# ZJU-FAST-Lab/uneven_planner

Hardware: AMD Instinct MI355X
Metric: MINCO traj-opts/sec (batch) (higher is better)
Workload: dtype f64

## Files before the change

### include/uneven_hip.h

```cpp
#ifndef UNEVEN_HIP_H
#define UNEVEN_HIP_H

#include <stdint.h>

#ifdef __cplusplus
extern "C" {
#endif

typedef struct uph_map uph_map;
typedef struct uph_ctx uph_ctx;
typedef struct uph_kino uph_kino;

#define UPH_OK 0
#define UPH_ERR_INVALID (-1)
#define UPH_ERR_HIP (-2)
#define UPH_ERR_NO_DEVICE (-3)
#define UPH_ERR_LIMIT (-4)
#define UPH_ERR_NO_CACHE (-5)

#define UPH_RET_STOPPED 3
#define UPH_RET_UNSUPPORTED 4

#define UPH_RET_LEFT_TILE 5
#define UPH_TILE_MARGIN 2.0
// ... 114 lines not shown
int uph_map_create(const uph_map_params* mp, int device, uph_map** out);
int uph_map_create_f32(const uph_map_params* mp, int device, uph_map** out);
int uph_map_storage_bytes(const uph_map* m);
int uph_map_create_tile(const uph_map_params* mp, int device, int32_t x0, int32_t x1, int32_t f32, uph_map** out);
int uph_map_tile(const uph_map* m, int32_t* x0, int32_t* x1);
int uph_map_fill_fbm(uph_map* m, const uph_fbm_params* fp, int32_t x0, int32_t x1);
int uph_fbm_table(const uph_fbm_params* fp, double* table);
int uph_map_get_window(uph_map* m, int32_t x0, int32_t x1, int32_t y0, int32_t y1, double* rxs2);
void uph_map_destroy(uph_map* m);
int uph_map_dims(const uph_map* m, int32_t dims3[3]);
int uph_map_set_cells(uph_map* m, const double* rxs2);
int uph_map_get_cells(uph_map* m, double* rxs2, double* c, char* occ, char* occ_r2);
int uph_map_save_csv(const char* path, const double* rxs2, const int32_t dims3[3]);
int uph_map_load_csv(const char* path, const int32_t dims3[3], double* rxs2, double* c, int64_t* n_lines);
int uph_map_save_bin(const char* path, const double* rxs2, const int32_t dims3[3]);
int uph_map_load_bin(const char* path, const int32_t dims3[3], double* rxs2);
int uph_map_save_cache(uph_map* m, const char* csv_path, const char* bin_path);
int uph_map_load_cache(uph_map* m, const char* csv_path, const char* bin_path, int32_t* source);
int uph_map_build(uph_map* m, const float* xyz, int64_t n, int32_t x0, int32_t x1);
int uph_map_build_filtered(uph_map* m, const float* xyz, int64_t n, int32_t x0, int32_t x1);
typedef struct uph_map_update_info {
    int32_t dirty[4];
    int32_t changed[4];
    int32_t n_refit;
    int32_t n_far;
    int32_t n_changed;
    int32_t full_refit;
    int64_t n_removed, n_added, n_cloud;
} uph_map_update_info;
int uph_map_update(uph_map* m, const float box[4], const float* xyz, int64_t n, uph_map_update_info* info);
int uph_map_update_rect(const uph_map_params* mp, const float box[4], int32_t rect[4]);
int uph_map_update_stages(uph_map* m, double* out6);
int uph_map_build_multi(uph_map* const* maps, int32_t n_gpus, const float* xyz, int64_t n);
int uph_multi_slab_plan(int32_t nx, int32_t n_gpus, int32_t* x0, int32_t* x1, int32_t* per, int32_t* in_place);
int uph_map_fill_fbm_multi(uph_map* const* maps, int32_t n_gpus, const uph_fbm_params* fp);
int uph_map_multi_stats(uph_map* lead, double* fit_ms, double* exchange_ms, double* commit_ms, double* exchange_device_ms, int32_t* via_rccl);
int uph_rccl_selftest(int32_t n_devices, char* info, int32_t info_cap);
void uph_multi_shutdown(void);

int uph_map_cells_device(uph_map* m, void** dptr, int64_t* nbytes);
int uph_map_commit(uph_map* m);
int uph_map_export_slab_dev(uph_map* m, int32_t x0, int32_t x1, void* dst_dev);
int uph_map_import_cells_dev(uph_map* m, const void* src_dev);
int uph_terrain_query(uph_map* m, const double* pos, int32_t n, double* values7, double* grads21);
int uph_frontend_query(uph_map* m, const double* pos, int32_t n, double* sigma, int32_t* occ, int32_t* occ_xy);
int uph_terrain_pose_query(uph_map* m, const double* pos, int32_t n, double* pose12);
int uph_frontend_query_ms(uph_map* m, double* kernel_ms);
int64_t uph_map_filter_cloud(const float* xyz, int64_t n, float* out_xyz, int64_t cap);
int uph_map_build_stats(uph_map* m, double* kernel_ms, int64_t* cell_iters, int64_t* cloud_points);
int uph_map_build_stages(uph_map* m, double* out6);
int64_t uph_map_built_cloud(uph_map* m, float* out_xyz, int64_t cap);

int uph_kino_create(uph_map* m, const uph_kino_params* kp, int32_t slots, uph_kino** out);
void uph_kino_destroy(uph_kino* k);
int uph_kino_slots(const uph_kino* k);
int uph_kino_set_wps(uph_kino* k, int32_t wps);
int uph_kino_set_flags(uph_kino* k, int32_t flags);
int uph_kino_primitives(const uph_kino* k);
int uph_kino_plan_batch(uph_kino* k, int32_t B, const double* starts, const double* goals, int32_t path_cap, double* paths, int32_t* n_path, int32_t* status,
                        int32_t* iter_num, int32_t* use_node_num, int32_t max_expand, int32_t exp_cap, int32_t* expanded);
int uph_kino_stats(uph_kino* k, double* kernel_ms);

#define UPH_PLAN_PATH_CAP 1024
int uph_plan_upload(uph_kino* k, uph_ctx* c, const uph_manager_params* mp, int32_t B, const double* starts, const double* goals, int32_t path_cap,
                    int32_t* status, int32_t* traj_of, int32_t* n_inner_xy, int32_t* n_inner_yaw);
int uph_replan_upload(uph_kino* k, uph_ctx* src, uph_ctx* dst, const uph_manager_params* mp, int32_t B, const int32_t* src_traj, const double* t_switch,
                      const double* goals, int32_t path_cap, double* switch_states, int32_t* status, int32_t* traj_of, int32_t* n_inner_xy, int32_t* n_inner_yaw);
int uph_traj_states(uph_ctx* c, int32_t n, const int32_t* traj, const double* t, double* out10);
#define UPH_REFINE_AT_END 7
int uph_refine_upload(uph_ctx* src, uph_ctx* dst, int32_t B, const int32_t* src_traj, const double* t_switch, double* switch_states ,
                      int32_t* status, int32_t* traj_of, int32_t* n_inner_xy, int32_t* n_inner_yaw);
int uph_plan_staged(uph_ctx* c, int32_t cap_xy, int32_t cap_yaw, double* init_xy, double* end_xy, double* init_yaw, double* end_yaw, double* inner_xy,
                    double* inner_yaw, int32_t* n_inner_xy, int32_t* n_inner_yaw, double* total_time);

int uph_ctx_create(uph_map* m, const uph_opt_params* p, uph_ctx** out);
void uph_ctx_destroy(uph_ctx* c);
int uph_ctx_set_lanes(uph_ctx* c, int32_t lanes);
int uph_ctx_set_xcd_locality(uph_ctx* c, int32_t group);
int uph_ctx_set_wps(uph_ctx* c, int32_t wps);
int uph_ctx_set_sample_precision(uph_ctx* c, int32_t bits);
int uph_ctx_set_rho(uph_ctx* c, double rho);
int uph_ctx_get_rho(uph_ctx* c, double* rho);
int uph_ctx_set_trial_abandon(uph_ctx* c, int32_t on);

int uph_ctx_set_trace(uph_ctx* c, int32_t cap);
int uph_ctx_get_trace(uph_ctx* c, double* out);

int uph_optimize_batch(uph_ctx* c, int32_t B, const uph_problem* probs, uph_result* results);
int uph_optimize_batch_multi(uph_ctx* const* ctxs, int32_t n_gpus, int32_t B, const uph_problem* probs, uph_result* results);
int uph_multi_batch_plan(int32_t n_gpus, int32_t B, const uph_problem* probs, int32_t* share_of, double* predicted_cost);
int uph_batch_count(const uph_ctx* c);
int uph_batch_origin(const uph_ctx* c, int32_t* idx);
int uph_batch_upload(uph_ctx* c, int32_t B, const uph_problem* probs);
int uph_batch_solve(uph_ctx* c);
int uph_batch_solve_async(uph_ctx* c);
int uph_batch_wait(uph_ctx* c);
int uph_batch_download(uph_ctx* c, uph_result* results);
int uph_batch_stats(uph_ctx* c, double* kernel_ms, int64_t* evals, int64_t* sample_evals, int64_t* lbfgs_iters, int64_t* hist_bytes);
int uph_batch_abandon_stats(uph_ctx* c, int64_t* out5);

int uph_batch_prepare_ms(uph_ctx* c, double* ms);

int uph_batch_cycles(uph_ctx* c, long long* out);

int uph_eval_batch(uph_ctx* c, const double* x_packed, double* f, double* grad_packed, int32_t repeat);
int uph_penalty_batch(uph_ctx* c, int32_t repeat, int32_t store_residuals, double* cost, double* gdcxy_packed, double* gdcyaw_packed, double* gdT2);
int uph_init_scaling_batch(uph_ctx* c);
int uph_microbench_batch(uph_ctx* c, int32_t reps);
int uph_batch_set_state(uph_ctx* c, const double* lambda, const double* mu, const double* scale_cx, const double* scale_fx, const double* rho);
int uph_batch_set_x(uph_ctx* c, const double* x_packed);
int uph_batch_alm_passes(uph_ctx* c, int32_t max_passes);
int uph_batch_set_lbfgs_state(uph_ctx* c, const double* g, const double* d, const double* pf, const double* lm_s, const double* lm_y, const double* lm_ys, const double* scal5);
int uph_batch_lbfgs_resume(uph_ctx* c, int32_t budget, int32_t finish_pass);
int uph_batch_get_lbfgs_state(uph_ctx* c, double* g, double* d, double* pf, double* lm_s, double* lm_y, double* lm_ys, double* scal8);
int uph_report_batch(uph_ctx* c, double* out7);

#define UPH_ROLLOUT_STATE 1
#define UPH_ROLLOUT_TERRAIN 2
#define UPH_ROLLOUT_POSE 4
#define UPH_ROLLOUT_ALL 7
#define UPH_ROLLOUT_MAX_SAMPLES 262144
int uph_rollout_sizes(int32_t B, const int32_t* n_xy, const double* T_xy, const int32_t* n_yaw, const double* T_yaw, double dt, int32_t with_end,
                      int64_t* offsets);
int uph_rollout_plan(uph_ctx* c, double dt, int32_t with_end, int64_t* offsets);
int uph_rollout_batch(uph_ctx* c, double dt, int32_t with_end, int32_t channels, int32_t b0, int32_t b1, double* out);
int uph_rollout_batch_dev(uph_ctx* c, double dt, int32_t with_end, int32_t channels, int32_t b0, int32_t b1, void* out_dev);

#define UPH_CHECK_OCC_BIT 7
int uph_check_limits(const uph_ctx* c, double* lim7);
int uph_check_window(double dt, int32_t with_end, double total, double t_from, double t_to, int32_t* q_lo, int32_t* q_hi, int32_t* end_row);
int uph_check_batch(uph_ctx* c, int32_t n, const int32_t* traj, const double* t_from, const double* t_to , double dt, int32_t with_end,
                    const double* lim7 , double* first_t , int32_t* first_mask ,
                    int32_t* counts , double* worst , double* worst_t );
int uph_check_kernel_ms(const uph_ctx* c, double* kernel_ms);

int uph_locate_batch(uph_ctx* c, int32_t n, const int32_t* traj, const double* poses , const double* t_from, const double* t_to ,
                     double dt, int32_t with_end, double* near_t , double* near_d2 , int32_t* count , double* t ,
                     int32_t* refined , double* state , double* d2 , double* err );
int uph_within_batch(uph_ctx* c, int32_t n, const int32_t* traj, const double* rects , const double* t_from, const double* t_to ,
                     double dt, int32_t with_end, double* enter_t , double* leave_t , int32_t* counts );
int uph_locate_kernel_ms(const uph_ctx* c, double* kernel_ms);

int uph_separation_times(double t_from, double t_to, double dt, int64_t* K);
int uph_extent_batch(uph_ctx* c, int32_t n, const int32_t* traj, const double* t0, const double* t_from, const double* t_to, double dt,
                     double* box , int32_t* counts );
int uph_separation_batch(uph_ctx* ca, uph_ctx* cb , int32_t n, const int32_t* traj_a, const int32_t* traj_b, const double* t0_a, const double* t0_b,
                         const double* t_from, const double* t_to, double dt, const double* radius, double* min_d2 , double* min_t ,
                         double* first_t , double* last_t , int32_t* counts );
int uph_conflict_candidates(int32_t n, const double* box , const double* radius , int64_t cap, int32_t* pairs , int64_t* n_pairs);
int uph_conflicts_batch(uph_ctx* c, int32_t n, const int32_t* traj, const double* t0, const double* radius , double t_from, double t_to, double dt,
                        int64_t cap, int32_t* pairs , double* rows , int32_t* below ,
                        int64_t* n_conflicts, int64_t* n_candidates);
int uph_separation_kernel_ms(const uph_ctx* c, double* kernel_ms);

int uph_footprint_radii(int32_t n, const double* shape , const double* margin , double* r );
int uph_footprint_separation_batch(uph_ctx* ca, uph_ctx* cb , int32_t n, const int32_t* traj_a, const int32_t* traj_b, const double* t0_a,
                                   const double* t0_b, const double* t_from, const double* t_to, double dt, const double* shape_a ,
                                   const double* shape_b , const double* margin , double* min_c2 , double* min_t ,
                                   double* first_t , double* last_t , int32_t* counts );
int uph_footprint_conflicts_batch(uph_ctx* c, int32_t n, const int32_t* traj, const double* t0, const double* shape ,
                                  const double* margin , double t_from, double t_to, double dt, int64_t cap, int32_t* pairs ,
                                  double* rows , int32_t* below , int64_t* n_conflicts,
                                  int64_t* n_candidates);
int uph_footprint_kernel_ms(const uph_ctx* c, double* kernel_ms);

#define UPH_DELAY_TILE 128
// ... 28 lines not shown
```

### uneven_planner_amd/_lib.py

```python
import ctypes as C
import os

_HERE = os.path.dirname(os.path.abspath(__file__))
LIB_PATH = os.environ.get("UNEVENHIP_LIB") or os.path.join(_HERE, "libunevenhip.so")


class MapParams(C.Structure):
    _fields_ = [("iter_num", C.c_int32), ("map_size_x", C.c_double), ("map_size_y", C.c_double),
                ("ellipsoid_x", C.c_double), ("ellipsoid_y", C.c_double), ("ellipsoid_z", C.c_double),
                ("xy_resolution", C.c_double), ("yaw_resolution", C.c_double), ("min_cnormal", C.c_double),
                ("max_rho", C.c_double), ("gravity", C.c_double)]


class OptParams(C.Structure):
    _fields_ = [("rho_T", C.c_double), ("rho_ter", C.c_double), ("max_vel", C.c_double), ("max_acc_lon", C.c_double),
                ("max_acc_lat", C.c_double), ("max_kap", C.c_double), ("min_cxi", C.c_double), ("max_sig", C.c_double),
                ("use_scaling", C.c_int32), ("rho", C.c_double), ("beta", C.c_double), ("gamma", C.c_double),
                ("epsilon_con", C.c_double), ("max_iter", C.c_double), ("g_epsilon", C.c_double),
                ("min_step", C.c_double), ("inner_max_iter", C.c_double), ("delta", C.c_double),
                ("mem_size", C.c_int32), ("past", C.c_int32), ("int_K", C.c_int32)]


class ManagerParams(C.Structure):
    _fields_ = [("piece_len", C.c_double), ("mean_vel", C.c_double), ("init_time_times", C.c_double), ("yaw_piece_times", C.c_double),
# ... 18 lines not shown
                ("full_refit", C.c_int32), ("n_removed", C.c_int64), ("n_added", C.c_int64), ("n_cloud", C.c_int64)]


FBM_MAX_WAVES = 48
FBM_TABLE_DOUBLES = 4 * FBM_MAX_WAVES + 12 + 9
DP = C.POINTER(C.c_double)


class Problem(C.Structure):
    _fields_ = [("n_inner_xy", C.c_int32), ("n_inner_yaw", C.c_int32), ("init_xy", C.c_double * 6),
                ("end_xy", C.c_double * 6), ("init_yaw", C.c_double * 3), ("end_yaw", C.c_double * 3),
                ("inner_xy", DP), ("inner_yaw", DP), ("total_time", C.c_double)]


class Result(C.Structure):
    _fields_ = [("ret_code", C.c_int32), ("alm_iters", C.c_int32), ("lbfgs_iters", C.c_int32), ("evals", C.c_int32),
                ("last_lbfgs_ret", C.c_int32), ("cost", C.c_double), ("jerk_cost", C.c_double),
                ("piece_T_xy", C.c_double), ("piece_T_yaw", C.c_double), ("rho_final", C.c_double),
                ("scale_fx", C.c_double), ("x_final", DP), ("c_xy", DP), ("c_yaw", DP), ("hx", DP), ("gx", DP),
                ("lambda_", DP), ("mu", DP), ("scale_cx", DP)]


_VP = C.c_void_p
_I32, _I64 = C.c_int32, C.c_int64
SYMBOLS = {
    "uph_last_error": (C.c_char_p, []),
    "uph_device_count": (C.c_int, []),
    "uph_version": (C.c_char_p, []),
    "uph_resample_batch": (C.c_int, [C.POINTER(ManagerParams), _I32, DP, C.POINTER(_I64), _I32, _I32, DP, DP, DP, DP, DP, DP, C.POINTER(_I32), C.POINTER(_I32), DP, DP]),
    "uph_map_create": (C.c_int, [C.POINTER(MapParams), C.c_int, C.POINTER(_VP)]),
    "uph_map_create_f32": (C.c_int, [C.POINTER(MapParams), C.c_int, C.POINTER(_VP)]),
    "uph_map_storage_bytes": (C.c_int, [_VP]),
    "uph_map_create_tile": (C.c_int, [C.POINTER(MapParams), C.c_int, _I32, _I32, _I32, C.POINTER(_VP)]),
    "uph_map_tile": (C.c_int, [_VP, C.POINTER(_I32), C.POINTER(_I32)]),
    "uph_map_fill_fbm": (C.c_int, [_VP, C.POINTER(FbmParams), _I32, _I32]),
    "uph_fbm_table": (C.c_int, [C.POINTER(FbmParams), DP]),
    "uph_map_get_window": (C.c_int, [_VP, _I32, _I32, _I32, _I32, DP]),
    "uph_map_save_csv": (C.c_int, [C.c_char_p, DP, C.POINTER(_I32)]),
    "uph_map_load_csv": (C.c_int, [C.c_char_p, C.POINTER(_I32), DP, DP, C.POINTER(_I64)]),
    "uph_map_save_bin": (C.c_int, [C.c_char_p, DP, C.POINTER(_I32)]),
    "uph_map_load_bin": (C.c_int, [C.c_char_p, C.POINTER(_I32), DP]),
    "uph_map_save_cache": (C.c_int, [_VP, C.c_char_p, C.c_char_p]),
    "uph_map_load_cache": (C.c_int, [_VP, C.c_char_p, C.c_char_p, C.POINTER(_I32)]),
    "uph_map_destroy": (None, [_VP]),
    "uph_map_dims": (C.c_int, [_VP, C.POINTER(_I32)]),
    "uph_map_set_cells": (C.c_int, [_VP, DP]),
    "uph_map_get_cells": (C.c_int, [_VP, DP, DP, C.c_char_p, C.c_char_p]),
    "uph_map_build": (C.c_int, [_VP, C.POINTER(C.c_float), _I64, _I32, _I32]),
    "uph_map_build_filtered": (C.c_int, [_VP, C.POINTER(C.c_float), _I64, _I32, _I32]),
    "uph_map_update": (C.c_int, [_VP, C.POINTER(C.c_float), C.POINTER(C.c_float), _I64, C.POINTER(MapUpdateInfo)]),
    "uph_map_update_rect": (C.c_int, [C.POINTER(MapParams), C.POINTER(C.c_float), C.POINTER(_I32)]),
    "uph_map_update_stages": (C.c_int, [_VP, DP]),
    "uph_map_build_multi": (C.c_int, [C.POINTER(_VP), _I32, C.POINTER(C.c_float), _I64]),
    "uph_map_fill_fbm_multi": (C.c_int, [C.POINTER(_VP), _I32, C.POINTER(FbmParams)]),
    "uph_multi_slab_plan": (C.c_int, [_I32, _I32, C.POINTER(_I32), C.POINTER(_I32), C.POINTER(_I32), C.POINTER(_I32)]),
    "uph_multi_batch_plan": (C.c_int, [_I32, _I32, C.POINTER(Problem), C.POINTER(_I32), DP]),
    "uph_map_multi_stats": (C.c_int, [_VP, DP, DP, DP, DP, C.POINTER(_I32)]),
    "uph_multi_shutdown": (None, []),
    "uph_rccl_selftest": (C.c_int, [_I32, C.c_char_p, _I32]),
    "uph_optimize_batch_multi": (C.c_int, [C.POINTER(_VP), _I32, _I32, C.POINTER(Problem), C.POINTER(Result)]),
    "uph_batch_count": (C.c_int, [_VP]),
    "uph_batch_origin": (C.c_int, [_VP, C.POINTER(_I32)]),
    "uph_map_cells_device": (C.c_int, [_VP, C.POINTER(_VP), C.POINTER(_I64)]),
    "uph_map_commit": (C.c_int, [_VP]),
    "uph_map_export_slab_dev": (C.c_int, [_VP, _I32, _I32, _VP]),
    "uph_map_import_cells_dev": (C.c_int, [_VP, _VP]),
    "uph_terrain_query": (C.c_int, [_VP, DP, _I32, DP, DP]),
    "uph_frontend_query": (C.c_int, [_VP, DP, _I32, DP, C.POINTER(C.c_int32), C.POINTER(C.c_int32)]),
    "uph_terrain_pose_query": (C.c_int, [_VP, DP, _I32, DP]),
    "uph_frontend_query_ms": (C.c_int, [_VP, DP]),
    "uph_map_filter_cloud": (_I64, [C.POINTER(C.c_float), _I64, C.POINTER(C.c_float), _I64]),
    "uph_map_build_stats": (C.c_int, [_VP, DP, C.POINTER(_I64), C.POINTER(_I64)]),
    "uph_map_build_stages": (C.c_int, [_VP, DP]),
    "uph_map_built_cloud": (_I64, [_VP, C.POINTER(C.c_float), _I64]),
    "uph_ctx_create": (C.c_int, [_VP, C.POINTER(OptParams), C.POINTER(_VP)]),
    "uph_ctx_destroy": (None, [_VP]),
    "uph_ctx_set_lanes": (C.c_int, [_VP, _I32]),
    "uph_ctx_set_wps": (C.c_int, [_VP, _I32]),
    "uph_ctx_set_xcd_locality": (C.c_int, [_VP, _I32]),
    "uph_ctx_set_sample_precision": (C.c_int, [_VP, _I32]),
    "uph_ctx_set_rho": (C.c_int, [_VP, C.c_double]),
    "uph_ctx_get_rho": (C.c_int, [_VP, DP]),
    "uph_ctx_set_trial_abandon": (C.c_int, [_VP, _I32]),
    "uph_ctx_set_trace": (C.c_int, [_VP, _I32]),
    "uph_ctx_get_trace": (C.c_int, [_VP, DP]),
    "uph_optimize_batch": (C.c_int, [_VP, _I32, C.POINTER(Problem), C.POINTER(Result)]),
    "uph_batch_upload": (C.c_int, [_VP, _I32, C.POINTER(Problem)]),
    "uph_batch_solve": (C.c_int, [_VP]),
    "uph_batch_solve_async": (C.c_int, [_VP]),
    "uph_batch_wait": (C.c_int, [_VP]),
    "uph_batch_download": (C.c_int, [_VP, C.POINTER(Result)]),
    "uph_batch_stats": (C.c_int, [_VP, DP, C.POINTER(_I64), C.POINTER(_I64), C.POINTER(_I64), C.POINTER(_I64)]),
    "uph_batch_prepare_ms": (C.c_int, [_VP, DP]),
    "uph_batch_abandon_stats": (C.c_int, [_VP, C.POINTER(_I64)]),
    "uph_batch_cycles": (C.c_int, [_VP, C.POINTER(C.c_longlong)]),
    "uph_build_id": (C.c_char_p, []),
    "uph_eval_batch": (C.c_int, [_VP, DP, DP, DP, _I32]),
    "uph_penalty_batch": (C.c_int, [_VP, _I32, _I32, DP, DP, DP, DP]),
    "uph_init_scaling_batch": (C.c_int, [_VP]),
    "uph_microbench_batch": (C.c_int, [_VP, _I32]),
    "uph_batch_set_state": (C.c_int, [_VP, DP, DP, DP, DP, DP]),
    "uph_report_batch": (C.c_int, [_VP, DP]),
    "uph_rollout_sizes": (C.c_int, [_I32, C.POINTER(_I32), DP, C.POINTER(_I32), DP, C.c_double, _I32, C.POINTER(_I64)]),
    "uph_rollout_plan": (C.c_int, [_VP, C.c_double, _I32, C.POINTER(_I64)]),
    "uph_rollout_batch": (C.c_int, [_VP, C.c_double, _I32, _I32, _I32, _I32, DP]),
    "uph_rollout_batch_dev": (C.c_int, [_VP, C.c_double, _I32, _I32, _I32, _I32, _VP]),
    "uph_batch_set_x": (C.c_int, [_VP, DP]),
    "uph_batch_alm_passes": (C.c_int, [_VP, _I32]),
    "uph_batch_set_lbfgs_state": (C.c_int, [_VP, DP, DP, DP, DP, DP, DP, DP]),
    "uph_batch_lbfgs_resume": (C.c_int, [_VP, _I32, _I32]),
    "uph_batch_get_lbfgs_state": (C.c_int, [_VP, DP, DP, DP, DP, DP, DP, DP]),
    "uph_kino_create": (C.c_int, [_VP, C.POINTER(KinoParams), _I32, C.POINTER(_VP)]),
    "uph_kino_destroy": (None, [_VP]),
    "uph_kino_slots": (C.c_int, [_VP]),
    "uph_kino_set_wps": (C.c_int, [_VP, _I32]),
    "uph_kino_set_flags": (C.c_int, [_VP, _I32]),
    "uph_kino_primitives": (C.c_int, [_VP]),
    "uph_kino_plan_batch": (C.c_int, [_VP, _I32, DP, DP, _I32, DP, C.POINTER(_I32), C.POINTER(_I32), C.POINTER(_I32), C.POINTER(_I32), _I32, _I32, C.POINTER(_I32)]),
    "uph_kino_stats": (C.c_int, [_VP, DP]),
    "uph_plan_upload": (C.c_int, [_VP, _VP, C.POINTER(ManagerParams), _I32, DP, DP, _I32, C.POINTER(_I32), C.POINTER(_I32), C.POINTER(_I32), C.POINTER(_I32)]),
    "uph_plan_staged": (C.c_int, [_VP, _I32, _I32, DP, DP, DP, DP, DP, DP, C.POINTER(_I32), C.POINTER(_I32), DP]),
    "uph_replan_upload": (C.c_int, [_VP, _VP, _VP, C.POINTER(ManagerParams), _I32, C.POINTER(_I32), DP, DP, _I32, DP, C.POINTER(_I32), C.POINTER(_I32),
                                    C.POINTER(_I32), C.POINTER(_I32)]),
    "uph_traj_states": (C.c_int, [_VP, _I32, C.POINTER(_I32), DP, DP]),
    "uph_refine_upload": (C.c_int, [_VP, _VP, _I32, C.POINTER(_I32), DP, DP, C.POINTER(_I32), C.POINTER(_I32), C.POINTER(_I32), C.POINTER(_I32)]),
    "uph_check_limits": (C.c_int, [_VP, DP]),
    "uph_check_window": (C.c_int, [C.c_double, _I32, C.c_double, C.c_double, C.c_double, C.POINTER(_I32), C.POINTER(_I32), C.POINTER(_I32)]),
    "uph_check_batch": (C.c_int, [_VP, _I32, C.POINTER(_I32), DP, DP, C.c_double, _I32, DP, DP, C.POINTER(_I32), C.POINTER(_I32), DP, DP]),
    "uph_check_kernel_ms": (C.c_int, [_VP, DP]),
    "uph_locate_batch": (C.c_int, [_VP, _I32, C.POINTER(_I32), DP, DP, DP, C.c_double, _I32, DP, DP, C.POINTER(_I32), DP, C.POINTER(_I32), DP, DP, DP]),
    "uph_within_batch": (C.c_int, [_VP, _I32, C.POINTER(_I32), DP, DP, DP, C.c_double, _I32, DP, DP, C.POINTER(_I32)]),
    "uph_locate_kernel_ms": (C.c_int, [_VP, DP]),
    "uph_separation_times": (C.c_int, [C.c_double, C.c_double, C.c_double, C.POINTER(_I64)]),
    "uph_extent_batch": (C.c_int, [_VP, _I32, C.POINTER(_I32), DP, DP, DP, C.c_double, DP, C.POINTER(_I32)]),
    "uph_separation_batch": (C.c_int, [_VP, _VP, _I32, C.POINTER(_I32), C.POINTER(_I32), DP, DP, DP, DP, C.c_double, DP, DP, DP, DP, DP, C.POINTER(_I32)]),
    "uph_conflict_candidates": (C.c_int, [_I32, DP, DP, _I64, C.POINTER(_I32), C.POINTER(_I64)]),
    "uph_conflicts_batch": (C.c_int, [_VP, _I32, C.POINTER(_I32), DP, DP, C.c_double, C.c_double, C.c_double, _I64, C.POINTER(_I32), DP, C.POINTER(_I32),
                                      C.POINTER(_I64), C.POINTER(_I64)]),
    "uph_separation_kernel_ms": (C.c_int, [_VP, DP]),
    "uph_footprint_radii": (C.c_int, [_I32, DP, DP, DP]),
    "uph_footprint_separation_batch": (C.c_int, [_VP, _VP, _I32, C.POINTER(_I32), C.POINTER(_I32), DP, DP, DP, DP, C.c_double, DP, DP, DP, DP, DP, DP, DP,
                                                 C.POINTER(_I32)]),
    "uph_footprint_conflicts_batch": (C.c_int, [_VP, _I32, C.POINTER(_I32), DP, DP, DP, C.c_double, C.c_double, C.c_double, _I64, C.POINTER(_I32), DP,
                                                C.POINTER(_I32), C.POINTER(_I64), C.POINTER(_I64)]),
    "uph_footprint_kernel_ms": (C.c_int, [_VP, DP]),
    "uph_delay_times": (C.c_int, [C.c_double, C.c_double, _I32, DP]),
    "uph_delay_levels": (C.c_int, [_I32, _I64, C.POINTER(_I32), C.POINTER(_I32)]),
    "uph_delay_sweep_batch": (C.c_int, [_VP, _VP, _I32, C.POINTER(_I32), C.POINTER(_I32), DP, DP, DP, DP, C.c_double, DP, C.c_double, C.c_double, _I32, DP, DP,
                                        C.POINTER(_I32), C.POINTER(_I32), C.POINTER(_I32)]),
    "uph_delay_extent_batch": (C.c_int, [_VP, _I32, C.POINTER(_I32), DP, DP, DP, C.c_double, C.c_double, C.c_double, _I32, DP, C.POINTER(_I32)]),
    "uph_delays_batch": (C.c_int, [_VP, _I32, C.POINTER(_I32), DP, DP, C.POINTER(_I32), C.c_double, C.c_double, C.c_double, C.c_double, C.c_double, _I32,
                                   C.POINTER(_I32), DP, C.POINTER(_I32), C.POINTER(_I64), C.POINTER(_I32), C.POINTER(_I32)]),
    "uph_footprint_delay_sweep_batch": (C.c_int, [_VP, _VP, _I32, C.POINTER(_I32), C.POINTER(_I32), DP, DP, DP, DP, C.c_double, DP, DP, DP, C.c_double, C.c_double,
                                                  _I32, DP, DP, C.POINTER(_I32), C.POINTER(_I32), C.POINTER(_I32), C.POINTER(_I32)]),
    "uph_footprint_delays_batch": (C.c_int, [_VP, _I32, C.POINTER(_I32), DP, DP, DP, C.POINTER(_I32), C.c_double, C.c_double, C.c_double, C.c_double, C.c_double,
                                             _I32, C.POINTER(_I32), DP, C.POINTER(_I32), C.POINTER(_I64), C.POINTER(_I32), C.POINTER(_I32)]),
    "uph_delay_kernel_ms": (C.c_int, [_VP, DP]),
}

_LIB = None


UPH_ERR_NO_CACHE = -5
UPH_PLAN_PATH_CAP = 1024
UPH_MAX_PIECE_XY = 128
UPH_MAX_PIECE_YAW = 256
# ... 70 lines not shown
```

### uneven_planner_amd/alm_traj_opt.py

```python
import ctypes as C

import numpy as np

from . import _lib

HILL_OPT_PARAMS = dict(rho_T=100000.0, rho_ter=10.0, max_vel=0.5, max_acc_lon=5.0, max_acc_lat=10.0, max_kap=2.1,
                       min_cxi=0.8, max_sig=0.05, use_scaling=True, rho=1.0, beta=1000.0, gamma=1.0,
                       epsilon_con=0.001, max_iter=10.0, g_epsilon=1.0e-3, min_step=1.0e-32, inner_max_iter=10000.0,
                       delta=1.0e-4, mem_size=256, past=3, int_K=16)
_INT_FIELDS = ("use_scaling", "mem_size", "past", "int_K")


def pack_problems(probs, int_K=16, with_sizes=False):
    arr = (_lib.Problem * len(probs))()
    keep, sizes = [], []
    for i, pr in enumerate(probs):
        ixy = np.ascontiguousarray(np.asarray(pr["inner_xy"], dtype=np.float64).T)
        iyw = np.ascontiguousarray(pr["inner_yaw"], dtype=np.float64)
        keep += [ixy, iyw]
        a = arr[i]
        a.n_inner_xy, a.n_inner_yaw = ixy.shape[0], iyw.shape[0]
        a.init_xy[:] = np.asarray(pr["init_xy"], dtype=np.float64).T.ravel().tolist()
        a.end_xy[:] = np.asarray(pr["end_xy"], dtype=np.float64).T.ravel().tolist()
        a.init_yaw[:] = np.asarray(pr["init_yaw"], dtype=np.float64).ravel().tolist()
# ... 417 lines not shown
        raise _lib.UnevenHipError("delay_levels: a pair does not have 0 <= i < j < n")
    level = np.zeros(n, dtype=np.int32)
    for j, i in sorted(map(tuple, pairs[:, ::-1].tolist())):
        level[j] = max(level[j], level[i] + 1)
    return level


def delay_schedule(sweep, pairs, n, n_delays=None, order=None):
    pairs = np.asarray(pairs, dtype=np.int64).reshape(-1, 2)
    ahead = [[] for _ in range(n)]
    for h, i in sorted(map(tuple, pairs.tolist())):
        ahead[i].append(h)
    choice, blocker = np.zeros(n, dtype=np.int32), np.full(n, -1, dtype=np.int32)
    placed = np.zeros(n, dtype=bool)
    for i in (range(n) if order is None else order):
        assert all(placed[h] for h in ahead[i]), "delay_schedule: a vehicle ahead of %d is not placed yet" % i
        placed[i] = True
        if not ahead[i]:
            continue
        below = np.stack([np.asarray(sweep(h, max(int(choice[h]), 0), i)) for h in ahead[i]])
        nd = below.shape[1] if n_delays is None else int(n_delays[i])
        clear = np.nonzero((below[:, :nd] == 0).all(axis=0))[0]
        if clear.size:
            choice[i] = clear[0]
        else:
            choice[i] = -1
            blocker[i] = ahead[i][int(np.nonzero(below[:, 0] > 0)[0][0])]
    return dict(choice=choice, blocker=blocker)


class ALMTrajOpt:
    def __init__(self, uneven_map=None, params=None):
        self.L = _lib.load()
        q = dict(HILL_OPT_PARAMS)
        if params:
            q.update(params)
        for k, v in q.items():
            setattr(self, k, v)
        self._pnames = list(q.keys())
        self.h = None
        self.uneven_map = None
        self.in_opt = False
        self._B = 0
        self._sizes = []
        self._last = []
        if uneven_map is not None:
            self.setEnvironment(uneven_map)

    def __del__(self):
        try:
            if self.h:
                self.L.uph_ctx_destroy(self.h)
                self.h = None
        except Exception:
            pass

    def setEnvironment(self, env):
        self.uneven_map = env
        if self.h:
            self.L.uph_ctx_destroy(self.h)
            self.h = None
        p = _lib.OptParams(**{k: (int(getattr(self, k)) if k in _INT_FIELDS else float(getattr(self, k))) for k in self._pnames})
        h = C.c_void_p()
        _lib.check(self.L.uph_ctx_create(env.h, C.byref(p), C.byref(h)), "uph_ctx_create")
        self.h = h

    def set_lanes(self, lanes):
        _lib.check(self.L.uph_ctx_set_lanes(self.h, int(lanes)), "uph_ctx_set_lanes")

    def set_xcd_locality(self, group):
        _lib.check(self.L.uph_ctx_set_xcd_locality(self.h, int(group)), "uph_ctx_set_xcd_locality")

    def set_wps(self, wps):
        _lib.check(self.L.uph_ctx_set_wps(self.h, int(wps)), "uph_ctx_set_wps")

    def set_sample_precision(self, bits):
        _lib.check(self.L.uph_ctx_set_sample_precision(self.h, int(bits)), "uph_ctx_set_sample_precision")

    def set_rho(self, rho):
        _lib.check(self.L.uph_ctx_set_rho(self.h, float(rho)), "uph_ctx_set_rho")

    def set_trial_abandon(self, on):
        _lib.check(self.L.uph_ctx_set_trial_abandon(self.h, 1 if on else 0), "uph_ctx_set_trial_abandon")

    def get_rho(self):
        r = C.c_double(0)
        _lib.check(self.L.uph_ctx_get_rho(self.h, C.byref(r)), "uph_ctx_get_rho")
        return r.value

    def _make_problems(self, probs):
        arr, keep, self._sizes = pack_problems(probs, int(self.int_K), with_sizes=True)
        return arr, keep

    def upload(self, probs):
        arr, keep = self._make_problems(probs)
        self._B = 0
        _lib.check(self.L.uph_batch_upload(self.h, len(probs), arr), "uph_batch_upload")
        self._B = len(probs)
        self._trace_cap_up = getattr(self, "_trace_cap", 0)

    def solve(self):
        _lib.check(self.L.uph_batch_solve(self.h), "uph_batch_solve")

    def solve_async(self):
        _lib.check(self.L.uph_batch_solve_async(self.h), "uph_batch_solve_async")

    def wait(self):
        _lib.check(self.L.uph_batch_wait(self.h), "uph_batch_wait")

    def stats(self):
        ms = C.c_double(0)
        v = [C.c_int64(0) for _ in range(4)]
        _lib.check(self.L.uph_batch_stats(self.h, C.byref(ms), *[C.byref(x) for x in v]), "uph_batch_stats")
        pm = C.c_double(0)
        _lib.check(self.L.uph_batch_prepare_ms(self.h, C.byref(pm)), "uph_batch_prepare_ms")
        ab = (C.c_int64 * 5)()
        _lib.check(self.L.uph_batch_abandon_stats(self.h, ab), "uph_batch_abandon_stats")
        return dict(kernel_ms=ms.value, prepare_ms=pm.value, evals=v[0].value, sample_evals=v[1].value, lbfgs_iters=v[2].value, hist_bytes=v[3].value,
                    ls_rejected=ab[0], ls_guarded=ab[1], ls_abandoned=ab[2], chunks_skipped=ab[3], adjoints_skipped=ab[4])

    def cycles(self):
        out = np.zeros((max(0, self.L.uph_batch_count(self.h)), 16), dtype=np.int64)
        _lib.check(self.L.uph_batch_cycles(self.h, out.ctypes.data_as(C.POINTER(C.c_longlong))), "uph_batch_cycles")
        return out

    def origin(self):
        idx = np.zeros(max(0, self.L.uph_batch_count(self.h)), dtype=np.int32)
        _lib.check(self.L.uph_batch_origin(self.h, _ip(idx)), "uph_batch_origin")
        return idx

    def download(self, full=True):
        res, bufs = self._result_array(self._sizes, full)
        _lib.check(self.L.uph_batch_download(self.h, res), "uph_batch_download")
        self._last = self._collect(res, bufs)
        return self._last

    def optimize_batch(self, probs):
        self.upload(probs)
        self.solve()
        return self.download()

    def _result_array(self, sizes, full):
        res = (_lib.Result * len(sizes))()
        bufs = []
        for i, sz in enumerate(sizes):
            b = dict(x=np.zeros(sz["n"]), c_xy=np.zeros((6 * sz["Nxy"], 2)), c_yaw=np.zeros(6 * sz["Nyaw"]))
            r = res[i]
            r.x_final, r.c_xy, r.c_yaw = _dp(b["x"]), _dp(b["c_xy"]), _dp(b["c_yaw"])
            if full:
                b.update(hx=np.zeros(sz["S"]), gx=np.zeros(6 * sz["S"]), lam=np.zeros(sz["S"]), mu=np.zeros(6 * sz["S"]), scale_cx=np.zeros(7 * sz["S"]))
                r.hx, r.gx, r.lambda_, r.mu, r.scale_cx = _dp(b["hx"]), _dp(b["gx"]), _dp(b["lam"]), _dp(b["mu"]), _dp(b["scale_cx"])
            bufs.append(b)
        return res, bufs

    @staticmethod
    def _collect(res, bufs):
        out = []
        for i, b in enumerate(bufs):
            r = res[i]
            b.update(ret=r.ret_code, alm_iters=r.alm_iters, lbfgs_iters=r.lbfgs_iters, evals=r.evals, last_lbfgs_ret=r.last_lbfgs_ret,
                     cost=r.cost, jerk_cost=r.jerk_cost, T_xy=r.piece_T_xy, T_yaw=r.piece_T_yaw, rho_final=r.rho_final, scale_fx=r.scale_fx)
            out.append(b)
        return out

    def prepare_boundary(self, probs, full=False):
        arr, keep = self._make_problems(probs)
# ... 518 lines not shown
```

### uneven_planner_amd/csrc/solver_program.hpp

```cpp
#pragma once
#include "terrain_dev.hpp"
#include "trajectory_dev.hpp"
#include "uph_common.hpp"

namespace uph {

#ifndef UPH_GRID_FROM_MEM
#define UPH_GRID_FROM_MEM 1
#endif
#ifndef UPH_PHASE_MASK
#define UPH_PHASE_MASK 15
#endif
#ifndef UPH_STATE_PROBE
#define UPH_STATE_PROBE(st) do { } while (0)
#endif
#ifndef UPH_SCALING_WB
#define UPH_SCALING_WB 8
#endif
#ifndef UPH_SC_XB
#define UPH_SC_XB 9
#endif
#ifndef UPH_SC_YB
#define UPH_SC_YB 14
#endif
#ifndef UPH_SC_WLO
#define UPH_SC_WLO 2
#endif
#ifndef UPH_SC_WHI
#define UPH_SC_WHI 3
#endif

#ifndef UPH_ASIDE_PREP
#define UPH_ASIDE_PREP 1
#endif
template <class WG, class F>
UPH_HD void asideKnotSolve(WG& wg, int lenW, int lenX, int n, F f) {
    (void)lenW; (void)lenX;
    wg.pfor(n, f);
}

template <class WG, class SR = double>
struct Solver {
    WG& wg;
    const GridDev& grid;
    const OptParams& P;
    const BatchDev& bd;
    const TrajDesc& td;
    int Nxy, Nyaw, n, S, K, mem, CH, CHP, recd;
    int CHS;
    int* rtag;
    double *x, *xp, *g, *gp, *d, *cxy, *cyaw, *Gxy, *Gyaw, *gamxy, *gamyaw, *bt, *rec, *wtab, *ttab, *pf, *hd;
    double* ab;
    int* abn;
    static constexpr int AB_DOUBLES = 4;
    double* up;
    static constexpr int UP_DOUBLES = 6;
    UPH_HD void tally(int k, bool yes) {
#if defined(__HIP_DEVICE_COMPILE__)
        if (yes && wg.wave == 0) abn[k] = abn[k] + 1;
#else
        if (yes) abn[k]++;
#endif
    }
    double *dual, *res, *scl, *hist;
    int hrow, hnp;
    const double *Wr_xy, *Wr_yaw;
    double rho, scale_fx, Txy, Tyaw, last_jerk, last_gd;
    long long hist_reads;
    long long cyc[16];
    long long t_last_eval_end;
    long long* sub_t = nullptr;
    int evals, bidx, trace_n;
    float inv_k1;
    double ec_irho, ec_step, ec_invK, ec_iTyaw, ec_omega, ec_omega_h;

    static constexpr int REC_FIELDS = 12;
    static UPH_HD size_t ldsDoubles(int Nxy, int Nyaw, int n, int CH, int mem, int K) {
        size_t recd = (size_t)REC_FIELDS * (CH + 1) + (CH + 1) / 2;
        const size_t nvec = 2 * (Nxy + 5) + (Nyaw + 5);
        const size_t knd = (size_t)knotBufDoubles(Nxy + 1, 4) + knotBufDoubles(Nyaw + 1, 2), adj = (size_t)knotBufDoubles(Nxy, 4) + knotBufDoubles(Nyaw, 2) + nvec;
        recd = recd < knd ? knd : recd;
        recd = recd < adj ? adj : recd;
        recd = recd < (size_t)mem ? (size_t)mem : recd;
        const size_t td_ = (size_t)Nxy + K + 2;
        return (size_t)5 * n + (nvec < td_ ? td_ : nvec) + 2 * (12 * Nxy + 6 * Nyaw) + recd + (size_t)6 * (K + 1) + THOMAS_DOUBLES + MAX_PAST + 8 + 18 + AB_DOUBLES + UP_DOUBLES;
    }

    UPH_HD Solver(WG& w, const GridDev& gr, const OptParams& p, const BatchDev& b, int bi, double* lds)
        : wg(w), grid(gr), P(p), bd(b), td(b.desc[bi]) {
        bidx = bi;
        Nxy = td.Nxy; Nyaw = td.Nyaw; n = td.n; S = td.S; K = P.int_K; mem = P.mem_size;
        inv_k1 = 1.0f / (float)(K + 1);
        CH = wg.size(); CHP = CH + 1; recd = REC_FIELDS * CHP + (CH + 1) / 2;
        CHS = CH;
#if !defined(UPH_ALIGNED_CHUNKS) || UPH_ALIGNED_CHUNKS
        {
            const int ppc = CH / (K + 1);
            if (ppc >= 1 && (Nxy + ppc - 1) / ppc == (S + CH - 1) / CH) CHS = ppc * (K + 1);
        }
#endif
        double* q = lds;
        x = q; q += n; g = q; q += n; d = q; q += n;
        xp = q; q += n; gp = q; q += n;
        const int nvec = 2 * (Nxy + 5) + (Nyaw + 5);
        bt = q;
        gamxy = q; gamyaw = q + 2 * (Nxy + 5);
        q += nvec < Nxy + K + 2 ? Nxy + K + 2 : nvec;
        cxy = q; q += 12 * Nxy; cyaw = q; q += 6 * Nyaw;
        Gxy = q; q += 12 * Nxy; Gyaw = q; q += 6 * Nyaw;
        wtab = q; q += 6 * (K + 1);
        rec = q;
        {
            size_t rd = (size_t)recd;
            const size_t knd = (size_t)knotBufDoubles(Nxy + 1, 4) + knotBufDoubles(Nyaw + 1, 2), adj = (size_t)knotBufDoubles(Nxy, 4) + knotBufDoubles(Nyaw, 2) + nvec;
            rd = rd < knd ? knd : rd; rd = rd < adj ? adj : rd; rd = rd < (size_t)mem ? (size_t)mem : rd;
            q += rd;
        }
        rtag = (int*)(rec + (size_t)REC_FIELDS * CHP);
        ttab = q; q += THOMAS_DOUBLES;
        pf = q; q += MAX_PAST + 8;
        hd = q; q += 18;
        ab = q; q += AB_DOUBLES;
        abn = (int*)(ab + 1);
        up = q; q += UP_DOUBLES;
        dual = bd.dual + 7 * td.off_s; res = bd.res + 7 * td.off_s; scl = bd.scl + 7 * td.off_s;
        hist = bd.hist + td.off_hist; hrow = histRowDoubles(n); hnp = 64 * histNQ(n);
        Wr_xy = bd.ops[td.op_xy].Wr; Wr_yaw = bd.ops[td.op_yaw].Wr;
        rho = 0; scale_fx = 1.0; Txy = Tyaw = 0; last_jerk = 0; hist_reads = 0; evals = 0; trace_n = 0;
        for (int q = 0; q < 16; q++) cyc[q] = 0;
        t_last_eval_end = 0;
        wg.pfor(18 + THOMAS_DOUBLES, [&](int t) {
            if (t == 0) { ab[0] = 0.0; abn[0] = abn[1] = abn[2] = abn[3] = 0; }
            if (t < 18) hd[t] = t < 6 ? td.init_xy[t] : (t < 12 ? td.end_xy[t - 6] : (t < 15 ? td.init_yaw[t - 12] : td.end_yaw[t - 15]));
            else ttab[t - 18] = bd.thomas[t - 18];
        });
    }

    UPH_HD void tracePush(double v) {
        if (bd.trace != nullptr && trace_n < bd.trace_cap) {
            const int at = trace_n;
            wg.one([&]() { bd.trace[(size_t)bidx * bd.trace_cap + at] = v; });
        }
        trace_n++;
    }

    static UPH_HD int divSmall(int a, int b, float inv) {
        int q = (int)((float)a * inv);
        const int r = a - q * b;
        if (r < 0) q--;
        else if (r >= b) q++;
        return q;
    }
    static UPH_HD int knotCol(int j, int N) { return j == 0 ? 0 : (j == N ? N + 2 : j + 2); }
    UPH_HD double knotPos(const double* xin, int j, int dd) const {
        if (dd < 2) return j == 0 ? hd[dd] : (j == Nxy ? hd[6 + dd] : xin[1 + 2 * (j - 1) + dd]);
        return j == 0 ? hd[12] : (j == Nyaw ? hd[15] : xin[1 + 2 * (Nxy - 1) + (j - 1)]);
    }

    UPH_HD double dot(const double* a, const double* b, int m) {
        double r[1];
        wg.template sum<1>(m, r, [&](int i, double* acc) { acc[0] += a[i] * b[i]; });
        return r[0];
    }
    UPH_HD double absmax(const double* a, int m) {
        return wg.maxv(m, [&](int i) { return fabs(a[i]); });
    }

    template <bool STEP>
    UPH_HD void generate(double* xin, double st) {
        UPH_MARK("generate");
        const long long tsub_start = wg.clock();
        const double tau_ = STEP ? fma(st, d[0], xp[0]) : xin[0];
        const double Ttot = expC2(tau_);
        Txy = wg.bcast(Ttot / (double)Nxy);
        Tyaw = wg.bcast(Ttot / (double)Nyaw);
#if !(UPH_ASIDE_PREP)
        ec_iTyaw = wg.bcast(1.0 / Tyaw);
#endif
        const double Tx = Txy, Ty = Tyaw;
        double* zxy = rec;
        double* zyaw = rec + knotBufDoubles(Nxy + 1, 4);
        wg.pfor(2 * (Nxy + 1) + (Nyaw + 1), [&](int t) {
            const bool isxy = t < 2 * (Nxy + 1);
            const int j = isxy ? (t >> 1) : t - 2 * (Nxy + 1), dd = isxy ? (t & 1) : 2, N = isxy ? Nxy : Nyaw, os = isxy ? 2 : 1;
            const double T1 = isxy ? Tx : Ty;
            const double* h0 = isxy ? hd + (dd & 1) : hd + 12;
            const double* h1 = isxy ? hd + 6 + (dd & 1) : hd + 15;
            double* z = isxy ? zxy + knotOffJ(j, 4) + (dd & 1) : zyaw + knotOffJ(j, 2);
            if (STEP && t == 0) xin[0] = tau_;
            if (j == 0) { z[0] = T1 * h0[os]; z[os] = T1 * T1 * h0[2 * os]; }
            else if (j == N) { z[0] = T1 * h1[os]; z[os] = T1 * T1 * h1[2 * os]; }
            else {
                double pm, p0, pp;
                if (STEP) {
                    const int ix = isxy ? 1 + 2 * (j - 1) + dd : 1 + 2 * (Nxy - 1) + (j - 1), ws = isxy ? 2 : 1;
                    p0 = fma(st, d[ix], xp[ix]);
                    pm = j == 1 ? h0[0] : fma(st, d[ix - ws], xp[ix - ws]);
                    pp = j == N - 1 ? h1[0] : fma(st, d[ix + ws], xp[ix + ws]);
                    xin[ix] = p0;
                } else { pm = knotPos(xin, j - 1, dd); p0 = knotPos(xin, j, dd); pp = knotPos(xin, j + 1, dd); }
                const double dp = pp - p0, dm = p0 - pm;
                double r0 = 20.0 * (dp - dm), r1 = -15.0 * (dp + dm);
                if (j == 1) { const double v0 = T1 * h0[os], a0 = T1 * T1 * h0[2 * os]; r0 += 8.0 * v0 + a0; r1 += 7.0 * v0 + a0; }
                if (j == N - 1) { const double vN = T1 * h1[os], aN = T1 * T1 * h1[2 * os]; r0 += -8.0 * vN + aN; r1 += 7.0 * vN - aN; }
                z[0] = r0; z[os] = r1;
            }
        });
// ... 575 lines not shown
    template <bool STEP>
    UPH_HD double eval(double* xin, double* gout, double st = 0.0, double thr = __builtin_huge_val()) {
        evals++;
        long long t0 = wg.clock();
        if (t_last_eval_end) cyc[5] += t0 - t_last_eval_end;
        if (UPH_PHASE_MASK & 1) generate<STEP>(xin, st);
        const double tau = wg.bcast(xin[0]);
        const double jw = wg.bcast(P.use_scaling ? scale_trick_jerk * scale_fx : scale_fx);
        double js[3] = {0.0, 0.0, 0.0};
        if (UPH_PHASE_MASK & 1) expand(xin, jw, js);
        long long t1 = wg.clock(); cyc[0] += t1 - t0;
        last_jerk = js[0];
        const double jerk_cost = wg.bcast(P.use_scaling ? js[0] * scale_fx * scale_trick_jerk : js[0] * scale_fx);
        evalConsts(evalStep());
        if (STEP && thr < __builtin_huge_val()) {
#if UPH_ASIDE_PREP
            double eq = wg.bcast(up[3]);
            pinv(eq);
            const double tau_lb = P.rho_T * eq * scale_fx;
#else
            double tq = tau;
            pinv(tq);
            const double tau_lb = P.rho_T * expC2(tq) * scale_fx;
#endif
            const double lbd = wg.bcast(ab[0]);
            const double L0 = wg.bcast(jerk_cost + tau_lb - lbd);
            const double mag = wg.bcast(fabs(jerk_cost) + fabs(tau_lb) + lbd);
            if (L0 > thr + ABANDON_REL * mag && L0 < __builtin_huge_val() && ec_omega >= 0.0) {
                tally(2, true);
                t_last_eval_end = wg.clock();
                return L0;
            }
        }
        double sm[3] = {0.0, 0.0, 0.0};
        wg.template accBegin<3>();
        for (int s0 = 0; s0 < S; s0 += CHS) {
            const int cnt = S - s0 < CHS ? S - s0 : CHS;
            t0 = wg.clock();
            if (UPH_PHASE_MASK & 2) wg.template accChunk<3>(cnt, [&](int t, double* acc) { sampleEval<false, SR>(s0 + t, t, acc); });
            t1 = wg.clock(); cyc[1] += t1 - t0;
            if (UPH_PHASE_MASK & 4) scatterChunk(s0, cnt);
            cyc[2] += wg.clock() - t1;
        }
        wg.template accEnd<3>(sm);
        t1 = wg.clock();
        if (STEP && thr < __builtin_huge_val()) {
#if UPH_ASIDE_PREP
            double eq = wg.bcast(up[3]);
            pinv(eq);
            const double tau_q = P.rho_T * eq * scale_fx;
#else
            double tq = tau;
            pinv(tq);
            const double tau_q = P.rho_T * expC2(tq) * scale_fx;
#endif
            const double fq = wg.bcast(jerk_cost + sm[0] + tau_q);
            const double mag = wg.bcast(fabs(jerk_cost) + fabs(sm[0]) + fabs(tau_q));
            if (fq > thr + ABANDON_REL_F * mag && fq < __builtin_huge_val()) {
                tally(3, true);
                t_last_eval_end = wg.clock();
                return fq;
            }
        }
        double chx = 0.0, chy = 0.0, gdw = 0.0;
        if (UPH_PHASE_MASK & 8) adjoint(chx, chy, gout, &gdw);
        t0 = wg.clock(); cyc[3] += t0 - t1;
        const double gTx = js[1] * jw + sm[1] + chx;
        const double gTy = js[2] * jw + sm[2] + chy;
        const double grad_Tsum = P.rho_T * scale_fx + gTx / Nxy + gTy / Nyaw;
#if UPH_ASIDE_PREP
        const double g0 = wg.bcast(grad_Tsum * wg.bcast(up[4]));
        const double etau = wg.bcast(up[3]);
#else
        const double g0 = wg.bcast(grad_Tsum * getTtoTauGrad(tau));
        const double etau = expC2(tau);
#endif
        wg.pfor(1, [&](int) { gout[0] = g0; });
        last_gd = wg.bcast(gdw + g0 * d[0]);
        const double tau_cost = P.rho_T * etau * scale_fx;
        t_last_eval_end = wg.clock();
        return wg.bcast(jerk_cost + sm[0] + tau_cost);
    }

    UPH_HD void initScaling(double* x0) {
        generate<false>(x0, 0.0);
        const double tau = x0[0];
        const double dTau = getTtoTauGrad(tau);
        double js[3];
        expand(x0, 1.0, js);
        double sm[3] = {0.0, 0.0, 0.0};
        for (int s0 = 0; s0 < S; s0 += CHS) {
            const int cnt = S - s0 < CHS ? S - s0 : CHS;
            double part[3];
            wg.template sum<3>(cnt, part, [&](int t, double* acc) { sampleObjective(s0 + t, t, acc); });
            sm[0] += part[0]; sm[1] += part[1]; sm[2] += part[2];
            scatterChunk(s0, cnt);
        }
        double chx, chy;
        adjoint(chx, chy);
        const double gTau_fx = (P.rho_T + (js[1] + sm[1] + chx) / Nxy + (js[2] + sm[2] + chy) / Nyaw) * dTau;
        const double mq = wg.maxv((Nxy - 1) * 2 + (Nyaw - 1), [&](int t) {
            return t < (Nxy - 1) * 2 ? fabs(gamxy[3 * 2 + t]) : fabs(gamyaw[3 + (t - (Nxy - 1) * 2)]);
        });
        scale_fx = wg.bcast(1.0 / dmax(1.0, dmax(mq, fabs(gTau_fx))));
        wg.pfor(2, [&](int u) { fillTimes(u); });
        wg.pfor(S, [&](int s) { scalingSample(s, dTau); });
    }

    UPH_HD void scalingSample(int s, double dTau) {
        const int i = divSmall(s, K + 1, inv_k1), j = s - i * (K + 1);
        Kin k;
        kin(i, j, k);
#if !defined(UPH_SCALING_GROUPS) || UPH_SCALING_GROUPS == 2
        scalingGroup<0, 4>(s, i, j, k, dTau);
        scalingGroup<4, 3>(s, i, j, k, dTau);
#elif UPH_SCALING_GROUPS == 3
        scalingGroup<0, 3>(s, i, j, k, dTau);
        scalingGroup<3, 2>(s, i, j, k, dTau);
        scalingGroup<5, 2>(s, i, j, k, dTau);
#else
        scalingGroup<0, 7>(s, i, j, k, dTau);
#endif
    }
    template <int Q0, int NQS>
    UPH_HD void scalingGroup(int s, int i, int j, const Kin& k, double dTau) {
        const int nbx = Nxy + 5, nby = Nyaw + 5;
        const double Tx = Txy, Ty = Tyaw, itx = 1.0 / Txy, ity = 1.0 / Tyaw;
        const double gravity = grid.gravity;
        const double alpha = 1.0 / K * j;
        const double icvx = k.tv[0], icvy = k.tv[2], icxi = k.tv[5];
        const int m = k.yaw_idx;
        double dpL[NQS][2], dvL[NQS][2], daL[NQS][2], dpR[NQS][2], dvR[NQS][2], daR[NQS][2];
        double ypL[NQS], yvL[NQS], yaL[NQS], ypR[NQS], yvR[NQS], yaR[NQS];
        double sumx[NQS], sumy[NQS], mx[NQS];
#pragma unroll
        for (int qi = 0; qi < NQS; qi++) {
            const int q = Q0 + qi;
            double gp_[2] = {0, 0}, gv_[2] = {0, 0}, ga_[2] = {0, 0}, gyaw = 0.0, gdyaw = 0.0, gse2[3];
            if (q == 0) {
                gv_[0] = k.syaw; gv_[1] = -k.cyaw;
                gyaw = k.vel[0] * k.cyaw + k.vel[1] * k.syaw;
            } else if (q == 1) {
                for (int t = 0; t < 2; t++) gv_[t] = 1.0 * icvx * icvx * 2.0 * k.vel[t];
                for (int t = 0; t < 3; t++) gse2[t] = 1.0 * k.v_norm * k.v_norm * 2.0 * icvx * k.tg[0][t];
                gp_[0] = gse2[0]; gp_[1] = gse2[1]; gyaw = gse2[2];
            } else if (q == 2) {
                const double gax = 2.0 * k.ax;
                ga_[0] = gax * icvx * k.cyaw; ga_[1] = gax * icvx * k.syaw;
                gyaw = gax * icvx * k.lat_acc;
                for (int t = 0; t < 3; t++) gse2[t] = gax * (gravity * k.tg[1][t] + k.tg[0][t] * k.lon_acc);
                gp_[0] = gse2[0]; gp_[1] = gse2[1]; gyaw += gse2[2];
            } else if (q == 3) {
                const double gay = 2.0 * k.ay;
                ga_[0] = gay * icvy * (-k.syaw); ga_[1] = gay * icvy * k.cyaw;
                gyaw = -gay * icvy * k.lon_acc;
                for (int t = 0; t < 3; t++) gse2[t] = gay * (gravity * k.tg[3][t] + k.tg[2][t] * k.lat_acc);
                gp_[0] = gse2[0]; gp_[1] = gse2[1]; gyaw += gse2[2];
            } else if (q == 4) {
                const double den = 1.0 / (k.vx * k.vx + delta_sigl);
                const double gwz = den * 2.0 * k.wz;
                const double gvx2 = -k.curv_snorm * den;
                gdyaw = gwz * icxi;
                for (int t = 0; t < 3; t++) gse2[t] = gwz * k.dyaw * k.tg[5][t];
                for (int t = 0; t < 2; t++) gv_[t] = gvx2 * icvx * icvx * 2.0 * k.vel[t];
                for (int t = 0; t < 3; t++) gse2[t] += gvx2 * k.v_norm * k.v_norm * 2.0 * icvx * k.tg[0][t];
                gp_[0] = gse2[0]; gp_[1] = gse2[1]; gyaw = gse2[2];
            } else if (q == 5) {
                gp_[0] = -k.tg[4][0]; gp_[1] = -k.tg[4][1]; gyaw = -k.tg[4][2];
            } else {
                gp_[0] = k.tg[6][0]; gp_[1] = k.tg[6][1]; gyaw = k.tg[6][2];
            }
            double gx_[6][2], gy_[6];
            double chain_x = 0.0, chain_y = 0.0, sx = 1.0, sy = 1.0;
            for (int kk = 0; kk < 6; kk++) {
                for (int t = 0; t < 2; t++) {
                    const double v = k.b0[kk] * gp_[t] + k.b1[kk] * gv_[t] + k.b2[kk] * ga_[t];
                    chain_x += -(double)kk * cxy[12 * i + kk * 2 + t] * itx * v;
                    gx_[kk][t] = v * sx;
                }
                const double vy = k.y0[kk] * gyaw + k.y1[kk] * gdyaw;
                chain_y += -(double)kk * cyaw[6 * m + kk] * ity * vy;
                gy_[kk] = vy * sy;
                sx *= itx; sy *= ity;
            }
            double tx = ((gp_[0] * k.vel[0] + gp_[1] * k.vel[1]) + (gv_[0] * k.acc[0] + gv_[1] * k.acc[1]) + (ga_[0] * k.jer[0] + ga_[1] * k.jer[1])) * alpha;
            const double yawdot = gyaw * k.dyaw + gdyaw * k.d2yaw;
            tx += yawdot * (alpha + i);
            const double ty = -yawdot * m;
            sumx[qi] = tx + chain_x;
            sumy[qi] = ty + chain_y;
            mx[qi] = 0.0;
            for (int t = 0; t < 2; t++) {
                const double g0 = gx_[0][t], g1 = gx_[1][t], g2 = gx_[2][t], g3 = gx_[3][t], g4 = gx_[4][t], g5 = gx_[5][t];
                dpL[qi][t] = g0 - 10.0 * g3 + 15.0 * g4 - 6.0 * g5; dvL[qi][t] = g1 - 6.0 * g3 + 8.0 * g4 - 3.0 * g5; daL[qi][t] = 0.5 * g2 - 1.5 * g3 + 1.5 * g4 - 0.5 * g5;
                dpR[qi][t] = 10.0 * g3 - 15.0 * g4 + 6.0 * g5; dvR[qi][t] = -4.0 * g3 + 7.0 * g4 - 3.0 * g5; daR[qi][t] = 0.5 * g3 - g4 + 0.5 * g5;
            }
            {
                const double g0 = gy_[0], g1 = gy_[1], g2 = gy_[2], g3 = gy_[3], g4 = gy_[4], g5 = gy_[5];
                ypL[qi] = g0 - 10.0 * g3 + 15.0 * g4 - 6.0 * g5; yvL[qi] = g1 - 6.0 * g3 + 8.0 * g4 - 3.0 * g5; yaL[qi] = 0.5 * g2 - 1.5 * g3 + 1.5 * g4 - 0.5 * g5;
                ypR[qi] = 10.0 * g3 - 15.0 * g4 + 6.0 * g5; yvR[qi] = -4.0 * g3 + 7.0 * g4 - 3.0 * g5; yaR[qi] = 0.5 * g3 - g4 + 0.5 * g5;
            }
        }
        const bool inL = i >= 1, inR = i + 1 <= Nxy - 1;
        const auto WL = UPH_AS_GLOBAL(Wr_xy + (size_t)(inL ? 2 * (i - 1) : 0) * nbx);
        const auto WR = UPH_AS_GLOBAL(Wr_xy + (size_t)(inR ? 2 * i : 0) * nbx);
        const int pcL = knotCol(i, Nxy), pcR = knotCol(i + 1, Nxy);
        for (int c0 = 3; c0 < Nxy + 2; c0 += UPH_SCALING_WB) {
            double w[4][UPH_SCALING_WB];
#pragma unroll
            for (int u = 0; u < UPH_SCALING_WB; u++) {
                const int cc = c0 + u < Nxy + 2 ? c0 + u : Nxy + 1;
                w[0][u] = WL[cc]; w[1][u] = WL[nbx + cc]; w[2][u] = WR[cc]; w[3][u] = WR[nbx + cc];
            }
#pragma unroll
            for (int q = 0; q < NQS; q++) {
                const double c00 = inL ? dvL[q][0] : 0.0, c01 = inL ? dvL[q][1] : 0.0, c10 = inL ? daL[q][0] : 0.0, c11 = inL ? daL[q][1] : 0.0;
                const double c20 = inR ? dvR[q][0] : 0.0, c21 = inR ? dvR[q][1] : 0.0, c30 = inR ? daR[q][0] : 0.0, c31 = inR ? daR[q][1] : 0.0;
                double mq = mx[q];
#pragma unroll
                for (int u = 0; u < UPH_SCALING_WB; u++) {
                    const int col = c0 + u;
                    double a0 = (w[0][u] * c00 + w[1][u] * c10) + (w[2][u] * c20 + w[3][u] * c30);
                    double a1 = (w[0][u] * c01 + w[1][u] * c11) + (w[2][u] * c21 + w[3][u] * c31);
                    if (col == pcL) { a0 += dpL[q][0]; a1 += dpL[q][1]; }
                    if (col == pcR) { a0 += dpR[q][0]; a1 += dpR[q][1]; }
                    if (col < Nxy + 2) mq = dmax(mq, dmax(fabs(a0), fabs(a1)));
                }
                mx[q] = mq;
            }
        }
        double htx[NQS], hty[NQS];
        {
            const int sc[4] = {1, 2, Nxy + 3, Nxy + 4};
            double w[4][4];
#pragma unroll
            for (int u = 0; u < 4; u++) { w[0][u] = WL[sc[u]]; w[1][u] = WL[nbx + sc[u]]; w[2][u] = WR[sc[u]]; w[3][u] = WR[nbx + sc[u]]; }
#pragma unroll
            for (int q = 0; q < NQS; q++) {
                const double c00 = inL ? dvL[q][0] : 0.0, c01 = inL ? dvL[q][1] : 0.0, c10 = inL ? daL[q][0] : 0.0, c11 = inL ? daL[q][1] : 0.0;
                const double c20 = inR ? dvR[q][0] : 0.0, c21 = inR ? dvR[q][1] : 0.0, c30 = inR ? daR[q][0] : 0.0, c31 = inR ? daR[q][1] : 0.0;
                double a0[4], a1[4];
#pragma unroll
                for (int u = 0; u < 4; u++) {
                    a0[u] = (w[0][u] * c00 + w[1][u] * c10) + (w[2][u] * c20 + w[3][u] * c30);
                    a1[u] = (w[0][u] * c01 + w[1][u] * c11) + (w[2][u] * c21 + w[3][u] * c31);
                }
                if (!inL) { a0[0] += dvL[q][0]; a1[0] += dvL[q][1]; a0[1] += daL[q][0]; a1[1] += daL[q][1]; }
                if (!inR) { a0[2] += dvR[q][0]; a1[2] += dvR[q][1]; a0[3] += daR[q][0]; a1[3] += daR[q][1]; }
                double headtail_x = 0.0;
                headtail_x += a0[0] * hd[2] + a1[0] * hd[3];
                headtail_x += 2.0 * Tx * (a0[1] * hd[4] + a1[1] * hd[5]);
                headtail_x += a0[2] * hd[8] + a1[2] * hd[9];
                headtail_x += 2.0 * Tx * (a0[3] * hd[10] + a1[3] * hd[11]);
                htx[q] = headtail_x;
            }
        }
        const bool yL = m >= 1, yR = m + 1 <= Nyaw - 1;
        const auto VL = UPH_AS_GLOBAL(Wr_yaw + (size_t)(yL ? 2 * (m - 1) : 0) * nby);
        const auto VR = UPH_AS_GLOBAL(Wr_yaw + (size_t)(yR ? 2 * m : 0) * nby);
        const int qL = knotCol(m, Nyaw), qR = knotCol(m + 1, Nyaw);
        for (int c0 = 3; c0 < Nyaw + 2; c0 += UPH_SCALING_WB) {
            double w[4][UPH_SCALING_WB];
#pragma unroll
            for (int u = 0; u < UPH_SCALING_WB; u++) {
                const int cc = c0 + u < Nyaw + 2 ? c0 + u : Nyaw + 1;
                w[0][u] = VL[cc]; w[1][u] = VL[nby + cc]; w[2][u] = VR[cc]; w[3][u] = VR[nby + cc];
            }
#pragma unroll
            for (int q = 0; q < NQS; q++) {
                const double y0_ = yL ? yvL[q] : 0.0, y1_ = yL ? yaL[q] : 0.0, y2_ = yR ? yvR[q] : 0.0, y3_ = yR ? yaR[q] : 0.0;
                double mq = mx[q];
#pragma unroll
                for (int u = 0; u < UPH_SCALING_WB; u++) {
                    const int col = c0 + u;
                    double a0 = (w[0][u] * y0_ + w[1][u] * y1_) + (w[2][u] * y2_ + w[3][u] * y3_);
                    if (col == qL) a0 += ypL[q];
                    if (col == qR) a0 += ypR[q];
                    if (col < Nyaw + 2) mq = dmax(mq, fabs(a0));
                }
                mx[q] = mq;
            }
        }
        {
            const int sc[4] = {1, 2, Nyaw + 3, Nyaw + 4};
            double w[4][4];
#pragma unroll
            for (int u = 0; u < 4; u++) { w[0][u] = VL[sc[u]]; w[1][u] = VL[nby + sc[u]]; w[2][u] = VR[sc[u]]; w[3][u] = VR[nby + sc[u]]; }
#pragma unroll
            for (int q = 0; q < NQS; q++) {
                const double y0_ = yL ? yvL[q] : 0.0, y1_ = yL ? yaL[q] : 0.0, y2_ = yR ? yvR[q] : 0.0, y3_ = yR ? yaR[q] : 0.0;
                double a0[4];
#pragma unroll
                for (int u = 0; u < 4; u++) a0[u] = (w[0][u] * y0_ + w[1][u] * y1_) + (w[2][u] * y2_ + w[3][u] * y3_);
                if (!yL) { a0[0] += yvL[q]; a0[1] += yaL[q]; }
                if (!yR) { a0[2] += yvR[q]; a0[3] += yaR[q]; }
                double headtail_y = 0.0;
                headtail_y += a0[0] * hd[13];
                headtail_y += 2.0 * Ty * a0[1] * hd[14];
                headtail_y += a0[2] * hd[16];
                headtail_y += 2.0 * Ty * a0[3] * hd[17];
                hty[q] = headtail_y;
            }
        }
#pragma unroll
        for (int q = 0; q < NQS; q++) {
            const double gTau = ((sumx[q] + htx[q]) / Nxy + (sumy[q] + hty[q]) / Nyaw) * dTau;
            scl[(Q0 + q) * S + s] = 1.0 / dmax(1.0, dmax(mx[q], fabs(gTau)));
        }
    }

    UPH_HD bool abandonAllowed() const {
        if (sizeof(SR) != sizeof(double)) return false;
#if defined(__HIP_DEVICE_COMPILE__) && UPH_GRID_FROM_MEM
        typedef const __attribute__((address_space(4))) int* pi_t;
        pi_t pt = (pi_t)(const void*)&bd.params_mem->no_trial_abandon;
        asm volatile("" : "+s"(pt));
        return *pt == 0;
#else
        return P.no_trial_abandon == 0;
#endif
    }
    static UPH_HD bool noExitAfterRejection(int count, double stp, double mu, double stpmin, double stpmax, int max_linesearch, double machine_prec) {
        return count + 1 < max_linesearch && (stp - mu) >= machine_prec * stp && 0.5 * (mu + stp) >= stpmin && stp <= stpmax;
    }
    UPH_HD int lineSearch(double& f, double& stp, double stpmin, double stpmax, double dginit) {
        int count = 0;
        bool brackt = false, touched = false;
        double mu = 0.0, nu = stpmax;
        if (!(stp > 0.0)) return LBFGSERR_INVALIDPARAMETERS;
        if (0.0 < dginit) return LBFGSERR_INCREASEGRADIENT;
        const double finit = wg.bcast(f);
        const double dgtest = wg.bcast(P.f_dec_coeff * dginit);
        const double dstest = wg.bcast(P.s_curv_coeff * dginit);
        const bool on = abandonAllowed();
        const double pst = wg.bcast(P.past > 0 ? P.delta / P.past * (fabs(finit) + 1.0) : 0.0);
        while (true) {
            const double arm = stp * dgtest;
            const bool may = on && noExitAfterRejection(count, stp, mu, stpmin, stpmax, P.max_linesearch, P.machine_prec);
            const double thr = wg.bcast(may ? dmax(finit + arm, finit + pst) + ABANDON_REL * (fabs(finit) + fabs(arm) + pst) : __builtin_huge_val());
            f = eval<true>(x, g, stp, thr);
            ++count;
            if (isinf(f) || isnan(f)) return LBFGSERR_INVALID_FUNCVAL;
            if (P.past > 0 && fabs(finit - f) / (fabs(finit) + 1.0) < P.delta / P.past) return count;
            if (f > finit + stp * dgtest) {
                tally(0, on); tally(1, on && !may);
                nu = stp;
                brackt = true;
            } else {
                if (last_gd < dstest) mu = stp;
                else return count;
            }
            if (P.max_linesearch <= count) return LBFGSERR_MAXIMUMLINESEARCH;
            if (brackt && (nu - mu) < P.machine_prec * nu) return LBFGSERR_WIDTHTOOSMALL;
            if (brackt) stp = wg.bcast(0.5 * (mu + nu));
            else stp = wg.bcast(stp * 2.0);
            if (stp < stpmin) return LBFGSERR_MINIMUMSTEP;
            if (stp > stpmax) {
                if (touched) return LBFGSERR_MAXIMUMSTEP;
                touched = true;
                stp = stpmax;
            }
        }
    }

    struct ResumeIO { double step, fx; int k, end, bound, budget; };
    static constexpr int LBFGS_RUNNING_HOOK = 999;
    template <bool RESUME>
    UPH_HD int lbfgs(double& f_out, int& k_out, ResumeIO* io = nullptr) {
        int ret = 0, k = 0, ls, end = 0, bound = 0, budget = 0;
        double step = 0.0, fx = 0.0, ys, yy, dginit = 0.0;
        const int m = mem;
        bool run = true;
        if constexpr (RESUME) {
            step = io->step; fx = io->fx; k = io->k; end = io->end; bound = io->bound; budget = io->budget;
            wg.pfor(n, [&](int i) { xp[i] = x[i]; gp[i] = g[i]; });
            dginit = dot(g, d, n);
        } else {
            fx = eval<false>(x, g);
            wg.pfor(n + 1, [&](int i) { if (i < n) { d[i] = -g[i]; xp[i] = x[i]; gp[i] = g[i]; } else pf[0] = fx; });
            const double gnorm0 = absmax(g, n), xnorm0 = absmax(x, n);
            if (gnorm0 / dmax(1.0, xnorm0) < P.g_epsilon) {
                ret = LBFGS_CONVERGENCE;
                run = false;
            } else {
                const double dd0 = dot(d, d, n);
                step = 1.0 / sqrt(dd0);
                dginit = -dd0;
                k = 1; end = 0; bound = 0;
            }
        }
// ... 47 lines not shown
                        double* h0 = hist + (size_t)e0 * hrow;
                        h0[0] = ysv; h0[1] = 1.0 / ysv;
                    });
                }
                ++k;
                dginit = -r5[4];
                if (ys > cau) {
                    ++bound;
                    bound = m < bound ? m : bound;
                    end = (end + 1) % m;
                    const long long tq = wg.clock();
                    cyc[7] += tq - t_last_eval_end;
                    UPH_MARK("twoLoop");
                    wg.twoLoop(d, g, n, hist, pf + MAX_PAST, rec, m, end, bound, ys / yy);
                    dginit = wg.bcast(pf[MAX_PAST]);
                    t_last_eval_end = wg.clock();
                    cyc[4] += t_last_eval_end - tq;
                    hist_reads += (long long)4 * bound * n;
                }
                step = 1.0;
            }
        }
        if constexpr (RESUME) { io->step = step; io->fx = fx; io->k = k; io->end = end; io->bound = bound; }
        f_out = fx;
        k_out = k;
        return ret;
    }

    UPH_HD void setDualBound(double sq) {
        const double v = rho > 0.0 ? sq * (0.5 / rho) : __builtin_huge_val();
        wg.one([&]() { ab[0] = v; });
    }
    UPH_HD void formDualBound() {
        double sq[1];
        wg.template sum<1>(S, sq, [&](int s, double* acc) {
            double a = 0.0;
            for (int q = 0; q < 7; q++) { const double v = dual[q * S + s]; a += v * v; }
            acc[0] += a;
        });
        setDualBound(sq[0]);
    }
    UPH_HD void updateDualVars() {
        UPH_MARK("updateDualVars");
        const double r = rho;
        double sq[1];
        wg.template sum<1>(S, sq, [&](int s, double* acc) {
            dual[s] += r * res[s];
            for (int q = 1; q < 7; q++) dual[q * S + s] = dmax(dual[q * S + s] + r * res[q * S + s], 0.0);
            double a = 0.0;
            for (int q = 0; q < 7; q++) { const double v = dual[q * S + s]; a += v * v; }
            acc[0] += a;
        });
        rho = wg.bcast(dmin((1 + P.gamma) * rho, P.beta));
        setDualBound(sq[0]);
    }
    UPH_HD bool judgeConvergence() {
        const double r = rho;
        const double rh = wg.maxv(S, [&](int s) { return fabs(res[s]); });
        const double rg = wg.maxv(6 * S, [&](int t) { return fabs(dmax(res[S + t], -dual[S + t] / r)); });
        return dmax(rh, rg) < P.epsilon_con;
    }

    UPH_HD void storeTrajectory(TrajState& st) {
        double* oc = bd.cxy + td.off_cxy;
        double* oy = bd.cyaw + td.off_cyaw;
        wg.pfor(12 * Nxy + 6 * Nyaw, [&](int t) { if (t < 12 * Nxy) oc[t] = cxy[t]; else oy[t - 12 * Nxy] = cyaw[t - 12 * Nxy]; });
        wg.pfor(1, [&](int) {
            st.T_xy = Txy; st.T_yaw = Tyaw; st.jerk_cost = last_jerk; st.scale_fx = scale_fx; st.rho = rho;
            st.evals = evals; st.hist_reads = hist_reads;
            st.ls_rejected = abn[0]; st.ls_guarded = abn[1]; st.ls_abandoned = abn[2]; st.adjoints_skipped = abn[3] + abn[2];
            st.chunks_skipped = abn[2] * ((S + CHS - 1) / CHS);
#ifdef UPH_TL_PROF
            for (int q = 0; q < 6; q++) cyc[8 + q] = wg.tl[q];
#endif
            for (int q = 0; q < 16; q++) st.cyc[q] = cyc[q];
        });
        UPH_STATE_PROBE(st);
#ifdef UPH_BAR_PROF
        wg.sync();
        wg.dumpBar(&st.cyc[8]);
#endif
    }

    UPH_HD void prepare(TrajState& st) {
        const double* gx0 = bd.x0 + td.off_x;
        double* gx = bd.x + td.off_x;
        rho = wg.bcast(st.rho);
        scale_fx = 1.0;
        wg.pfor(S > n ? S : n, [&](int t) {
            if (t < n) { x[t] = gx0[t]; gx[t] = gx0[t]; }
            if (t < S) for (int q = 0; q < 7; q++) { dual[q * S + t] = 0.0; res[q * S + t] = 0.0; scl[q * S + t] = 1.0; }
        });
        const long long tstart = wg.clock();
        if (P.use_scaling) initScaling(x);
        cyc[5] += wg.clock() - tstart;
        wg.pfor(1, [&](int) { st.scale_fx = scale_fx; st.cyc[5] = cyc[5]; });
    }

    UPH_HD void optimize(TrajState& st, int cap = 0) {
        double* gx0 = bd.x + td.off_x;
        rho = wg.bcast(st.rho);
        scale_fx = wg.bcast(st.scale_fx);
        wg.pfor(n, [&](int t) { x[t] = gx0[t]; });
        formDualBound();
        const long long tstart = wg.clock();
        cyc[14] = wg.realtime();
        int ret_code = 0, iter = 0, total_k = 0, last_ret = 0;
        double inner_cost = 0.0;
        while (true) {
            int kk = 0;
            tracePush(-1.0);
            const int result = lbfgs<false>(inner_cost, kk);
            refreshResiduals();
            total_k += kk;
            last_ret = result;
            if (result == LBFGS_CONVERGENCE || result == LBFGS_CANCELED || result == LBFGS_STOP || result == LBFGSERR_MAXIMUMITERATION) {
            } else if (result == LBFGSERR_MAXIMUMLINESEARCH) {
            } else { ret_code = 1; break; }
            updateDualVars();
            if (judgeConvergence()) break;
            if (++iter > P.max_iter) { ret_code = 2; break; }
            if (cap > 0 && iter >= cap) { ret_code = 3; break; }
        }
        wg.pfor(n, [&](int t) { gx0[t] = x[t]; bd.gout[td.off_x + t] = g[t]; });
        cyc[6] = wg.clock() - tstart;
        cyc[15] = wg.realtime();
        storeTrajectory(st);
        wg.pfor(1, [&](int) {
            st.ret_code = ret_code; st.alm_iters = iter; st.lbfgs_iters = total_k; st.last_lbfgs_ret = last_ret; st.f = inner_cost;
        });
    }

    UPH_HD void resumeHook(TrajState& st, int budget, int finish) {
        double* gx = bd.x + td.off_x;
        double* gg = bd.gout + td.off_x;
        double* gd = bd.rs_d + td.off_x;
        double* rs = bd.rs + (size_t)bidx * 24;
        rho = wg.bcast(st.rho); scale_fx = wg.bcast(st.scale_fx);
        formDualBound();
        wg.pfor(n + MAX_PAST, [&](int t) { if (t < n) { x[t] = gx[t]; g[t] = gg[t]; d[t] = gd[t]; } else pf[t - n] = rs[8 + t - n]; });
        ResumeIO io;
        io.step = wg.bcast(rs[0]); io.fx = wg.bcast(rs[1]);
        io.k = (int)wg.bcast(rs[2]); io.end = (int)wg.bcast(rs[3]); io.bound = (int)wg.bcast(rs[4]); io.budget = budget;
        double f = 0.0;
        int kk = 0;
        const int ret = lbfgs<true>(f, kk, &io);
        int accepted = 0, conv = 0;
        if (evals > 0) refreshResiduals();
        if (finish && ret != LBFGS_RUNNING_HOOK) {
            accepted = (ret == LBFGS_CONVERGENCE || ret == LBFGS_CANCELED || ret == LBFGS_STOP || ret == LBFGSERR_MAXIMUMITERATION || ret == LBFGSERR_MAXIMUMLINESEARCH) ? 1 : 0;
            if (accepted) { updateDualVars(); conv = judgeConvergence() ? 1 : 0; }
        }
        wg.pfor(n + MAX_PAST, [&](int t) { if (t < n) { gx[t] = x[t]; gg[t] = g[t]; gd[t] = d[t]; } else rs[8 + t - n] = pf[t - n]; });
        wg.pfor(1, [&](int) {
            rs[0] = io.step; rs[1] = io.fx; rs[2] = io.k; rs[3] = io.end; rs[4] = io.bound; rs[5] = ret; rs[6] = accepted; rs[7] = conv;
            st.f = io.fx; st.last_lbfgs_ret = ret; st.lbfgs_iters = io.k;
        });
        storeTrajectory(st);
    }

    UPH_HD void microbench(TrajState& st, int reps) {
        const double* gx0 = bd.x + td.off_x;
        rho = wg.bcast(st.rho); scale_fx = wg.bcast(st.scale_fx);
        wg.pfor(n, [&](int t) { x[t] = gx0[t]; d[t] = 0.5; xp[t] = gx0[t]; gp[t] = 0.25; });
        long long a[9];
        long long sub[8] = {0, 0, 0, 0, 0, 0, 0, 0};
        sub_t = sub;
        double acc = 0.0, js[3], part[3], c1, c2;
        const int cnt = S < CH ? S : CH;
        a[0] = wg.clock();
        for (int r = 0; r < reps; r++) generate<false>(x, 0.0);
        a[1] = wg.clock();
        for (int r = 0; r < reps; r++) { expand(x, 1.0, js); acc += js[0]; }
        a[2] = wg.clock();
        for (int r = 0; r < reps; r++) evalConsts(evalStep());
        a[3] = wg.clock();
        for (int r = 0; r < reps; r++) { wg.template sum<3>(cnt, part, [&](int t, double* ac) { sampleEval<false>(t, t, ac); }); acc += part[0]; }
        a[4] = wg.clock();
        for (int r = 0; r < reps; r++) scatterChunk(0, cnt);
        a[5] = wg.clock();
        for (int r = 0; r < reps; r++) { adjoint(c1, c2); acc += c1 + c2; }
        a[6] = wg.clock();
        const int m = mem;
        for (int r = 0; r < reps; r++) {
            const int end = (r * 7) % m, bound = m;
            acc += absmax(g, n) + absmax(x, n);
            wg.sync();
            wg.pfor(1, [&](int) { pf[r % 3] = acc; });
            double* sc = hist + (size_t)end * hrow + 2;
            double* yc = sc + hnp;
            double r6[6] = {0, 0, 0, 0, 0, 0};
            wg.template sum<3>(n, r6, [&](int i, double* ac) {
                const double sv = x[i] - xp[i], yv = g[i] - gp[i];
                sc[i] = sv; yc[i] = yv;
                ac[0] += yv * sv; ac[1] += yv * yv; ac[2] += sv * sv;
                d[i] = -g[i];
            });
            acc += r6[0] + r6[3] + sqrt(dot(gp, gp, n));
            wg.sync();
            wg.pfor(1, [&](int) { hist[(size_t)end * hrow] = acc; });
            (void)bound;
        }
        a[7] = wg.clock();
        wg.pfor(1, [&](int) {
            for (int q = 0; q < 7; q++) st.cyc[q] = (a[q + 1] - a[q]) / reps;
            st.cyc[7] = a[7] - a[0];
            for (int q = 0; q < 8; q++) st.cyc[8 + q] = sub[q] / reps;
            st.f = acc;
        });
        sub_t = nullptr;
    }

    UPH_HD void evalOnly(TrajState& st, int repeat) {
        const double* gx0 = bd.x + td.off_x;
        rho = wg.bcast(st.rho); scale_fx = wg.bcast(st.scale_fx);
        wg.pfor(n, [&](int t) { x[t] = gx0[t]; });
        double f = 0.0;
        for (int r = 0; r < repeat; r++) f = eval<false>(x, g);
        refreshResiduals();
        wg.pfor(n, [&](int t) { bd.gout[td.off_x + t] = g[t]; });
        storeTrajectory(st);
        wg.pfor(1, [&](int) { st.f = f; });
    }
    template <bool STORE_RES>
    UPH_HD void penaltyOnly(TrajState& st, int repeat) {
        rho = wg.bcast(st.rho); scale_fx = wg.bcast(st.scale_fx);
        Txy = wg.bcast(st.T_xy); Tyaw = wg.bcast(st.T_yaw);
        ec_iTyaw = wg.bcast(1.0 / Tyaw);
        const double* oc = bd.cxy + td.off_cxy;
        const double* oy = bd.cyaw + td.off_cyaw;
        const int nc = 12 * Nxy + 6 * Nyaw;
        wg.pfor(nc, [&](int t) { if (t < 12 * Nxy) cxy[t] = oc[t]; else cyaw[t - 12 * Nxy] = oy[t - 12 * Nxy]; });
        double sm[3] = {0.0, 0.0, 0.0};
        for (int r = 0; r < repeat; r++) {
            wg.pfor(nc + 2, [&](int t) { if (t < 12 * Nxy) Gxy[t] = 0.0; else if (t < nc) Gyaw[t - 12 * Nxy] = 0.0; else fillTimes(t - nc); });
            evalConsts(Txy / K);
            wg.template accBegin<3>();
            for (int s0 = 0; s0 < S; s0 += CHS) {
                const int cnt = S - s0 < CHS ? S - s0 : CHS;
                wg.template accChunk<3>(cnt, [&](int t, double* acc) { sampleEval<STORE_RES ? 2 : 0, SR>(s0 + t, t, acc); });
                scatterChunk(s0, cnt);
            }
            wg.template accEnd<3>(sm);
        }
        double* ogx = bd.pen_gxy + td.off_cxy;
        double* ogy = bd.pen_gyaw + td.off_cyaw;
        wg.pfor(nc + 1, [&](int t) {
            if (t < 12 * Nxy) ogx[t] = Gxy[t];
            else if (t < nc) ogy[t - 12 * Nxy] = Gyaw[t - 12 * Nxy];
            else { double* o = bd.pen_out + (size_t)bidx * 3; o[0] = sm[0]; o[1] = sm[1]; o[2] = sm[2]; }
        });
    }
    UPH_HD void scalingOnly(TrajState& st) {
        const double* gx0 = bd.x + td.off_x;
        rho = wg.bcast(st.rho); scale_fx = 1.0;
        wg.pfor(n, [&](int t) { x[t] = gx0[t]; });
        initScaling(x);
        storeTrajectory(st);
    }

    UPH_HD void report(const TrajState& st) {
        const double* oc = bd.cxy + td.off_cxy;
        const double* oy = bd.cyaw + td.off_cyaw;
        wg.pfor(12 * Nxy + 6 * Nyaw, [&](int t) { if (t < 12 * Nxy) cxy[t] = oc[t]; else cyaw[t - 12 * Nxy] = oy[t - 12 * Nxy]; });
        const double Tx = st.T_xy, Ty = st.T_yaw;
        double durx = 0.0, dury = 0.0;
        for (int i = 0; i < Nxy; i++) durx += Tx;
        for (int i = 0; i < Nyaw; i++) dury += Ty;
        const double total = dmin(durx, dury);
        int cnt = 0;
        {
            double cnt_d[1];
            wg.template sum<1>(1, cnt_d, [&](int, double* acc) { double t = 0.0; int q = 0; for (; q < 200000 && t < total; q++) t += 0.01; acc[0] += (double)q; });
            cnt = (int)cnt_d[0];
        }
        const double gravity = grid.gravity;
        const GridDev fgrid = framedGrid();
        double tcur = 0.0;
        int qcur = 0;
        auto sampleAt = [&](int q, double out[7]) {
            if (q < qcur) { tcur = 0.0; qcur = 0; }
            for (; qcur < q; qcur++) tcur += 0.01;
            TrajSample smp;
            trajectorySample<true>(cxy, cyaw, Nxy, Nyaw, Tx, Ty, tcur, fgrid, gravity, smp, out);
        };
        double o[7], e1[1], ma[7], mb[3], dum[1];
        wg.template sumMax<1, 7>(cnt, e1, ma, [&](int q, double* acc, double* mx) {
            double r[7];
            sampleAt(q, r);
            acc[0] += r[6];
            mx[0] = dmax(mx[0], r[0]); mx[1] = dmax(mx[1], -r[0]); mx[2] = dmax(mx[2], r[1]); mx[3] = dmax(mx[3], -r[1]);
            mx[4] = dmax(mx[4], r[2]); mx[5] = dmax(mx[5], -r[2]); mx[6] = dmax(mx[6], r[3]);
        });
        wg.template sumMax<1, 3>(cnt, dum, mb, [&](int q, double* acc, double* mx) {
            double r[7];
            sampleAt(q, r);
            acc[0] += 0.0;
            mx[0] = dmax(mx[0], -r[3]); mx[1] = dmax(mx[1], r[4] + 1.0); mx[2] = dmax(mx[2], r[5]);
        });
        o[0] = ma[0] >= ma[1] ? ma[0] : -ma[1];
        o[1] = ma[2] >= ma[3] ? ma[2] : -ma[3];
        o[2] = ma[4] >= ma[5] ? ma[4] : -ma[5];
        o[3] = ma[6] >= mb[0] ? ma[6] : -mb[0];
        o[4] = mb[1] - 1.0;
        o[5] = mb[2];
        o[6] = e1[0];
        wg.pfor(7, [&](int t) { bd.report[(size_t)bidx * 7 + t] = o[t]; });
    }
};

}
```

### uneven_planner_amd/csrc/unevenhip.hip

```cpp
#include <hip/hip_runtime.h>

#include <type_traits>

#include <algorithm>
#include <cmath>
#include <cstdio>
#include <cstdlib>
#include <cstring>
#include <map>
#include <numeric>
#include <string>
#include <thread>
#include <vector>

#include "../../include/uneven_hip.h"
#include "minco_op_host.hpp"
#include "resample_walk.hpp"
#include "solver_program.hpp"
#include "uph_ctx.hpp"
#include "wave_dev.hpp"

using namespace uph;

#ifndef UPH_THOMAS_KPL
// ... 5 lines not shown
#ifndef UPH_TWOLOOP_PF
#define UPH_TWOLOOP_PF 5
#endif

template <int NT>
struct DevWG {
    static constexpr int NW = NT / 64;
    static constexpr int MAXM = 8;
    static constexpr int SCRATCH = 2 * NW * MAXM;
    double* red;
    int tid, lane, wave, par;
#ifdef UPH_TL_PROF
    long long tl[6] = {0, 0, 0, 0, 0, 0};
#endif
#ifdef UPH_BAR_PROF
    long long barw[4] = {0, 0, 0, 0};
    __device__ __forceinline__ void bar(int cls) {
        const long long t0 = __builtin_readcyclecounter();
        __syncthreads();
        barw[cls] += __builtin_readcyclecounter() - t0;
    }
    __device__ __forceinline__ void dumpBar(long long* dst) {
        if (lane == 0 && wave == 0) for (int q = 0; q < 4; q++) dst[q] = barw[q];
        if (lane == 0 && wave == 1) { dst[4] = barw[0] + barw[3]; dst[5] = barw[1] + barw[2]; }
    }
#else
    __device__ __forceinline__ void bar(int) { __syncthreads(); }
#endif
    __device__ DevWG(double* scratch) : red(scratch), tid(threadIdx.x), lane(threadIdx.x & 63), wave(uni((int)(threadIdx.x >> 6))), par(0) {}
    __device__ __forceinline__ int ftid() const { int v = tid; asm volatile("" : "+v"(v)); return v; }
    __device__ __forceinline__ int flane() const { int v = lane; asm volatile("" : "+v"(v)); return v; }

    template <class F>
    __device__ __forceinline__ void pfor(int n, F f) {
        for (int i = ftid(); i < n; i += NT) f(i);
        bar(0);
    }
    template <class F>
    __device__ __forceinline__ void pforRev(int n, F f) {
        for (int i = (NW - 1 - wave) * 64 + flane(); i < n; i += NT) f(i);
        bar(3);
    }
#ifndef UPH_MFMA_SCATTER
#define UPH_MFMA_SCATTER 1
#endif
    static constexpr bool MFMA_SCATTER = UPH_MFMA_SCATTER != 0;
    __device__ __forceinline__ void scatterXY17(const double* rec, const double* wtab, double* Gxy, int i0_, int P_, int s0_, int cnt_) {
        typedef double d4_t __attribute__((ext_vector_type(4)));
        constexpr int K1 = 17, NQ = 3 * K1, CHP = NT + 1;
        const int P = uni(P_), s0 = uni(s0_), cnt = uni(cnt_), i0 = uni(i0_);
        const int ntile = (2 * P + 15) >> 4;
        const int ln = flane();
        const int c = ln & 15, kk = (ln >> 4) & 3;
        const double c1 = (double)c, c2 = (double)(c * (c - 1));
        for (int t = wave; t < ntile; t += NW) {
            const int col = 16 * t + c, pi = col >> 1, dd = col & 1;
            const int pbase = (i0 + pi) * K1 - s0;
            const int jlo = pbase < 0 ? -pbase : 0;
            int jhi = cnt - pbase < K1 ? cnt - pbase : K1;
            if (pi >= P) jhi = 0;
            const double* rb = rec + dd * CHP + pbase;
            d4_t acc0 = {0.0, 0.0, 0.0, 0.0}, acc1 = {0.0, 0.0, 0.0, 0.0};
#pragma unroll
            for (int st = 0; st < (NQ + 3) / 4; st++) {
                const int q = 4 * st + kk;
                const int f = (q >= K1 ? 1 : 0) + (q >= 2 * K1 ? 1 : 0) + (q >= 3 * K1 ? 1 : 0);
                const int j = q - K1 * f;
                const double wv = wtab[6 * j + c - f];
                const double rv = rb[2 * f * CHP + j];
                const double cf = f == 0 ? 1.0 : (f == 1 ? c1 : c2);
                const double a = (c < 6 && c >= f && q < NQ) ? cf * wv : 0.0;
                const double b = (j >= jlo && j < jhi && q < NQ) ? rv : 0.0;
                if (st & 1) acc1 = __builtin_amdgcn_mfma_f64_16x16x4f64(a, b, acc1, 0, 0, 0);
                else acc0 = __builtin_amdgcn_mfma_f64_16x16x4f64(a, b, acc0, 0, 0, 0);
            }
            if (pi < P) {
                double* gp = Gxy + 12 * (i0 + pi) + dd;
                gp[2 * kk] += acc0[0] + acc1[0];
                if (kk < 2) gp[2 * (4 + kk)] += acc0[1] + acc1[1];
            }
        }
    }
    __device__ __forceinline__ void sync() { bar(0); }
    __device__ __forceinline__ int size() const { return NT; }
#ifndef UPH_CYC
#define UPH_CYC 0
#endif
#if UPH_CYC
    __device__ __forceinline__ long long clock() { return (long long)__builtin_readcyclecounter(); }
    __device__ __forceinline__ long long realtime() { return (long long)__builtin_amdgcn_s_memrealtime(); }
#else
    __device__ __forceinline__ long long clock() { return 0; }
    __device__ __forceinline__ long long realtime() { return 0; }
#endif
    template <class F>
    __device__ __forceinline__ void one(F f) { if (tid == 0) f(); }

    template <int M, class F>
    __device__ __forceinline__ void sum(int n, double* out, F f) {
        double acc[M];
#pragma unroll
        for (int m = 0; m < M; m++) acc[m] = 0.0;
        for (int i = ftid(); i < n; i += NT) f(i, acc);
#pragma unroll
        for (int m = 0; m < M; m++) acc[m] = waveSum(acc[m]);
        double* r = red + par * (NW * MAXM);
        par ^= 1;
        if (lane == 0) {
#pragma unroll
            for (int m = 0; m < M; m++) r[wave * MAXM + m] = acc[m];
        }
        bar(0);
#pragma unroll
        for (int m = 0; m < M; m++) {
            double t = r[m];
#pragma unroll
            for (int w = 1; w < NW; w++) t += r[w * MAXM + m];
            out[m] = uni(t);
        }
    }
    double pacc[MAXM];
    template <int M>
    __device__ __forceinline__ void accBegin() {
#pragma unroll
        for (int m = 0; m < M; m++) pacc[m] = 0.0;
    }
    template <int M, class F>
    __device__ __forceinline__ void accChunk(int n, F f) {
        for (int i = ftid(); i < n; i += NT) f(i, pacc);
        bar(0);
    }
    template <int M>
    __device__ __forceinline__ void accEnd(double* out) {
        double acc[M];
#pragma unroll
        for (int m = 0; m < M; m++) acc[m] = waveSum(pacc[m]);
        double* r = red + par * (NW * MAXM);
        par ^= 1;
        if (lane == 0) {
#pragma unroll
            for (int m = 0; m < M; m++) r[wave * MAXM + m] = acc[m];
        }
        bar(0);
#pragma unroll
        for (int m = 0; m < M; m++) {
            double t = r[m];
#pragma unroll
            for (int w = 1; w < NW; w++) t += r[w * MAXM + m];
            out[m] = uni(t);
        }
    }
    template <int MS, int MM, class F>
    __device__ __forceinline__ void sumMax(int n, double* outS, double* outM, F f) {
        static_assert(MS + MM <= MAXM, "reduction scratch too small");
        double acc[MS], mx[MM];
#pragma unroll
        for (int m = 0; m < MS; m++) acc[m] = 0.0;
#pragma unroll
        for (int m = 0; m < MM; m++) mx[m] = 0.0;
        for (int i = ftid(); i < n; i += NT) f(i, acc, mx);
#pragma unroll
        for (int m = 0; m < MS; m++) acc[m] = waveSum(acc[m]);
#pragma unroll
        for (int m = 0; m < MM; m++) mx[m] = waveMax(mx[m]);
        double* r = red + par * (NW * MAXM);
        par ^= 1;
// ... 222 lines not shown
        }
        double z0 = 0.0, z1 = 0.0;
        for (int s = 0; s < steps; s++) {
            const double p0 = shl1(z0), p1 = shl1(z1);
            z0 = fma(F[0][1], p1, fma(F[0][0], p0, c[0][0]));
            z1 = fma(F[0][3], p1, fma(F[0][2], p0, c[0][1]));
        }
        {
            const double p0 = shl1(z0), p1 = shl1(z1);
#pragma unroll
            for (int k = 0; k < KPL; k++) {
                if (j0 + k <= len) {
                    pk[k * ks] = fma(F[k][1], p1, fma(F[k][0], p0, c[k][0]));
                    pk[k * ks + cs] = fma(F[k][3], p1, fma(F[k][2], p0, c[k][1]));
                }
            }
        }
    }
    template <bool ADJ>
    __device__ __forceinline__ void thomasT(const double* tab, double* bw, int lenW, double* bx, int lenX) {
        UPH_MARK("thomas");
        __builtin_amdgcn_s_setprio(3);
        const bool packed = uni(lenW) <= 32 * UPH_THOMAS_KPL - 1 && uni(lenX) <= 16 * UPH_THOMAS_KPL - 1;
        if (packed) {
            if (wave == 0) thomasWave<2, ADJ, UPH_THOMAS_KPL>(tab, bw, lenW, bx, lenX);
        } else if (NW >= 2) {
            if (wave == 0) thomasWave<0, ADJ, UPH_THOMAS_KPL>(tab, bw, lenW, bx, lenX);
            else if (wave == 1) thomasWave<1, ADJ, UPH_THOMAS_KPL>(tab, bw, lenW, bx, lenX);
        } else {
            thomasWave<0, ADJ, UPH_THOMAS_KPL>(tab, bw, lenW, bx, lenX);
            thomasWave<1, ADJ, UPH_THOMAS_KPL>(tab, bw, lenW, bx, lenX);
        }
        __builtin_amdgcn_s_setprio(0);
        bar(2);
    }
    template <class F>
    __device__ __forceinline__ void aside(int lenW, int lenX, int n, F f) {
        const bool packed = uni(lenW) <= 32 * UPH_THOMAS_KPL - 1 && uni(lenX) <= 16 * UPH_THOMAS_KPL - 1;
        const int aw = NW >= 2 && packed ? 1 : (NW >= 3 ? 2 : 0);
        if (wave == aw) {
            const int l = flane();
            if (l < n) f(l);
        }
    }
    __device__ __forceinline__ void thomas(const double* tab, bool adj, double* bw, int lenW, double* bx, int lenX) {
        if (adj) thomasT<true>(tab, bw, lenW, bx, lenX);
        else thomasT<false>(tab, bw, lenW, bx, lenX);
    }
    __device__ __forceinline__ void twoLoop(double* d, const double* g, int n, const double* __restrict__ hist, double* dg_out, double* al_lds, int m, int end, int bound, double scale) {
        if (wave == 0) {
            __builtin_amdgcn_s_setprio(3);
            constexpr int PF = UPH_TWOLOOP_PF;
            const int nq = uni((n + 63) >> 6);
            if (nq == 1) twoLoopT<1, PF>(d, g, dg_out, al_lds, n, hist, m, end, bound, scale);
            else if (nq == 2) twoLoopT<2, PF>(d, g, dg_out, al_lds, n, hist, m, end, bound, scale);
            else if (nq == 3) twoLoopT<3, PF>(d, g, dg_out, al_lds, n, hist, m, end, bound, scale);
            else if (nq == 4) twoLoopT<4, PF>(d, g, dg_out, al_lds, n, hist, m, end, bound, scale);
            else if (nq == 5) twoLoopT<5, 2>(d, g, dg_out, al_lds, n, hist, m, end, bound, scale);
            else if (nq == 6) twoLoopT<6, 2>(d, g, dg_out, al_lds, n, hist, m, end, bound, scale);
            else if (nq == 7) twoLoopT<7, 2>(d, g, dg_out, al_lds, n, hist, m, end, bound, scale);
            else twoLoopT<8, 2>(d, g, dg_out, al_lds, n, hist, m, end, bound, scale);
            __builtin_amdgcn_s_setprio(0);
        }
        bar(1);
    }
    template <class F>
    __device__ __forceinline__ double maxv(int n, F f) {
        double a = 0.0;
        for (int i = ftid(); i < n; i += NT) { const double v = f(i); a = v > a ? v : a; }
        a = waveMax(a);
        double* r = red + par * (NW * MAXM);
        par ^= 1;
        if (lane == 0) r[wave * MAXM] = a;
        bar(0);
        double t = r[0];
#pragma unroll
        for (int w = 1; w < NW; w++) t = r[w * MAXM] > t ? r[w * MAXM] : t;
        return uni(t);
    }
};

template <int NT, class F>
__device__ __forceinline__ void asideKnotSolve(DevWG<NT>& wg, int lenW, int lenX, int n, F f) { wg.aside(lenW, lenX, n, f); }

template <int NT, int WPS, int MODE, bool F32S = false>
__global__ __launch_bounds__(NT, WPS) void uph_solver_kernel(GridDev grid, OptParams P, BatchDev bd, int repeat) {
    extern __shared__ double lds[];
    const int w = blockIdx.x;
    if (w >= bd.B) return;
    const int b = bd.order ? bd.order[w] : w;
    DevWG<NT> wg(lds);
    typedef typename std::conditional<F32S, f32r, double>::type SR;
    Solver<DevWG<NT>, SR> sol(wg, grid, P, bd, b, lds + DevWG<NT>::SCRATCH);
    TrajState& st = bd.state[b];
    if (MODE == 0) sol.evalOnly(st, repeat);
    else if (MODE == 1) sol.prepare(st);
    else if (MODE == 2) sol.optimize(st, repeat);
    else if (MODE == 7) sol.resumeHook(st, repeat >> 1, repeat & 1);
    else if (MODE == 8) { if (repeat & 1) sol.template penaltyOnly<true>(st, repeat >> 1); else sol.template penaltyOnly<false>(st, repeat >> 1); }
    else if (MODE == 3) sol.report(st);
    else if (MODE == 5) sol.microbench(st, repeat);
    else sol.scalingOnly(st);
}

__global__ void uph_fill_kernel(double* __restrict__ p, size_t n, double v) {
    for (size_t i = (size_t)blockIdx.x * blockDim.x + threadIdx.x; i < n; i += (size_t)gridDim.x * blockDim.x) p[i] = v;
}

__global__ void uph_terrain_kernel(GridDev grid, const double* __restrict__ pos, int n, double* __restrict__ values, double* __restrict__ grads) {
    const int i = blockIdx.x * blockDim.x + threadIdx.x;
    if (i >= n) return;
    const double yaw = pos[3 * i + 2];
    double v[7], g[7][3];
    terrainAllWithGrad(grid, pos[3 * i], pos[3 * i + 1], yaw, cos(yaw), sin(yaw), v, g);
    for (int k = 0; k < 7; k++) {
        values[7 * i + k] = v[k];
        for (int q = 0; q < 3; q++) grads[21 * i + 3 * k + q] = g[k][q];
    }
}

constexpr int PLAN_SX = UPH_MAX_PIECE_XY - 1, PLAN_SY = UPH_MAX_PIECE_YAW - 1;
struct PlanHead {
    int32_t n_inner_xy, n_inner_yaw;
    int32_t short_path, pad;
    double p_init[2], p_end[2];
    double yaw_init, yaw_end;
    double total_time;
    double lo[2], hi[2];
    double turn, kink;
};
struct PlanPath {
    const double* p;
    __host__ __device__ double operator()(int64_t k, int j) const { return p[3 * k + j]; }
};
struct PlanSink {
    double *oxy, *oyw;
    int nxy, nyw;
    double nlo[2], nhi[2], prev, turn, kink;
    __device__ void xy(double x, double y) {
        if (nxy < PLAN_SX) { oxy[2 * nxy] = x; oxy[2 * nxy + 1] = y; }
        nxy++;
        nlo[0] = x < nlo[0] ? x : nlo[0]; nlo[1] = y < nlo[1] ? y : nlo[1];
        nhi[0] = nhi[0] < x ? x : nhi[0]; nhi[1] = nhi[1] < y ? y : nhi[1];
    }
    __device__ void yaw(double v) {
        if (nyw < PLAN_SY) oyw[nyw] = v;
        nyw++;
        const double d = fabs(v - prev);
        turn += d; kink = kink < d ? d : kink; prev = v;
    }
    __device__ void unwrapped(int64_t, double) {}
};
__global__ __launch_bounds__(64) void uph_plan_resample_kernel(uph_manager_params mp, const double* __restrict__ paths, int path_cap, const int* __restrict__ n_path,
                                                               const int* __restrict__ status, int nq, const int* __restrict__ goal_of, double* __restrict__ st_xy,
                                                               double* __restrict__ st_yaw, PlanHead* __restrict__ heads) {
#pragma clang fp contract(off)
    const int q = blockIdx.x * blockDim.x + threadIdx.x;
    if (q >= nq) return;
    const int m = n_path[q];
    if (status[q] != UPH_KINO_OK || m > path_cap) return;
    const int g = goal_of ? goal_of[q] : q;
    PlanHead h = PlanHead{};
    if (m < 2) { h.short_path = 1; heads[g] = h; return; }
    const double* p = paths + (size_t)q * path_cap * 3;
    const WalkSetup ws = walkSetup(mp);
    PlanSink s;
    s.oxy = st_xy + (size_t)g * PLAN_SX * 2; s.oyw = st_yaw + (size_t)g * PLAN_SY;
    s.nxy = s.nyw = 0;
    s.nlo[0] = s.nlo[1] = __builtin_huge_val(); s.nhi[0] = s.nhi[1] = -__builtin_huge_val();
    s.prev = p[2]; s.turn = 0.0; s.kink = 0.0;
    const WalkEnd e = resampleWalk(ws, PlanPath{p}, (int64_t)m, s);
    h.n_inner_xy = s.nxy; h.n_inner_yaw = s.nyw;
    h.p_init[0] = p[0]; h.p_init[1] = p[1]; h.p_end[0] = p[3 * (m - 1)]; h.p_end[1] = p[3 * (m - 1) + 1];
    h.yaw_init = e.yaw_first; h.yaw_end = e.yaw_last;
    h.total_time = walkTotalTime(ws, mp, e.len);
    for (int d = 0; d < 2; d++) {
        const double a = h.p_init[d] < h.p_end[d] ? h.p_init[d] : h.p_end[d], b = h.p_init[d] < h.p_end[d] ? h.p_end[d] : h.p_init[d];
        h.lo[d] = s.nlo[d] < a ? s.nlo[d] : a;
        h.hi[d] = b < s.nhi[d] ? s.nhi[d] : b;
    }
    const double d = fabs(e.yaw_last - s.prev);
    h.turn = s.turn + d; h.kink = s.kink < d ? d : s.kink;
    heads[g] = h;
}
struct PlanScatter {
// ... 14 lines not shown
            v = (r.src >= 0 ? st_xy[(size_t)r.src * PLAN_SX * 2 + j] : (j == 0 ? 0.3 : 0.0)) - r.shift[j & 1];
        } else {
            const int j = i - 1 - 2 * r.nxy;
            v = r.src >= 0 ? st_yaw[(size_t)r.src * PLAN_SY + j] : 0.0;
        }
        x[r.off_x + i] = v;
        x0[r.off_x + i] = v;
    }
}

struct RefineStage {
    int32_t q, nxy, nyw, pad;
    int64_t row_xy, row_yaw;
    double p_end[2], yaw_end;
    double total_time;
};
__global__ __launch_bounds__(64) void uph_refine_stage_kernel(const RefineStage* __restrict__ rec, int n, const double* __restrict__ states,
                                                              double* __restrict__ st_xy, double* __restrict__ st_yaw, PlanHead* __restrict__ heads) {
    const int j = blockIdx.x * blockDim.x + threadIdx.x;
    if (j >= n) return;
    const RefineStage r = rec[j];
    const double* z = states + (size_t)r.q * TRAJ_STATE_COLS;
    PlanHead h = PlanHead{};
    h.n_inner_xy = r.nxy; h.n_inner_yaw = r.nyw;
    h.p_init[0] = z[0]; h.p_init[1] = z[1]; h.p_end[0] = r.p_end[0]; h.p_end[1] = r.p_end[1];
    h.yaw_init = z[9]; h.yaw_end = r.yaw_end;
    h.total_time = r.total_time;
    for (int d = 0; d < 2; d++) {
        h.lo[d] = h.p_end[d] < h.p_init[d] ? h.p_end[d] : h.p_init[d];
        h.hi[d] = h.p_init[d] < h.p_end[d] ? h.p_end[d] : h.p_init[d];
    }
    double* oxy = st_xy + (size_t)r.q * PLAN_SX * 2;
    for (int k = 0; k < r.nxy; k++) {
        const double* w = states + (size_t)(r.row_xy + k) * TRAJ_STATE_COLS;
        for (int d = 0; d < 2; d++) {
            oxy[2 * k + d] = w[d];
            h.lo[d] = w[d] < h.lo[d] ? w[d] : h.lo[d];
            h.hi[d] = h.hi[d] < w[d] ? w[d] : h.hi[d];
        }
    }
    double* oyw = st_yaw + (size_t)r.q * PLAN_SY;
    double prev = h.yaw_init;
    for (int k = 0; k <= r.nyw; k++) {
        const double cur = k < r.nyw ? states[(size_t)(r.row_yaw + k) * TRAJ_STATE_COLS + 9] : h.yaw_end;
        if (k < r.nyw) oyw[k] = cur;
        const double dy = fabs(cur - prev);
        h.turn += dy; h.kink = h.kink < dy ? dy : h.kink; prev = cur;
    }
    heads[r.q] = h;
}

#ifdef UPH_ONE_KERNEL
#ifndef UPH_OK_F32
#define UPH_OK_F32 false
#endif
template __global__ void uph_solver_kernel<UPH_OK_NT, UPH_OK_WPS, UPH_OK_MODE, UPH_OK_F32>(GridDev, OptParams, BatchDev, int);
#else
namespace uph {
thread_local std::string g_last_error;
void setError(const std::string& s) { g_last_error = s; }
}

static BatchDev makeBatchDev(uph_ctx* c) {
    BatchDev bd;
    std::memset(&bd, 0, sizeof(bd));
    bd.B = c->B;
    bd.desc = c->d_desc.as<TrajDesc>();
    bd.state = c->d_state.as<TrajState>();
    bd.ops = c->d_ops.as<MincoOp>();
    bd.x = c->d_x.as<double>(); bd.x0 = c->d_x0.as<double>(); bd.gout = c->d_gout.as<double>();
    bd.dual = c->d_dual.as<double>(); bd.res = c->d_res.as<double>(); bd.scl = c->d_scl.as<double>();
    bd.cxy = c->d_cxy.as<double>(); bd.cyaw = c->d_cyaw.as<double>();
    bd.hist = c->d_hist.as<double>();
    bd.report = c->d_report.as<double>();
    bd.pen_gxy = c->d_pen_gxy.as<double>(); bd.pen_gyaw = c->d_pen_gyaw.as<double>(); bd.pen_out = c->d_pen_out.as<double>();
    bd.trace = c->trace_cap_up > 0 ? c->d_trace.as<double>() : nullptr;
    bd.trace_cap = c->trace_cap_up;
    bd.order = c->d_order.as<int>();
    bd.thomas = c->d_thomas.as<double>();
    bd.grid_per_traj = c->frames.empty() ? 0 : 1;
    bd.grid_mem = c->d_gridmem.as<GridDev>();
    bd.params_mem = c->d_parammem.as<OptParams>();
    bd.rs_d = c->d_rsd.as<double>(); bd.rs = c->d_rs.as<double>();
    return bd;
}

static int ensureOp(uph_ctx* c, int N) {
    auto it = c->op_index.find(N);
    if (it != c->op_index.end()) return it->second;
    std::vector<double> Mt, Mr;
    buildMincoOp(N, Mt, Mr);
    double *dt = nullptr, *dr = nullptr;
    const size_t bytes = Mt.size() * sizeof(double);
    if (hipMalloc((void**)&dt, bytes) != hipSuccess || hipMalloc((void**)&dr, bytes) != hipSuccess) { setError("hipMalloc(MincoOp) failed"); return -1; }
    if (hipMemcpy(dt, Mt.data(), bytes, hipMemcpyHostToDevice) != hipSuccess || hipMemcpy(dr, Mr.data(), bytes, hipMemcpyHostToDevice) != hipSuccess) {
        setError("hipMemcpy(MincoOp) failed");
        return -1;
    }
    c->op_allocs.push_back(dt); c->op_allocs.push_back(dr);
    MincoOp op; op.N = N; op.Wt = dt; op.Wr = dr;
    const int idx = (int)c->ops_host.size();
    c->ops_host.push_back(op);
    c->op_index[N] = idx;
    c->ops_dirty = true;
    return idx;
}

int syncGridMem(uph_ctx* c, GridDev& grid) {
    grid = uphMapGrid(c->map);
    c->grid_host = grid;
    if (c->frames.empty()) {
        c->framed_valid = false;
        if (c->d_gridmem.ensure(sizeof(GridDev))) return UPH_ERR_HIP;
        HIPCHK(hipMemcpyAsync(c->d_gridmem.p, &c->grid_host, sizeof(GridDev), hipMemcpyHostToDevice, c->stream));
    } else {
        const GridDev& fg = c->frames_grid;
        if (grid.nx != fg.nx || grid.ny != fg.ny || grid.nyaw != fg.nyaw || grid.xy_res != fg.xy_res || grid.origin[0] != fg.origin[0] || grid.origin[1] != fg.origin[1] ||
            grid.lo[0] != fg.lo[0] || grid.hi[0] != fg.hi[0] || grid.lo[1] != fg.lo[1] || grid.hi[1] != fg.hi[1]) {
            setError("the map's geometry changed since this batch was uploaded (its per-trajectory local frames were formed from the old one): upload the batch again");
            return UPH_ERR_INVALID;
        }
        if (!c->framed_valid || std::memcmp(&c->framed_from, &grid, sizeof(GridDev)) != 0) {
            if (c->d_gridmem.ensure(sizeof(GridDev) * c->frames.size())) return UPH_ERR_HIP;
            c->grid_host_framed.assign(c->frames.size(), grid);
            for (size_t b = 0; b < c->frames.size(); b++) applyFrame(c->grid_host_framed[b], c->frames[b]);
            HIPCHK(hipMemcpyAsync(c->d_gridmem.p, c->grid_host_framed.data(), sizeof(GridDev) * c->frames.size(), hipMemcpyHostToDevice, c->stream));
            c->framed_from = grid;
            c->framed_valid = true;
        }
    }
    return UPH_OK;
}

int refreshStates(uph_ctx* c) {
    HIPCHK(hipMemcpy(c->state_host.data(), c->d_state.p, sizeof(TrajState) * c->B, hipMemcpyDeviceToHost));
    return UPH_OK;
}

static int launchSolver(uph_ctx* c, int mode, int repeat, bool async = false, hipEvent_t evb = nullptr, hipEvent_t eve = nullptr) {
    if (!async && c->pending) { setError("an asynchronous solve is in flight on this context: call uph_batch_wait first"); return UPH_ERR_INVALID; }
    if (!evb) { evb = c->ev0; eve = c->ev1; }
    HIPCHK(hipSetDevice(uphMapDevice(c->map)));
    GridDev grid;
    const int rg = syncGridMem(c, grid);
    if (rg != UPH_OK) return rg;
    if (c->d_parammem.ensure(sizeof(OptParams))) return UPH_ERR_HIP;
    HIPCHK(hipMemcpyAsync(c->d_parammem.p, &c->P, sizeof(OptParams), hipMemcpyHostToDevice, c->stream));
    BatchDev bd = makeBatchDev(c);
#define UPH_LAUNCH(NTL, WPS, MODE)                                                                                                     \
    do {                                                                                                                             \
        const size_t ldsmax = 160 * 1024;    \
        HIPCHK(hipFuncSetAttribute((const void*)uph_solver_kernel<NTL, WPS, MODE>, hipFuncAttributeMaxDynamicSharedMemorySize, (int)ldsmax)); \
        HIPCHK(hipEventRecord(evb, c->stream));                                                                                   \
        BatchDev bm = bd;                                                                                                            \
        bm.B = c->n_main;                                                                                                            \
        if (c->n_main < c->B) {            \
            BatchDev bb = bd;              \
            bb.B = c->B - c->n_main;                                                                                                 \
            bb.order = bd.order + c->n_main;                                                                                         \
            HIPCHK(hipStreamWaitEvent(c->stream2, evb, 0));                                                                       \
            hipLaunchKernelGGL((uph_solver_kernel<NTL, WPS, MODE>), dim3(bb.B), dim3(NTL), c->lds_big, c->stream2, grid, c->P, bb, repeat); \
            HIPCHK(hipEventRecord(c->ev2, c->stream2));                                                                              \
        }                                                                                                                            \
        hipLaunchKernelGGL((uph_solver_kernel<NTL, WPS, MODE>), dim3(c->n_main), dim3(NTL), c->lds_bytes, c->stream, grid, c->P, bm, repeat); \
        if (c->n_main < c->B) HIPCHK(hipStreamWaitEvent(c->stream, c->ev2, 0));                                                      \
    } while (0)
#define UPH_LAUNCH_MODE(NTL, WPS)                                                                                                      \
    do {                                                                                                                             \
        if (mode == 0) UPH_LAUNCH(NTL, WPS, 0);                                                                                      \
        else if (mode == 1) UPH_LAUNCH(NTL, WPS, 1);                                                                                 \
        else if (mode == 2) UPH_LAUNCH(NTL, WPS, 2);                                                                                 \
        else if (mode == 3) UPH_LAUNCH(NTL, WPS, 3);                                                                                 \
        else if (mode == 5) UPH_LAUNCH(NTL, WPS, 5);                                                                                 \
        else UPH_LAUNCH(NTL, WPS, 4);                                                                                                \
    } while (0)
#define UPH_LAUNCH32(NTL, WPS, MODE)                                                                                                   \
    do {                                                                                                                             \
        const size_t ldsmax = 160 * 1024;    \
        HIPCHK(hipFuncSetAttribute((const void*)uph_solver_kernel<NTL, WPS, MODE, true>, hipFuncAttributeMaxDynamicSharedMemorySize, (int)ldsmax)); \
        HIPCHK(hipEventRecord(evb, c->stream));                                                                                   \
        BatchDev bm = bd;                                                                                                            \
        bm.B = c->n_main;                                                                                                            \
        if (c->n_main < c->B) {                                                                                                      \
            BatchDev bb = bd;                                                                                                        \
            bb.B = c->B - c->n_main;                                                                                                 \
            bb.order = bd.order + c->n_main;                                                                                         \
            HIPCHK(hipStreamWaitEvent(c->stream2, evb, 0));                                                                       \
            hipLaunchKernelGGL((uph_solver_kernel<NTL, WPS, MODE, true>), dim3(bb.B), dim3(NTL), c->lds_big, c->stream2, grid, c->P, bb, repeat); \
            HIPCHK(hipEventRecord(c->ev2, c->stream2));                                                                              \
        }                                                                                                                            \
        hipLaunchKernelGGL((uph_solver_kernel<NTL, WPS, MODE, true>), dim3(c->n_main), dim3(NTL), c->lds_bytes, c->stream, grid, c->P, bm, repeat); \
        if (c->n_main < c->B) HIPCHK(hipStreamWaitEvent(c->stream, c->ev2, 0));                                                      \
    } while (0)
    if (c->sample_f32 && (mode == 0 || mode == 2) && (c->lanes == 128 || c->lanes == 256 || c->lanes == 512)) {
        if (c->lanes == 128) { if (mode == 0) UPH_LAUNCH32(128, 2, 0); else UPH_LAUNCH32(128, 2, 2); }
        else if (c->lanes == 512) { if (mode == 0) UPH_LAUNCH32(512, 1, 0); else UPH_LAUNCH32(512, 1, 2); }
        else if (mode == 0) UPH_LAUNCH32(256, 1, 0);
        else if (c->wps == 2 && c->lds_bytes <= 80 * 1024) UPH_LAUNCH32(256, 2, 2);
        else UPH_LAUNCH32(256, 1, 2);
    }
    else if (mode == 7) {
        if (c->lanes == 128) UPH_LAUNCH(128, 2, 7);
        else if (c->lanes == 256) UPH_LAUNCH(256, 1, 7);
        else { setError("the L-BFGS resume hook is built for 128 and 256 lanes"); return UPH_ERR_INVALID; }
    }
    else if (mode == 8) {
        if (c->lanes == 128) UPH_LAUNCH(128, 2, 8);
        else if (c->lanes == 256) UPH_LAUNCH(256, 1, 8);
        else if (c->lanes == 512) UPH_LAUNCH(512, 1, 8);
        else UPH_LAUNCH(64, 1, 8);
    }
    else if (c->lanes == 64 && c->wps_forced == 2) UPH_LAUNCH_MODE(64, 2);
    else if (c->lanes == 64) UPH_LAUNCH_MODE(64, 1);
    else if (c->lanes == 128 && mode == 1) UPH_LAUNCH(128, 1, 1);
    else if (c->lanes == 128) UPH_LAUNCH_MODE(128, UPH_WPS128);
    else if (c->lanes == 512) UPH_LAUNCH_MODE(512, 1);
    else if (c->wps == 2 && mode == 2 && c->lds_bytes <= 80 * 1024) UPH_LAUNCH(256, 2, 2);
    else if (c->wps == 2 && mode == 5 && c->lds_bytes <= 80 * 1024) UPH_LAUNCH(256, 2, 5);
    else UPH_LAUNCH_MODE(256, 1);
#undef UPH_LAUNCH_MODE
#undef UPH_LAUNCH32
#undef UPH_LAUNCH
    HIPCHK(hipGetLastError());
    if (mode == 0 || mode == 2 || mode == 4 || mode == 7) c->traj_resident = true;
    HIPCHK(hipEventRecord(eve, c->stream));
    if (async) return UPH_OK;
    HIPCHK(hipStreamSynchronize(c->stream));
    float ms = 0.f;
    HIPCHK(hipEventElapsedTime(&ms, evb, eve));
    c->last_ms = ms;
    return UPH_OK;
}

static int uploadPackedX(uph_ctx* c, const double* x_packed) {
    if (c->frames.empty()) { HIPCHK(hipMemcpy(c->d_x.p, x_packed, 8 * c->sum_n, hipMemcpyHostToDevice)); return UPH_OK; }
    std::vector<double> xl(x_packed, x_packed + c->sum_n);
    for (int b = 0; b < c->B; b++) {
        const TrajDesc& t = c->desc[b];
        for (int i = 0; i < 2 * (t.Nxy - 1); i++) xl[t.off_x + 1 + i] -= c->frames[b].shift[i & 1];
    }
    HIPCHK(hipMemcpy(c->d_x.p, xl.data(), 8 * c->sum_n, hipMemcpyHostToDevice));
    return UPH_OK;
}

extern "C" {

const char* uph_last_error(void) { return g_last_error.c_str(); }
const char* uph_version(void) { return "unevenhip 0.1 (gfx950)"; }
int uph_device_count(void) {
    int n = 0;
    if (hipGetDeviceCount(&n) != hipSuccess) return 0;
    return n;
}

int uph_ctx_create(uph_map* m, const uph_opt_params* p, uph_ctx** out) {
    if (!m || !p || !out) { setError("uph_ctx_create: null argument"); return UPH_ERR_INVALID; }
    if (p->mem_size < 1 || p->mem_size > UPH_MAX_MEM || p->past < 0 || p->past > UPH_MAX_PAST || p->int_K < 1 || p->int_K > 64) {
        setError("uph_ctx_create: mem_size/past/int_K outside compiled limits");
        return UPH_ERR_LIMIT;
    }
    HIPCHK(hipSetDevice(uphMapDevice(m)));
    uph_ctx* c = new uph_ctx();
    c->map = m;
    c->device = uphMapDevice(m);
    OptParams& P = c->P;
    P.rho_T = p->rho_T; P.rho_ter = p->rho_ter; P.max_vel = p->max_vel; P.max_acc_lon = p->max_acc_lon; P.max_acc_lat = p->max_acc_lat;
    P.max_kap = p->max_kap; P.min_cxi = p->min_cxi; P.max_sig = p->max_sig; P.use_scaling = p->use_scaling;
    P.beta = p->beta; P.gamma = p->gamma; P.epsilon_con = p->epsilon_con; P.max_iter = p->max_iter;
    P.g_epsilon = p->g_epsilon; P.min_step = p->min_step; P.delta = p->delta;
    P.inner_max_iter = (int)p->inner_max_iter; P.mem_size = p->mem_size; P.past = p->past; P.int_K = p->int_K;
    P.max_linesearch = 64; P.max_step = 1.0e20; P.f_dec_coeff = 1.0e-4; P.s_curv_coeff = 0.9; P.cautious_factor = 1.0e-6; P.machine_prec = 1.0e-16;
    P.no_trial_abandon = 0; P.pad_ = 0;
    finishParams(P);
    c->rho = p->rho;
    {
        std::vector<double> tab;
        buildThomasTable(tab);
        if (c->d_thomas.ensure(tab.size() * sizeof(double))) { delete c; return UPH_ERR_HIP; }
        if (hipMemcpy(c->d_thomas.p, tab.data(), tab.size() * sizeof(double), hipMemcpyHostToDevice) != hipSuccess) { setError("hipMemcpy(thomas table) failed"); c->d_thomas.release(); delete c; return UPH_ERR_HIP; }
    }
    HIPCHK(hipStreamCreateWithFlags(&c->stream, hipStreamNonBlocking));
    {
        int prio_lo = 0, prio_hi = 0;
        hipDeviceGetStreamPriorityRange(&prio_lo, &prio_hi);
        HIPCHK(hipStreamCreateWithPriority(&c->stream2, hipStreamNonBlocking, prio_hi));
    }
    HIPCHK(hipEventCreate(&c->ev2));
    HIPCHK(hipEventCreate(&c->evp0)); HIPCHK(hipEventCreate(&c->evp1));
    HIPCHK(hipEventCreate(&c->ev0));
    HIPCHK(hipEventCreate(&c->ev1));
    *out = c;
    return UPH_OK;
}

void uph_ctx_destroy(uph_ctx* c) {
    if (!c) return;
    hipSetDevice(c->device);
    for (void* p : c->op_allocs) hipFree(p);
    DevBuf* bufs[] = {&c->d_ops, &c->d_desc, &c->d_state, &c->d_x, &c->d_gout, &c->d_dual, &c->d_res, &c->d_scl, &c->d_cxy, &c->d_cyaw,
                      &c->d_hist, &c->d_report, &c->d_order, &c->d_trace, &c->d_x0, &c->d_thomas, &c->d_rsd, &c->d_rs, &c->d_gridmem, &c->d_parammem,
                      &c->d_pen_gxy, &c->d_pen_gyaw, &c->d_pen_out, &c->d_roll_tt, &c->d_roll_traj, &c->d_roll_stage,
                      &c->d_plan_head, &c->d_plan_xy, &c->d_plan_yaw, &c->d_plan_goal, &c->d_plan_rec, &c->d_sw_q, &c->d_sw_out, &c->d_refine_rec, &c->d_win_q,
                      &c->d_win_out, &c->d_delay};
    for (DevBuf* b : bufs) b->release();
    HostBuf* hbufs[] = {&c->h_x, &c->h_cxy, &c->h_cyaw, &c->h_dual, &c->h_res, &c->h_scl};
    for (HostBuf* b : hbufs) b->release();
    if (c->ev0) hipEventDestroy(c->ev0);
    if (c->ev1) hipEventDestroy(c->ev1);
    if (c->stream) hipStreamDestroy(c->stream);
    if (c->stream2) hipStreamDestroy(c->stream2);
    if (c->ev2) hipEventDestroy(c->ev2);
    if (c->evp0) hipEventDestroy(c->evp0);
    if (c->evp1) hipEventDestroy(c->evp1);
    delete c;
}

int uph_ctx_set_lanes(uph_ctx* c, int32_t lanes) {
    if (!c || (lanes != 0 && lanes != 64 && lanes != 128 && lanes != 256 && lanes != 512)) return UPH_ERR_INVALID;
    c->lanes_forced = lanes;
    return UPH_OK;
}
int uph_ctx_set_xcd_locality(uph_ctx* c, int32_t group) { if (!c || group < 0) return UPH_ERR_INVALID; c->xcd_group = group; return UPH_OK; }
int uph_ctx_set_wps(uph_ctx* c, int32_t wps) { if (!c || wps < 0 || wps > 2) return UPH_ERR_INVALID; c->wps_forced = wps; return UPH_OK; }
int uph_ctx_set_sample_precision(uph_ctx* c, int32_t bits) {
    if (!c || (bits != 32 && bits != 64)) { setError("uph_ctx_set_sample_precision: 32 or 64"); return UPH_ERR_INVALID; }
    c->sample_f32 = bits == 32;
    return UPH_OK;
}
int uph_ctx_set_rho(uph_ctx* c, double rho) { if (!c) return UPH_ERR_INVALID; c->rho = rho; return UPH_OK; }
int uph_ctx_set_trial_abandon(uph_ctx* c, int32_t on) { if (!c || (on != 0 && on != 1)) return UPH_ERR_INVALID; c->P.no_trial_abandon = on ? 0 : 1; return UPH_OK; }
int uph_ctx_get_rho(uph_ctx* c, double* rho) { if (!c || !rho) return UPH_ERR_INVALID; *rho = c->rho; return UPH_OK; }

int uph_ctx_set_trace(uph_ctx* c, int32_t cap) { if (!c || cap < 0) return UPH_ERR_INVALID; c->trace_cap = cap; return UPH_OK; }
int uph_ctx_get_trace(uph_ctx* c, double* out ) {
    if (c && c->pending) { setError("an asynchronous solve is in flight on this context: call uph_batch_wait first"); return UPH_ERR_INVALID; }
    if (!c || !out || c->trace_cap_up <= 0 || c->B <= 0) return UPH_ERR_INVALID;
    HIPCHK(hipSetDevice(uphMapDevice(c->map)));
    HIPCHK(hipMemcpy(out, c->d_trace.p, sizeof(double) * (size_t)c->B * c->trace_cap_up, hipMemcpyDeviceToHost));
    return UPH_OK;
}

static void yawTurnKink(const uph_problem& pr, double& turn, double& kink) {
    double prev = pr.init_yaw[0];
    turn = 0.0; kink = 0.0;
    for (int i = 0; i <= pr.n_inner_yaw; i++) {
        const double cur = i < pr.n_inner_yaw ? pr.inner_yaw[i] : pr.end_yaw[0];
        const double dy = std::fabs(cur - prev);
        turn += dy; kink = std::max(kink, dy); prev = cur;
    }
}
static double predictedCostOf(int32_t n_inner_xy, int32_t n_inner_yaw, double turn, double kink) {
    const double n = 2.0 * n_inner_xy + n_inner_yaw + 1.0;
    return std::pow(n, 0.831) * std::exp(0.129 * turn) * std::pow(1.0 + kink, 0.408);
}
static double predictedCost(const uph_problem& pr) {
    double turn, kink;
    yawTurnKink(pr, turn, kink);
    return predictedCostOf(pr.n_inner_xy, pr.n_inner_yaw, turn, kink);
}

static ProblemHead headOf(const uph_problem& q) {
    ProblemHead h;
    h.n_inner_xy = q.n_inner_xy; h.n_inner_yaw = q.n_inner_yaw;
    for (int k = 0; k < 6; k++) { h.init_xy[k] = q.init_xy[k]; h.end_xy[k] = q.end_xy[k]; }
    for (int k = 0; k < 3; k++) { h.init_yaw[k] = q.init_yaw[k]; h.end_yaw[k] = q.end_yaw[k]; }
    h.total_time = q.total_time;
    if (q.n_inner_xy < 0 || q.n_inner_yaw < 0 || (q.n_inner_xy > 0 && !q.inner_xy) || (q.n_inner_yaw > 0 && !q.inner_yaw)) {
        h.refused = UPH_ERR_INVALID; h.why = "uph_batch_upload: negative way-point count or missing way-point array";
        return h;
    }
    for (int d = 0; d < 2; d++) { h.lo[d] = std::min(q.init_xy[d], q.end_xy[d]); h.hi[d] = std::max(q.init_xy[d], q.end_xy[d]); }
    for (int i = 0; i < q.n_inner_xy; i++)
        for (int d = 0; d < 2; d++) { h.lo[d] = std::min(h.lo[d], q.inner_xy[2 * i + d]); h.hi[d] = std::max(h.hi[d], q.inner_xy[2 * i + d]); }
    yawTurnKink(q, h.turn, h.kink);
    return h;
}
static const double ph_inner_xy[2] = {0.3, 0.0}, ph_inner_yaw[1] = {0.0};
static uph_problem placeholderProblem() {
    uph_problem placeholder;
    std::memset(&placeholder, 0, sizeof(placeholder));
    placeholder.n_inner_xy = 1; placeholder.n_inner_yaw = 1; placeholder.inner_xy = ph_inner_xy; placeholder.inner_yaw = ph_inner_yaw;
    placeholder.init_xy[2] = 0.05; placeholder.end_xy[0] = 0.6; placeholder.end_xy[2] = 0.05; placeholder.total_time = 1.44;
    return placeholder;
}

static int admitBatch(uph_ctx* c, int32_t B, const ProblemHead* heads, std::vector<const ProblemHead*>& pp) {
    const int K1 = c->P.int_K + 1, mem = c->P.mem_size;
    c->B = 0;
    c->traj_resident = false;
    c->planned = false;
    c->origin.clear(); c->all_rejected = false;
    int first_rj = 0;
    c->desc.assign(B, TrajDesc());
    int64_t on = 0, os = 0, ocx = 0, ocy = 0, oh = 0;
    size_t lds_d = 0;
    c->lanes = c->lanes_forced ? c->lanes_forced : (B >= 2304 ? 128 : (B <= 256 ? 512 : 256));
    c->wps = c->wps_forced ? c->wps_forced : ((B >= 512) ? 2 : 1);
    c->fp_bytes.assign(B, 0);
    static const ProblemHead placeholder = headOf(placeholderProblem());
    pp.assign(B, nullptr);
    c->rejected.assign(B, 0); c->n_rejected = 0;
    c->end_pose.assign((size_t)3 * B, 0.0);
    c->end_bnd.assign((size_t)9 * B, 0.0);
    const GridDev tg = uphMapGrid(c->map);
    const bool tiled = tg.nx_hold < tg.nx;
    const double tile_lo = tg.origin[0] + tg.x_off * tg.xy_res, tile_hi = tg.origin[0] + (tg.x_off + tg.nx_hold) * tg.xy_res;
    std::string why;
    for (int b = 0; b < B; b++) {
        const ProblemHead& q = heads[b];
        int rj = 0;
        const char* msg = nullptr;
        if (q.refused) { rj = q.refused; msg = q.why; }
        else if (q.n_inner_xy + 1 > UPH_MAX_PIECE_XY || q.n_inner_yaw + 1 > UPH_MAX_PIECE_YAW) { rj = UPH_ERR_LIMIT; msg = "uph_batch_upload: piece count exceeds UPH_MAX_PIECE_*"; }
// ... 17 lines not shown
        for (int b = 0; b < B; b++) {
            const ProblemHead& q = *pp[b];
            TrajFrame& f = c->frames[b];
            const int nn[2] = {tg.nx, tg.ny};
            for (int d = 0; d < 2; d++) {
                long long ci = std::llround((0.5 * (q.lo[d] + q.hi[d]) - tg.origin[d]) * tg.xy_inv);
                ci = ci < 0 ? 0 : (ci > nn[d] ? nn[d] : ci);
                f.ioff[d] = (int)ci;
                f.shift[d] = tg.origin[d] + (double)ci * tg.xy_res;
                f.fo[d] = 0.0;
                f.lo[d] = tg.lo[d] - f.shift[d];
                f.hi[d] = tg.hi[d] - f.shift[d];
            }
        }
    }
    for (int b = 0; b < B; b++) {
        const ProblemHead& pr = *pp[b];
        const int Nxy = pr.n_inner_xy + 1, Nyaw = pr.n_inner_yaw + 1;
        TrajDesc& t = c->desc[b];
        std::memset(&t, 0, sizeof(t));
        t.Nxy = Nxy; t.Nyaw = Nyaw; t.n = 2 * pr.n_inner_xy + pr.n_inner_yaw + 1; t.S = Nxy * K1;
        t.op_xy = ensureOp(c, Nxy);
        t.op_yaw = ensureOp(c, Nyaw);
        if (t.op_xy < 0 || t.op_yaw < 0) return UPH_ERR_HIP;
        t.off_x = on; t.off_s = os; t.off_cxy = ocx; t.off_cyaw = ocy; t.off_hist = oh;
        for (int k = 0; k < 6; k++) { t.init_xy[k] = pr.init_xy[k]; t.end_xy[k] = pr.end_xy[k]; }
        for (int k = 0; k < 3; k++) { t.init_yaw[k] = pr.init_yaw[k]; t.end_yaw[k] = pr.end_yaw[k]; }
        if (!c->frames.empty()) for (int d = 0; d < 2; d++) { t.init_xy[d] -= c->frames[b].shift[d]; t.end_xy[d] -= c->frames[b].shift[d]; }
        on += t.n; os += t.S; ocx += 12 * Nxy; ocy += 6 * Nyaw; oh += (int64_t)mem * histRowDoubles(t.n);
        c->fp_bytes[b] = (Solver<DevWG<64>>::ldsDoubles(Nxy, Nyaw, t.n, c->lanes, mem, c->P.int_K) + 2 * (c->lanes / 64) * DevWG<64>::MAXM) * sizeof(double);
        lds_d = std::max(lds_d, Solver<DevWG<64>>::ldsDoubles(Nxy, Nyaw, t.n, c->lanes, mem, c->P.int_K));
    }
    c->sum_n = on; c->sum_S = os; c->sum_cxy = ocx; c->sum_cyaw = ocy; c->sum_hist = oh;
    c->lds_bytes = (lds_d + 2 * (c->lanes / 64) * DevWG<64>::MAXM) * sizeof(double);
    if (c->lds_bytes > 160 * 1024) { setError("uph_batch_upload: trajectory does not fit the 160 KiB LDS"); return UPH_ERR_LIMIT; }
    if (c->ops_dirty) {
        if (c->d_ops.ensure(sizeof(MincoOp) * c->ops_host.size())) return UPH_ERR_HIP;
        HIPCHK(hipMemcpy(c->d_ops.p, c->ops_host.data(), sizeof(MincoOp) * c->ops_host.size(), hipMemcpyHostToDevice));
        c->ops_dirty = false;
    }
    if (c->d_desc.ensure(sizeof(TrajDesc) * B) || c->d_state.ensure(sizeof(TrajState) * B) || c->d_x.ensure(8 * on) || c->d_x0.ensure(8 * on) || c->d_gout.ensure(8 * on) ||
        c->d_dual.ensure(8 * 7 * os) || c->d_res.ensure(8 * 7 * os) || c->d_scl.ensure(8 * 7 * os) || c->d_cxy.ensure(8 * ocx) || c->d_cyaw.ensure(8 * ocy) ||
        c->d_hist.ensure(8 * oh) || c->d_report.ensure(8 * 7 * B) || c->d_order.ensure(4 * B) ||
        c->d_trace.ensure(8 * (size_t)std::max(1, c->trace_cap) * B))
        return UPH_ERR_HIP;
    {
        std::vector<double> cost(B);
        for (int b = 0; b < B; b++) cost[b] = predictedCostOf(pp[b]->n_inner_xy, pp[b]->n_inner_yaw, pp[b]->turn, pp[b]->kink);
        c->order.resize(B);
        std::iota(c->order.begin(), c->order.end(), 0);
        std::stable_sort(c->order.begin(), c->order.end(), [&](int a, int b2) { return cost[a] > cost[b2]; });
        if (c->xcd_group >= 16) {
            const GridDev gg = uphMapGrid(c->map);
            auto octant = [&](int b) {
                const ProblemHead& q = *pp[b];
                const double mx = 0.5 * (q.init_xy[0] + q.end_xy[0]), my = 0.5 * (q.init_xy[1] + q.end_xy[1]);
                const int ix = mx < 0.5 * (gg.minb[0] + gg.maxb[0]) ? 0 : 1;
                int iy = (int)((my - gg.minb[1]) / (gg.maxb[1] - gg.minb[1]) * 4.0);
                iy = iy < 0 ? 0 : (iy > 3 ? 3 : iy);
                return ix * 4 + iy;
            };
            const int G = c->xcd_group & ~7;
            for (int g0 = 0; g0 + G <= B; g0 += G) {
                std::vector<int> bins[8], spill, placed((size_t)G, -1);
                for (int k = 0; k < G; k++) bins[octant(c->order[g0 + k])].push_back(c->order[g0 + k]);
                for (int r = 0; r < 8; r++) {
                    int at = r;
                    for (int b : bins[r]) { if (at < G) { placed[at] = b; at += 8; } else spill.push_back(b); }
                }
                size_t sp = 0;
                for (int k = 0; k < G; k++) if (placed[k] < 0) placed[k] = spill[sp++];
                for (int k = 0; k < G; k++) c->order[g0 + k] = placed[k];
            }
        }
        const size_t limit = c->lanes == 128 ? 40960 : (c->lanes == 256 ? 81920 : (c->lanes == 512 ? 163840 : 32768));
        c->n_main = B; c->lds_big = 0;
        size_t mmain = 0, mbig = 0;
        int nbig = 0;
        for (int b = 0; b < B; b++) { if (c->fp_bytes[b] > limit) { nbig++; mbig = std::max(mbig, c->fp_bytes[b]); } else mmain = std::max(mmain, c->fp_bytes[b]); }
        if (nbig > 0 && nbig < B) {
            std::stable_partition(c->order.begin(), c->order.end(), [&](int a) { return c->fp_bytes[a] <= limit; });
            c->n_main = B - nbig; c->lds_bytes = mmain; c->lds_big = mbig;
        }
    }
    c->state_host.assign(B, TrajState());
    for (int b = 0; b < B; b++) { std::memset(&c->state_host[b], 0, sizeof(TrajState)); c->state_host[b].rho = c->rho; c->state_host[b].scale_fx = 1.0; }
    return UPH_OK;
}

static int commitBatch(uph_ctx* c, int32_t B) {
    HIPCHK(hipMemcpyAsync(c->d_desc.p, c->desc.data(), sizeof(TrajDesc) * B, hipMemcpyHostToDevice, c->stream));
    HIPCHK(hipMemcpyAsync(c->d_order.p, c->order.data(), 4 * B, hipMemcpyHostToDevice, c->stream));
    HIPCHK(hipMemcpyAsync(c->d_state.p, c->state_host.data(), sizeof(TrajState) * B, hipMemcpyHostToDevice, c->stream));
    HIPCHK(hipMemsetAsync(c->d_hist.p, 0, 8 * c->sum_hist, c->stream));
    HIPCHK(hipMemsetAsync(c->d_dual.p, 0, 8 * 7 * c->sum_S, c->stream));
    HIPCHK(hipMemsetAsync(c->d_res.p, 0, 8 * 7 * c->sum_S, c->stream));
    hipLaunchKernelGGL(uph_fill_kernel, dim3(1024), dim3(256), 0, c->stream, c->d_scl.as<double>(), (size_t)7 * c->sum_S, 1.0);
    HIPCHK(hipGetLastError());
    if (c->trace_cap > 0) HIPCHK(hipMemsetAsync(c->d_trace.p, 0, 8 * (size_t)c->trace_cap * B, c->stream));
    HIPCHK(hipStreamSynchronize(c->stream));
    c->trace_cap_up = c->trace_cap;
    c->B = B;
    return UPH_OK;
}

int uph_batch_upload(uph_ctx* c, int32_t B, const uph_problem* probs) {
    if (!c || B <= 0 || !probs) { setError("uph_batch_upload: bad arguments"); return UPH_ERR_INVALID; }
    if (c->pending) { setError("uph_batch_upload: an asynchronous solve is in flight (uph_batch_wait first)"); return UPH_ERR_INVALID; }
    HIPCHK(hipSetDevice(uphMapDevice(c->map)));
    std::vector<ProblemHead> heads(B);
    for (int b = 0; b < B; b++) heads[b] = headOf(probs[b]);
    std::vector<const ProblemHead*> pp;
    const int r = admitBatch(c, B, heads.data(), pp);
    if (r != UPH_OK) return r;
    static const uph_problem placeholder = placeholderProblem();
    std::vector<double> x0(c->sum_n);
    for (int b = 0; b < B; b++) {
        const uph_problem& pr = c->rejected[b] ? placeholder : probs[b];
        double* x = x0.data() + c->desc[b].off_x;
        x[0] = logC2(pr.total_time);
        for (int i = 0; i < 2 * pr.n_inner_xy; i++) x[1 + i] = pr.inner_xy[i] - (c->frames.empty() ? 0.0 : c->frames[b].shift[i & 1]);
        for (int i = 0; i < pr.n_inner_yaw; i++) x[1 + 2 * pr.n_inner_xy + i] = pr.inner_yaw[i];
    }
    HIPCHK(hipMemcpy(c->d_x.p, x0.data(), 8 * c->sum_n, hipMemcpyHostToDevice));
    HIPCHK(hipMemcpy(c->d_x0.p, x0.data(), 8 * c->sum_n, hipMemcpyHostToDevice));
    return commitBatch(c, B);
}

static bool managerParamsOk(const uph_manager_params* mp) {
    return mp->test_mode ? mp->test_max_vel > 0.0 : (mp->piece_len > 0.0 && mp->yaw_piece_times > 0.0 && mp->mean_vel > 0.0);
}

static int uploadStaged(uph_ctx* c, const std::vector<int>& found, const std::vector<ProblemHead>& heads, int32_t* traj_of);
static int planUpload(uph_kino* k, uph_ctx* c, const uph_manager_params* mp, int32_t B, const double* starts, const double* goals, int32_t path_cap,
                      const double* init_state, double* init_out, const char* who, int32_t* status, int32_t* traj_of, int32_t* n_inner_xy, int32_t* n_inner_yaw) {
    c->B = 0;
    c->traj_resident = false; c->planned = false; c->origin.clear(); c->plan_probs.clear();
    const int cap = path_cap > 0 ? path_cap : UPH_PLAN_PATH_CAP;
    UphKinoOut io;
    int r = uphKinoSearch(k, B, starts, goals, cap, 0, 0, io);
    if (r != UPH_OK) return r;
    HIPCHK(hipSetDevice(uphMapDevice(c->map)));
    std::vector<int> st((size_t)B), np((size_t)B);
    HIPCHK(hipMemcpy(st.data(), io.status, 4 * (size_t)B, hipMemcpyDeviceToHost));
    HIPCHK(hipMemcpy(np.data(), io.n_path, 4 * (size_t)B, hipMemcpyDeviceToHost));
    if (c->d_plan_head.ensure(sizeof(PlanHead) * (size_t)B) || c->d_plan_xy.ensure(sizeof(double) * 2 * PLAN_SX * (size_t)B) ||
        c->d_plan_yaw.ensure(sizeof(double) * PLAN_SY * (size_t)B))
        return UPH_ERR_HIP;
    const uph_manager_params mpv = *mp;
    hipLaunchKernelGGL(uph_plan_resample_kernel, dim3((B + 63) / 64), dim3(64), 0, c->stream, mpv, io.paths, cap, io.n_path, io.status, (int)B, (const int*)nullptr,
                       c->d_plan_xy.as<double>(), c->d_plan_yaw.as<double>(), c->d_plan_head.as<PlanHead>());
    HIPCHK(hipGetLastError());
    HIPCHK(hipStreamSynchronize(c->stream));
    std::vector<int> longer;
    int need = 0;
    for (int b = 0; b < B; b++) if (st[b] == UPH_KINO_OK && np[b] > cap) { longer.push_back(b); need = std::max(need, np[b]); }
    if (!longer.empty()) {
        const int L = (int)longer.size();
        std::vector<double> s2((size_t)3 * L), g2((size_t)3 * L);
        for (int j = 0; j < L; j++) for (int q = 0; q < 3; q++) { s2[(size_t)3 * j + q] = starts[(size_t)3 * longer[j] + q]; g2[(size_t)3 * j + q] = goals[(size_t)3 * longer[j] + q]; }
        UphKinoOut io2;
        r = uphKinoSearch(k, L, s2.data(), g2.data(), need, 0, 0, io2);
        if (r != UPH_OK) return r;
        HIPCHK(hipSetDevice(uphMapDevice(c->map)));
        std::vector<int> st2((size_t)L), np2((size_t)L);
        HIPCHK(hipMemcpy(st2.data(), io2.status, 4 * (size_t)L, hipMemcpyDeviceToHost));
// ... 158 lines not shown
        for (int k = 1; k <= s.nxy; k++) sq.push_back(trajQuery(src, b, tc + k * hx));
        s.row_yaw = (int64_t)sq.size();
        for (int k = 1; k <= s.nyw; k++) sq.push_back(trajQuery(src, b, tc + k * hy));
        const double* e = src->end_bnd.data() + (size_t)9 * b;
        s.p_end[0] = e[0]; s.p_end[1] = e[1]; s.yaw_end = e[6]; s.total_time = R;
        rec.push_back(s);
        found.push_back(q);
        ends.insert(ends.end(), e, e + 9);
    }
    r = launchTrajStates(src, sq);
    if (r != UPH_OK) { hipStreamSynchronize(src->stream); return r; }
    std::vector<double> zs((size_t)TRAJ_STATE_COLS * B);
    HIPCHK(hipMemcpyAsync(zs.data(), src->d_sw_out.p, sizeof(double) * TRAJ_STATE_COLS * (size_t)B, hipMemcpyDeviceToHost, src->stream));
    HIPCHK(hipStreamSynchronize(src->stream));
    dst->B = 0;
    dst->traj_resident = false; dst->planned = false; dst->origin.clear(); dst->plan_probs.clear();
    const int F = (int)found.size();
    std::vector<PlanHead> ph((size_t)B);
    if (F > 0) {
        if (dst->d_plan_head.ensure(sizeof(PlanHead) * (size_t)B) || dst->d_plan_xy.ensure(sizeof(double) * 2 * PLAN_SX * (size_t)B) ||
            dst->d_plan_yaw.ensure(sizeof(double) * PLAN_SY * (size_t)B) || dst->d_refine_rec.ensure(sizeof(RefineStage) * (size_t)F))
            return UPH_ERR_HIP;
        HIPCHK(hipMemcpyAsync(dst->d_refine_rec.p, rec.data(), sizeof(RefineStage) * (size_t)F, hipMemcpyHostToDevice, src->stream));
        hipLaunchKernelGGL(uph_refine_stage_kernel, dim3((F + 63) / 64), dim3(64), 0, src->stream, dst->d_refine_rec.as<RefineStage>(), F, src->d_sw_out.as<double>(),
                           dst->d_plan_xy.as<double>(), dst->d_plan_yaw.as<double>(), dst->d_plan_head.as<PlanHead>());
        const hipError_t e = hipGetLastError();
        if (e != hipSuccess) { hipStreamSynchronize(src->stream); setError(std::string("uph_refine_upload: ") + hipGetErrorString(e)); return UPH_ERR_HIP; }
        HIPCHK(hipMemcpyAsync(ph.data(), dst->d_plan_head.p, sizeof(PlanHead) * (size_t)B, hipMemcpyDeviceToHost, src->stream));
        HIPCHK(hipStreamSynchronize(src->stream));
    }
    if (switch_states) std::memcpy(switch_states, zs.data(), sizeof(double) * TRAJ_STATE_COLS * (size_t)B);
    for (int32_t q = 0; q < B; q++) {
        status[q] = rem[(size_t)q] > 0.0 ? UPH_KINO_OK : UPH_REFINE_AT_END; traj_of[q] = -1;
        n_inner_xy[q] = nxy[(size_t)q]; n_inner_yaw[q] = nyw[(size_t)q];
    }
    if (F == 0) { setError("uph_refine_upload: no query left to refine (every switch time at or past its trajectory's end)"); return UPH_ERR_INVALID; }
    std::vector<ProblemHead> heads((size_t)F);
    for (int j = 0; j < F; j++) {
        const int q = found[(size_t)j];
        const PlanHead& g = ph[(size_t)q];
        const double* z = zs.data() + (size_t)TRAJ_STATE_COLS * q;
        const double* e = ends.data() + (size_t)9 * j;
        ProblemHead& h = heads[(size_t)j];
        h.n_inner_xy = nxy[(size_t)q]; h.n_inner_yaw = nyw[(size_t)q];
        for (int k = 0; k < 6; k++) { h.init_xy[k] = z[k]; h.end_xy[k] = e[k]; }
        h.init_yaw[0] = z[9]; h.init_yaw[1] = z[7]; h.init_yaw[2] = z[8];
        for (int k = 0; k < 3; k++) h.end_yaw[k] = e[6 + k];
        h.total_time = rem[(size_t)q];
        for (int d = 0; d < 2; d++) { h.lo[d] = g.lo[d]; h.hi[d] = g.hi[d]; }
        h.turn = g.turn; h.kink = g.kink;
    }
    return uploadStaged(dst, found, heads, traj_of);
}

int uph_plan_staged(uph_ctx* c, int32_t cap_xy, int32_t cap_yaw, double* init_xy, double* end_xy, double* init_yaw, double* end_yaw, double* inner_xy, double* inner_yaw,
                    int32_t* n_inner_xy, int32_t* n_inner_yaw, double* total_time) {
    if (!c || cap_xy < 0 || cap_yaw < 0 || !init_xy || !end_xy || !init_yaw || !end_yaw || !inner_xy || !inner_yaw || !n_inner_xy || !n_inner_yaw || !total_time) {
        setError("uph_plan_staged: bad arguments"); return UPH_ERR_INVALID;
    }
    if (c->B <= 0 || !c->planned) { setError("uph_plan_staged: the resident batch did not come from uph_plan_upload"); return UPH_ERR_INVALID; }
    if (c->pending) { setError("uph_plan_staged: an asynchronous solve is in flight (uph_batch_wait first)"); return UPH_ERR_INVALID; }
    HIPCHK(hipSetDevice(uphMapDevice(c->map)));
    int status = UPH_OK;
    for (int j = 0; j < c->B; j++) {
        const ProblemHead& h = c->plan_probs[(size_t)j];
        const int g = c->origin[(size_t)j];
        for (int q = 0; q < 6; q++) { init_xy[(size_t)6 * j + q] = h.init_xy[q]; end_xy[(size_t)6 * j + q] = h.end_xy[q]; }
        for (int q = 0; q < 3; q++) { init_yaw[(size_t)3 * j + q] = h.init_yaw[q]; end_yaw[(size_t)3 * j + q] = h.end_yaw[q]; }
        total_time[j] = h.total_time;
        n_inner_xy[j] = h.n_inner_xy; n_inner_yaw[j] = h.n_inner_yaw;
        const int nx = std::min(std::min(h.n_inner_xy, PLAN_SX), cap_xy), ny = std::min(std::min(h.n_inner_yaw, PLAN_SY), cap_yaw);
        if (h.n_inner_xy > cap_xy || h.n_inner_yaw > cap_yaw || h.n_inner_xy > PLAN_SX || h.n_inner_yaw > PLAN_SY) status = UPH_ERR_LIMIT;
        if (nx > 0) HIPCHK(hipMemcpy(inner_xy + (size_t)2 * cap_xy * j, c->d_plan_xy.as<double>() + (size_t)2 * PLAN_SX * g, sizeof(double) * 2 * nx, hipMemcpyDeviceToHost));
        if (ny > 0) HIPCHK(hipMemcpy(inner_yaw + (size_t)cap_yaw * j, c->d_plan_yaw.as<double>() + (size_t)PLAN_SY * g, sizeof(double) * ny, hipMemcpyDeviceToHost));
    }
    if (status == UPH_ERR_LIMIT) setError("uph_plan_staged: a problem has more way-points than the caller's capacity or the staging's");
    return status;
}

int uph_batch_solve_async(uph_ctx* c) {
    if (!c || c->B <= 0) { setError("uph_batch_solve_async: no batch uploaded"); return UPH_ERR_INVALID; }
    if (c->pending) { setError("uph_batch_solve_async: the previous asynchronous solve has not been waited for"); return UPH_ERR_INVALID; }
    HIPCHK(hipSetDevice(uphMapDevice(c->map)));
    for (int b = 0; b < c->B; b++) { std::memset(&c->state_host[b], 0, sizeof(TrajState)); c->state_host[b].rho = c->rho; c->state_host[b].scale_fx = 1.0; }
    HIPCHK(hipMemcpyAsync(c->d_state.p, c->state_host.data(), sizeof(TrajState) * c->B, hipMemcpyHostToDevice, c->stream));
    int r = launchSolver(c, 1, 1, true, c->evp0, c->evp1);
    if (r != UPH_OK) { hipStreamSynchronize(c->stream); return r; }
    r = launchSolver(c, 2, 0, true, c->ev0, c->ev1);
    if (r != UPH_OK) { hipStreamSynchronize(c->stream); if (c->stream2) hipStreamSynchronize(c->stream2); return r; }
    c->pending = true;
    return UPH_OK;
}

int uph_batch_wait(uph_ctx* c) {
    if (!c || !c->pending) { setError("uph_batch_wait: no asynchronous solve in flight"); return UPH_ERR_INVALID; }
    HIPCHK(hipSetDevice(uphMapDevice(c->map)));
    c->pending = false;
    HIPCHK(hipStreamSynchronize(c->stream));
    float ms = 0.f;
    HIPCHK(hipEventElapsedTime(&ms, c->evp0, c->evp1));
    c->last_prepare_ms = ms;
    HIPCHK(hipEventElapsedTime(&ms, c->ev0, c->ev1));
    c->last_ms = ms;
    int r = refreshStates(c);
    if (r != UPH_OK) return r;
    c->last_evals = c->last_sample_evals = c->last_iters = c->last_hist_bytes = 0;
    for (int q = 0; q < 5; q++) c->last_abandon[q] = 0;
    for (int b = 0; b < c->B; b++) {
        if (c->rejected[b]) continue;
        const TrajState& s = c->state_host[b];
        c->last_evals += s.evals;
        c->last_sample_evals += (int64_t)(s.evals - s.ls_abandoned) * c->desc[b].S;
        c->last_abandon[0] += s.ls_rejected; c->last_abandon[1] += s.ls_guarded; c->last_abandon[2] += s.ls_abandoned;
        c->last_abandon[3] += s.chunks_skipped; c->last_abandon[4] += s.adjoints_skipped;
        c->last_iters += s.lbfgs_iters;
        c->last_hist_bytes += s.hist_reads * 8;
    }
    if (c->B == 1 && !c->rejected[0]) c->rho = c->state_host[0].rho;
    return UPH_OK;
}

int uph_batch_solve(uph_ctx* c) {
    const int r = uph_batch_solve_async(c);
    return r != UPH_OK ? r : uph_batch_wait(c);
}

int uph_batch_count(const uph_ctx* c) { return c ? c->B : UPH_ERR_INVALID; }
int uph_batch_origin(const uph_ctx* c, int32_t* idx) {
    if (!c || !idx || c->B <= 0) { setError("uph_batch_origin: no batch uploaded"); return UPH_ERR_INVALID; }
    for (int b = 0; b < c->B; b++) idx[b] = c->origin.empty() ? b : c->origin[b];
    return UPH_OK;
}

int uph_batch_stats(uph_ctx* c, double* kernel_ms, int64_t* evals, int64_t* sample_evals, int64_t* lbfgs_iters, int64_t* hist_bytes) {
    if (!c) return UPH_ERR_INVALID;
    if (kernel_ms) *kernel_ms = c->last_ms;
    if (evals) *evals = c->last_evals;
    if (sample_evals) *sample_evals = c->last_sample_evals;
    if (lbfgs_iters) *lbfgs_iters = c->last_iters;
    if (hist_bytes) *hist_bytes = c->last_hist_bytes;
    return UPH_OK;
}

int uph_batch_abandon_stats(uph_ctx* c, int64_t* out5) {
    if (!c || !out5) return UPH_ERR_INVALID;
    for (int q = 0; q < 5; q++) out5[q] = c->last_abandon[q];
    return UPH_OK;
}

int uph_batch_prepare_ms(uph_ctx* c, double* ms) { if (!c || !ms) return UPH_ERR_INVALID; *ms = c->last_prepare_ms; return UPH_OK; }

int uph_batch_cycles(uph_ctx* c, long long* out) {
    if (!c || c->B <= 0 || !out) return UPH_ERR_INVALID;
    for (int b = 0; b < c->B; b++) for (int q = 0; q < 16; q++) out[b * 16 + q] = c->state_host[b].cyc[q];
    return UPH_OK;
}

int uph_batch_download(uph_ctx* c, uph_result* results) {
    if (!c || c->B <= 0 || !results) { setError("uph_batch_download: bad arguments"); return UPH_ERR_INVALID; }
    if (c->pending) { setError("uph_batch_download: an asynchronous solve is in flight (uph_batch_wait first)"); return UPH_ERR_INVALID; }
    HIPCHK(hipSetDevice(uphMapDevice(c->map)));
    int r = refreshStates(c);
    if (r != UPH_OK) return r;
    const GridDev tg = uphMapGrid(c->map);
    const bool tiled = tg.nx_hold < tg.nx;
    const double tile_lo = tg.origin[0] + tg.x_off * tg.xy_res, tile_hi = tg.origin[0] + (tg.x_off + tg.nx_hold) * tg.xy_res;
    bool want_x = tiled, want_cxy = false, want_cyaw = false, want_dual = false, want_res = false, want_scl = false;
    for (int b = 0; b < c->B; b++) {
        const uph_result& o = results[b];
// ... 350 lines not shown
```

### uneven_planner_amd/csrc/uph_common.hpp

```cpp
#pragma once
#include <math.h>
#include <stdint.h>

#if defined(__HIPCC__)
#define UPH_HD __host__ __device__ __forceinline__
#define UPH_NOINLINE __host__ __device__ __attribute__((noinline))
#else
#define UPH_HD inline
#define UPH_NOINLINE __attribute__((noinline))
#endif

#if defined(__HIP_DEVICE_COMPILE__)
#define UPH_AS_GLOBAL(p) ((const __attribute__((address_space(1))) double*)(p))
#else
#define UPH_AS_GLOBAL(p) (p)
#endif

#if defined(UPH_ISA_MARKS) && defined(__HIP_DEVICE_COMPILE__)
#define UPH_MARK(name) asm volatile("; UPHMARK " name)
#else
#define UPH_MARK(name) do { } while (0)
#endif

namespace uph {

constexpr int MAX_PIECE_XY = 128;
constexpr int MAX_PIECE_YAW = 256;
constexpr int MAX_MEM = 256;
constexpr int MAX_PAST = 8;

constexpr double delta_sigl = 0.01;
constexpr double cur_scale = 10.0;
constexpr double sig_scale = 1000.0;
constexpr double scale_trick_jerk = 1000.0;

enum {
    LBFGS_CONVERGENCE = 0,
    LBFGS_STOP,
    LBFGS_CANCELED,
    LBFGSERR_UNKNOWNERROR = -1024,
    LBFGSERR_INVALID_N,
    LBFGSERR_INVALID_MEMSIZE,
    LBFGSERR_INVALID_GEPSILON,
    LBFGSERR_INVALID_TESTPERIOD,
    LBFGSERR_INVALID_DELTA,
    LBFGSERR_INVALID_MINSTEP,
    LBFGSERR_INVALID_MAXSTEP,
    LBFGSERR_INVALID_FDECCOEFF,
    LBFGSERR_INVALID_SCURVCOEFF,
    LBFGSERR_INVALID_MACHINEPREC,
    LBFGSERR_INVALID_MAXLINESEARCH,
    LBFGSERR_INVALID_FUNCVAL,
    LBFGSERR_MINIMUMSTEP,
    LBFGSERR_MAXIMUMSTEP,
    LBFGSERR_MAXIMUMLINESEARCH,
    LBFGSERR_MAXIMUMITERATION,
    LBFGSERR_WIDTHTOOSMALL,
    LBFGSERR_INVALIDPARAMETERS,
    LBFGSERR_INCREASEGRADIENT,
};

struct GridDev {
    int nx, ny, nyaw;
    int x_off, nx_hold;
    int ix_off = 0, iy_off = 0;
    double xy_res, yaw_res, xy_inv, yaw_inv;
    double origin[3], minb[3], maxb[3];
    double lo[3], hi[3];
    double half_xy, half_yaw;
    double gravity;
    const double* cells;
    const float* cells32;
};

struct OptParams {
    double rho_T, rho_ter, max_vel, max_acc_lon, max_acc_lat, max_kap, min_cxi, max_sig;
    int use_scaling;
    double beta, gamma, epsilon_con, max_iter;
    double g_epsilon, min_step, delta;
    int inner_max_iter, mem_size, past, int_K;
    int max_linesearch;
    double max_step, f_dec_coeff, s_curv_coeff, cautious_factor, machine_prec;
    double max_vel2, max_acc_lon2, max_acc_lat2, max_kap2;
    int no_trial_abandon = 0, pad_ = 0;
};

inline void finishGrid(GridDev& g) {
    for (int i = 0; i < 3; i++) { g.lo[i] = g.minb[i] + 1e-4; g.hi[i] = g.maxb[i] - 1e-4; }
    g.half_xy = 0.5 * g.xy_res; g.half_yaw = 0.5 * g.yaw_res;
}
inline void finishParams(OptParams& P) {
    P.max_vel2 = P.max_vel * P.max_vel; P.max_acc_lon2 = P.max_acc_lon * P.max_acc_lon;
    P.max_acc_lat2 = P.max_acc_lat * P.max_acc_lat; P.max_kap2 = P.max_kap * P.max_kap;
}

struct MincoOp {
    int N;
    const double* Wt;
    const double* Wr;
};

constexpr double FRAME_EXTENT = 32.0;
struct TrajFrame {
    double fo[2];
    double lo[2], hi[2];
    double shift[2];
    int ioff[2];
};
inline void applyFrame(GridDev& g, const TrajFrame& f) {
    g.origin[0] = f.fo[0]; g.origin[1] = f.fo[1];
    g.lo[0] = f.lo[0]; g.lo[1] = f.lo[1]; g.hi[0] = f.hi[0]; g.hi[1] = f.hi[1];
    g.ix_off = f.ioff[0]; g.iy_off = f.ioff[1];
}

struct TrajDesc {
    int Nxy, Nyaw, n, S;
    int op_xy, op_yaw;
    int64_t off_x;
    int64_t off_s;
    int64_t off_cxy, off_cyaw;
    int64_t off_hist;
    double init_xy[6], end_xy[6], init_yaw[3], end_yaw[3];
};

struct TrajState {
    double rho, scale_fx;
    double f, jerk_cost, T_xy, T_yaw;
    int ret_code, alm_iters, lbfgs_iters, evals, last_lbfgs_ret, pad;
    long long hist_reads;
    long long cyc[16];
    int ls_rejected, ls_guarded, ls_abandoned, chunks_skipped, adjoints_skipped, pad2;
};

struct BatchDev {
    int B;
    const TrajDesc* desc;
    TrajState* state;
    const MincoOp* ops;
    const double* x0;
    double* x;
    double* gout;
    double* dual;
    double* res;
    double* scl;
    double* cxy;
    double* cyaw;
    double* hist;
    double* rs_d;
    double* rs;
    double* report;
    double* pen_gxy;
    double* pen_gyaw;
    double* pen_out;
    double* trace;
    int trace_cap;
    const int* order;
    const OptParams* params_mem;
    const GridDev* grid_mem;
    int grid_per_traj;
    const double* thomas;
};

#if defined(__HIP_DEVICE_COMPILE__)
UPH_HD void pinv(double& v) { asm volatile("" : "+v"(v)); }
UPH_HD void pinv(float& v) { asm volatile("" : "+v"(v)); }
UPH_HD void pinv(int& v) { asm volatile("" : "+v"(v)); }
#else
UPH_HD void pinv(double&) {}
UPH_HD void pinv(float&) {}
UPH_HD void pinv(int&) {}
#endif
#ifndef UPH_DIET
#define UPH_DIET 0
#endif

UPH_HD double dmax(double a, double b) { return a > b ? a : b; }
UPH_HD double dmin(double a, double b) { return a < b ? a : b; }

UPH_HD double expC2(double tau) { return tau > 0.0 ? ((0.5 * tau + 1.0) * tau + 1.0) : 1.0 / ((0.5 * tau - 1.0) * tau + 1.0); }
UPH_HD double divR(double x, double y, double r) {
    const double q0 = x * r;
    return fma(fma(-q0, y, x), r, q0);
}
UPH_HD void mv2(const double* M, double v0, double v1, double& o0, double& o1) {
    o0 = fma(M[1], v1, M[0] * v0);
    o1 = fma(M[3], v1, M[2] * v0);
}
UPH_HD void submv2(double r0, double r1, const double* M, double p0, double p1, double& o0, double& o1) {
    o0 = fma(-M[1], p1, fma(-M[0], p0, r0));
    o1 = fma(-M[3], p1, fma(-M[2], p0, r1));
}
UPH_HD int histNQ(int n) { return (n + 63) >> 6; }
UPH_HD int histRowDoubles(int n) { return 2 + 128 * histNQ(n); }
constexpr int THOMAS_J = 26;
constexpr int THOMAS_STRIDE = 8;
constexpr int THOMAS_DOUBLES = (THOMAS_J + 1) * THOMAS_STRIDE;
constexpr int THOMAS_KPL = 4;
UPH_HD int knotOff(int q, int ks) { return ks * q + (q >> 2); }
UPH_HD int knotOffJ(int j, int ks) { return ks * j + ((j + 3) >> 2); }
UPH_HD int knotBufDoubles(int nknots, int ks) { return ks * nknots + (nknots >> 2) + 2; }
template <bool ADJ>
UPH_HD void thomasFactors(const double* tab, int j, double* P, double* M1, double* Q, double* M2) {
    const double* e = tab + (j < THOMAS_J ? j : THOMAS_J) * THOMAS_STRIDE;
    const double* en = tab + (j + 1 < THOMAS_J ? j + 1 : THOMAS_J) * THOMAS_STRIDE;
    const double D00 = e[4], D01 = e[5], D10 = e[6], D11 = e[7];
    if (!ADJ) {
        P[0] = 1.0; P[1] = 0.0; P[2] = 0.0; P[3] = 1.0;
        M1[0] = e[0]; M1[1] = e[1]; M1[2] = e[2]; M1[3] = e[3];
        Q[0] = D00; Q[1] = D01; Q[2] = D10; Q[3] = D11;
        M2[0] = fma(8.0, D00, -7.0 * D01); M2[1] = D01 - D00; M2[2] = fma(8.0, D10, -7.0 * D11); M2[3] = D11 - D10;
    } else {
        P[0] = D00; P[1] = D10; P[2] = D01; P[3] = D11;
        const double z = j == 1 ? 0.0 : 1.0;
        M1[0] = z * fma(8.0, D00, -D10); M1[1] = z * fma(-7.0, D00, D10); M1[2] = z * fma(8.0, D01, -D11); M1[3] = z * fma(-7.0, D01, D11);
        Q[0] = 1.0; Q[1] = 0.0; Q[2] = 0.0; Q[3] = 1.0;
        M2[0] = en[0]; M2[1] = en[2]; M2[2] = en[1]; M2[3] = en[3];
    }
}
#if defined(__HIP_DEVICE_COMPILE__)
static __device__ __constant__ const double UPH_SINCOS_TAB[16] = {
#else
static const double UPH_SINCOS_TAB[16] = {
#endif
    0x1.45f306dc9c883p-1,
    0x1.921fb54442d18p+0, 0x1.1a62633145c07p-54, -0x1.f1976b7ed8fbcp-110,
    -1.66666666666666324348e-01, 8.33333333332248946124e-03, -1.98412698298579493134e-04,
    2.75573137070700676789e-06, -2.50507602534068634195e-08, 1.58969099521155010221e-10,
    4.16666666666666019037e-02, -1.38888888888741095749e-03, 2.48015872894767294178e-05,
    -2.75573143513906633035e-07, 2.08757232129817482790e-09, -1.13596475577881948265e-11};
UPH_HD void sincosFast(double x, double& sn, double& cs) {
#if defined(__HIP_DEVICE_COMPILE__)
    typedef const __attribute__((address_space(4))) double* ctab_t;
    ctab_t T = (ctab_t)UPH_SINCOS_TAB;
    asm volatile("" : "+s"(T));
#else
    const double* T = UPH_SINCOS_TAB;
#endif
    const double q = rint(x * T[0]);
    const double t = fma(-q, T[1], x);
    const double w = q * T[2];
    const double r = t - w;
    double rt = (t - r) - w;
    rt = fma(-q, T[2], w) + rt;
// ... 82 lines not shown
```

### uneven_planner_amd/csrc/uph_ctx.hpp

```cpp
#pragma once
#include <hip/hip_runtime.h>

#include <map>
#include <string>
#include <vector>

#include "uph_internal.hpp"

using namespace uph;

struct DevBuf {
    void* p = nullptr;
    size_t cap = 0;
    int ensure(size_t bytes) {
        if (bytes <= cap) return 0;
        if (p) hipFree(p);
        p = nullptr; cap = 0;
        size_t want = bytes + bytes / 4 + 256;
        if (hipMalloc(&p, want) != hipSuccess) { setError("hipMalloc failed"); return -1; }
        cap = want;
        return 0;
    }
    void release() { if (p) hipFree(p); p = nullptr; cap = 0; }
    template <class T> T* as() { return (T*)p; }
};

struct HostBuf {
    void* p = nullptr;
    size_t cap = 0;
    int ensure(size_t bytes) {
        if (bytes <= cap) return 0;
        if (p) hipHostFree(p);
        p = nullptr; cap = 0;
        const size_t want = bytes + bytes / 4 + 256;
        if (hipHostMalloc(&p, want, hipHostMallocDefault) != hipSuccess) { setError("hipHostMalloc failed"); return -1; }
        cap = want;
        return 0;
    }
    void release() { if (p) hipHostFree(p); p = nullptr; cap = 0; }
    template <class T> T* as() { return (T*)p; }
};

struct ProblemHead {
    int32_t n_inner_xy = 0, n_inner_yaw = 0;
    int refused = 0;
    const char* why = nullptr;
    double init_xy[6], end_xy[6], init_yaw[3], end_yaw[3], total_time = 0.0;
    double lo[2], hi[2];
    double turn = 0.0, kink = 0.0;
};
struct uph_ctx {
    uph_map* map = nullptr;
    int device = 0;
    OptParams P;
    double rho = 1.0;
    hipStream_t stream = nullptr;
    hipEvent_t ev0 = nullptr, ev1 = nullptr;
    std::map<int, int> op_index;
    std::vector<MincoOp> ops_host;
    std::vector<void*> op_allocs;
    DevBuf d_ops;
    bool ops_dirty = false;
    int B = 0;
    std::vector<TrajDesc> desc;
    std::vector<int> order;
    int64_t sum_n = 0, sum_S = 0, sum_cxy = 0, sum_cyaw = 0, sum_hist = 0;
    size_t lds_bytes = 0;
    size_t lds_big = 0;
    int n_main = 0;
    std::vector<int> rejected;
    int n_rejected = 0;
    bool all_rejected = false;
    std::vector<TrajFrame> frames;
    std::vector<GridDev> grid_host_framed;
    GridDev frames_grid;
    GridDev framed_from;
    bool framed_valid = false;
    std::vector<int> origin;
    bool sample_f32 = false;
    int xcd_group = 0;
    hipStream_t stream2 = nullptr;
    hipEvent_t evp0 = nullptr, evp1 = nullptr;
    bool pending = false;
    hipEvent_t ev2 = nullptr;
    std::vector<size_t> fp_bytes;
    int lanes = 64;
    int lanes_forced = 0;
    int wps = 1;
    int wps_forced = 0;
    DevBuf d_thomas, d_rsd, d_rs, d_gridmem, d_parammem;
    GridDev grid_host;
    DevBuf d_desc, d_state, d_x, d_x0, d_gout, d_dual, d_res, d_scl, d_cxy, d_cyaw, d_hist, d_report, d_order, d_trace;
    DevBuf d_pen_gxy, d_pen_gyaw, d_pen_out;
    DevBuf d_roll_tt, d_roll_traj, d_roll_stage;
    bool traj_resident = false;
    DevBuf d_plan_head, d_plan_xy, d_plan_yaw, d_plan_goal, d_plan_rec;
    bool planned = false;
    std::vector<ProblemHead> plan_probs;
    std::vector<double> end_pose;
    std::vector<double> end_bnd;
    DevBuf d_sw_q, d_sw_out;
    DevBuf d_refine_rec;
    DevBuf d_win_q, d_win_out;
    double last_check_ms = 0.0;
    double last_locate_ms = 0.0;
    double last_sep_ms = 0.0;
    DevBuf d_delay;
    double last_delay_ms = 0.0;
    double last_foot_ms = 0.0;
    int trace_cap = 0;
    int trace_cap_up = 0;
    std::vector<TrajState> state_host;
    HostBuf h_x, h_cxy, h_cyaw, h_dual, h_res, h_scl;
    double last_ms = 0.0, last_prepare_ms = 0.0;
    int64_t last_evals = 0, last_sample_evals = 0, last_iters = 0, last_hist_bytes = 0;
    int64_t last_abandon[5] = {0, 0, 0, 0, 0};
};

#define HIPCHK(call)                                                                               \
    do {                                                                                           \
        hipError_t _e = (call);                                                                    \
        if (_e != hipSuccess) {                                                                    \
            setError(std::string(#call) + ": " + hipGetErrorString(_e));                           \
            return UPH_ERR_HIP;                                                                    \
        }                                                                                          \
    } while (0)

int refreshStates(uph_ctx* c);
int syncGridMem(uph_ctx* c, uph::GridDev& grid);

struct SwitchQuery {
    int32_t b, framed;
    double t;
    double shift[2];
};
constexpr int SWITCH_COLS = 9, TRAJ_STATE_COLS = 10;
int checkTrajQueries(const uph_ctx* c, int32_t n, const int32_t* traj, const double* t, const char* who);
SwitchQuery trajQuery(const uph_ctx* c, int32_t b, double t);
int launchTrajStates(uph_ctx* c, const std::vector<SwitchQuery>& sq, int cols = TRAJ_STATE_COLS);
```

Before: 53990.

## Add optional LDS staging of knot rows for scaling init and in-kernel state reset

Adds an optional path that stages the relevant Wr_xy/Wr_yaw knot rows into LDS in chunks before computing initial scaling samples, reading them from shared memory instead of global. The path is selected by a new ctx flag, with LDS capacity-driven chunk sizing and extra dynamic LDS at launch. Separately, the per-solve TrajState reset moves from a host memset plus H2D copy into the prepare kernel via reset flags in BatchDev. Staging adds LDS footprint and barriers, which could reduce occupancy when enabled.

```diff
diff --git a/include/uneven_hip.h b/include/uneven_hip.h
--- a/include/uneven_hip.h
+++ b/include/uneven_hip.h
@@ -220,6 +220,7 @@
 int uph_ctx_set_rho(uph_ctx* c, double rho);
 int uph_ctx_get_rho(uph_ctx* c, double* rho);
 int uph_ctx_set_trial_abandon(uph_ctx* c, int32_t on);
+int uph_ctx_set_scaling_stage(uph_ctx* c, int32_t on);
 
 int uph_ctx_set_trace(uph_ctx* c, int32_t cap);
 int uph_ctx_get_trace(uph_ctx* c, double* out);
diff --git a/uneven_planner_amd/_lib.py b/uneven_planner_amd/_lib.py
--- a/uneven_planner_amd/_lib.py
+++ b/uneven_planner_amd/_lib.py
@@ -124,6 +124,7 @@
     "uph_ctx_set_rho": (C.c_int, [_VP, C.c_double]),
     "uph_ctx_get_rho": (C.c_int, [_VP, DP]),
     "uph_ctx_set_trial_abandon": (C.c_int, [_VP, _I32]),
+    "uph_ctx_set_scaling_stage": (C.c_int, [_VP, _I32]),
     "uph_ctx_set_trace": (C.c_int, [_VP, _I32]),
     "uph_ctx_get_trace": (C.c_int, [_VP, DP]),
     "uph_optimize_batch": (C.c_int, [_VP, _I32, C.POINTER(Problem), C.POINTER(Result)]),
diff --git a/uneven_planner_amd/alm_traj_opt.py b/uneven_planner_amd/alm_traj_opt.py
--- a/uneven_planner_amd/alm_traj_opt.py
+++ b/uneven_planner_amd/alm_traj_opt.py
@@ -523,6 +523,9 @@
 
     def set_trial_abandon(self, on):
         _lib.check(self.L.uph_ctx_set_trial_abandon(self.h, 1 if on else 0), "uph_ctx_set_trial_abandon")
+
+    def set_scaling_stage(self, on):
+        _lib.check(self.L.uph_ctx_set_scaling_stage(self.h, 1 if on else 0), "uph_ctx_set_scaling_stage")
 
     def get_rho(self):
         r = C.c_double(0)
diff --git a/uneven_planner_amd/csrc/solver_program.hpp b/uneven_planner_amd/csrc/solver_program.hpp
--- a/uneven_planner_amd/csrc/solver_program.hpp
+++ b/uneven_planner_amd/csrc/solver_program.hpp
@@ -17,6 +17,15 @@
 #ifndef UPH_SCALING_WB
 #define UPH_SCALING_WB 8
 #endif
+#ifndef UPH_SCALING_GROUPS
+#define UPH_SCALING_GROUPS 2
+#endif
+#ifndef UPH_SCALING_WB_LDS
+#define UPH_SCALING_WB_LDS UPH_SCALING_WB
+#endif
+#ifndef UPH_SCALING_GROUPS_LDS
+#define UPH_SCALING_GROUPS_LDS UPH_SCALING_GROUPS
+#endif
 #ifndef UPH_SC_XB
 #define UPH_SC_XB 9
 #endif
@@ -37,6 +46,11 @@
 UPH_HD void asideKnotSolve(WG& wg, int lenW, int lenX, int n, F f) {
     (void)lenW; (void)lenX;
     wg.pfor(n, f);
+}
+template <class WG>
+UPH_HD const double* stageRows(WG& wg, double* dst, const double* src, int n) {
+    (void)wg; (void)dst; (void)n;
+    return src;
 }
 
 template <class WG, class SR = double>
@@ -55,6 +69,8 @@
     static constexpr int AB_DOUBLES = 4;
     double* up;
     static constexpr int UP_DOUBLES = 6;
+    double* stg;
+    static constexpr int STAGE_SLACK = 2;
     UPH_HD void tally(int k, bool yes) {
 #if defined(__HIP_DEVICE_COMPILE__)
         if (yes && wg.wave == 0) abn[k] = abn[k] + 1;
@@ -123,6 +139,7 @@
         ab = q; q += AB_DOUBLES;
         abn = (int*)(ab + 1);
         up = q; q += UP_DOUBLES;
+        stg = q + ((q - lds) & 1);
         dual = bd.dual + 7 * td.off_s; res = bd.res + 7 * td.off_s; scl = bd.scl + 7 * td.off_s;
         hist = bd.hist + td.off_hist; hrow = histRowDoubles(n); hnp = 64 * histNQ(n);
         Wr_xy = bd.ops[td.op_xy].Wr; Wr_yaw = bd.ops[td.op_yaw].Wr;
@@ -864,6 +881,7 @@
         return wg.bcast(jerk_cost + sm[0] + tau_cost);
     }
 
+    template <bool STAGE = true>
     UPH_HD void initScaling(double* x0) {
         generate<false>(x0, 0.0);
         const double tau = x0[0];
@@ -886,26 +904,79 @@
         });
         scale_fx = wg.bcast(1.0 / dmax(1.0, dmax(mq, fabs(gTau_fx))));
         wg.pfor(2, [&](int u) { fillTimes(u); });
-        wg.pfor(S, [&](int s) { scalingSample(s, dTau); });
-    }
-
-    UPH_HD void scalingSample(int s, double dTau) {
+        if constexpr (!STAGE) {
+            wg.pfor(S, [&](int s) { scalingSample<false>(s, dTau, nullptr, 0, nullptr, 0); });
+        } else {
+            const int nbx = Nxy + 5, nby = Nyaw + 5;
+            int cs = CH;
+            while (bd.stage_cap > 0 && cs > 1 && stageNeed(Nxy, Nyaw, K, cs) > (size_t)bd.stage_cap) cs >>= 1;
+            for (int s0 = 0; s0 < S; s0 += cs) {
+                const int cnt = S - s0 < cs ? S - s0 : cs;
+                int rx0, nx, ry0, ny;
+                stageRange(s0, cnt, rx0, nx, ry0, ny);
+                if (bd.stage_cap > 0 && (size_t)nx * nbx + (size_t)ny * nby > (size_t)bd.stage_cap) {
+                    if ((size_t)nx * nbx > (size_t)bd.stage_cap) nx = 0;
+                    ny = (int)(((size_t)bd.stage_cap - (size_t)nx * nbx) / nby) & ~1;
+                }
+                const double* sx = stageRows(wg, stg, Wr_xy + (size_t)rx0 * nbx, nx * nbx);
+                const double* sy = stageRows(wg, stg + nx * nbx, Wr_yaw + (size_t)ry0 * nby, ny * nby);
+                wg.sync();
+                wg.pfor(cnt, [&](int t) { scalingSample<true>(s0 + t, dTau, sx, rx0, sy, ry0); });
+            }
+        }
+    }
+    UPH_HD int yawPieceOf(int i, int j) const {
+        const double now_time = bt[Nxy + 1 + j] + bt[i];
+        int yi = toInt<double>(divR(now_time, Tyaw, ec_iTyaw));
+        if (yi >= Nyaw) yi = Nyaw - 1;
+        if (yi < 0) yi = 0;
+        return yi;
+    }
+    static UPH_HD void knotRows(int p0, int p1, int N, int& r0, int& nr) {
+        const int ka = p0 < 1 ? 1 : p0, kb = p1 + 1 > N - 1 ? N - 1 : p1 + 1;
+        if (kb < ka) { r0 = 0; nr = 2; }
+        else { r0 = 2 * (ka - 1); nr = 2 * (kb - ka + 1); }
+    }
+    UPH_HD void stageRange(int s0, int cnt, int& rx0, int& nx, int& ry0, int& ny) const {
+        const int K1 = K + 1;
+        const int i0 = s0 / K1, sl = s0 + cnt - 1, i1 = sl / K1;
+        knotRows(i0, i1, Nxy, rx0, nx);
+        int m0 = yawPieceOf(i0, s0 - i0 * K1) - 1, m1 = yawPieceOf(i1, sl - i1 * K1) + 1;
+        if (m0 < 0) m0 = 0;
+        if (m1 > Nyaw - 1) m1 = Nyaw - 1;
+        knotRows(m0, m1, Nyaw, ry0, ny);
+    }
+    static UPH_HD size_t stageNeed(int Nxy, int Nyaw, int K, int cs) {
+        const int K1 = K + 1;
+        int px = (cs + K1 - 2) / K1 + 1;
+        if (px > Nxy) px = Nxy;
+        int kx = px + 1 > Nxy - 1 ? Nxy - 1 : px + 1;
+        if (kx < 1) kx = 1;
+        int ky = cs == 1 ? 4 : (int)((double)(cs - 1) / (double)K * (double)Nyaw / (double)Nxy) + 6;
+        if (ky > Nyaw - 1) ky = Nyaw - 1;
+        if (ky < 1) ky = 1;
+        return (size_t)2 * kx * (Nxy + 5) + (size_t)2 * ky * (Nyaw + 5);
+    }
+
+    template <bool STAGE>
+    UPH_HD void scalingSample(int s, double dTau, const double* sx, int rx0, const double* sy, int ry0) {
         const int i = divSmall(s, K + 1, inv_k1), j = s - i * (K + 1);
         Kin k;
         kin(i, j, k);
-#if !defined(UPH_SCALING_GROUPS) || UPH_SCALING_GROUPS == 2
-        scalingGroup<0, 4>(s, i, j, k, dTau);
-        scalingGroup<4, 3>(s, i, j, k, dTau);
-#elif UPH_SCALING_GROUPS == 3
-        scalingGroup<0, 3>(s, i, j, k, dTau);
-        scalingGroup<3, 2>(s, i, j, k, dTau);
-        scalingGroup<5, 2>(s, i, j, k, dTau);
-#else
-        scalingGroup<0, 7>(s, i, j, k, dTau);
-#endif
-    }
-    template <int Q0, int NQS>
-    UPH_HD void scalingGroup(int s, int i, int j, const Kin& k, double dTau) {
+        constexpr int NG = STAGE ? UPH_SCALING_GROUPS_LDS : UPH_SCALING_GROUPS;
+        if constexpr (NG == 2) {
+            scalingGroup<0, 4, STAGE>(s, i, j, k, dTau, sx, rx0, sy, ry0);
+            scalingGroup<4, 3, STAGE>(s, i, j, k, dTau, sx, rx0, sy, ry0);
+        } else if constexpr (NG == 3) {
+            scalingGroup<0, 3, STAGE>(s, i, j, k, dTau, sx, rx0, sy, ry0);
+            scalingGroup<3, 2, STAGE>(s, i, j, k, dTau, sx, rx0, sy, ry0);
+            scalingGroup<5, 2, STAGE>(s, i, j, k, dTau, sx, rx0, sy, ry0);
+        } else {
+            scalingGroup<0, 7, STAGE>(s, i, j, k, dTau, sx, rx0, sy, ry0);
+        }
+    }
+    template <int Q0, int NQS, bool STAGE>
+    UPH_HD void scalingGroup(int s, int i, int j, const Kin& k, double dTau, const double* sx, int rx0, const double* sy, int ry0) {
         const int nbx = Nxy + 5, nby = Nyaw + 5;
         const double Tx = Txy, Ty = Tyaw, itx = 1.0 / Txy, ity = 1.0 / Tyaw;
         const double gravity = grid.gravity;
@@ -983,6 +1054,7 @@
                 ypR[qi] = 10.0 * g3 - 15.0 * g4 + 6.0 * g5; yvR[qi] = -4.0 * g3 + 7.0 * g4 - 3.0 * g5; yaR[qi] = 0.5 * g3 - g4 + 0.5 * g5;
             }
         }
+        if constexpr (!STAGE) {
         const bool inL = i >= 1, inR = i + 1 <= Nxy - 1;
         const auto WL = UPH_AS_GLOBAL(Wr_xy + (size_t)(inL ? 2 * (i - 1) : 0) * nbx);
         const auto WR = UPH_AS_GLOBAL(Wr_xy + (size_t)(inR ? 2 * i : 0) * nbx);
@@ -1088,6 +1160,115 @@
         for (int q = 0; q < NQS; q++) {
             const double gTau = ((sumx[q] + htx[q]) / Nxy + (sumy[q] + hty[q]) / Nyaw) * dTau;
             scl[(Q0 + q) * S + s] = 1.0 / dmax(1.0, dmax(mx[q], fabs(gTau)));
+        }
+        } else {
+        const bool inL = i >= 1, inR = i + 1 <= Nxy - 1;
+        const int pcL = knotCol(i, Nxy), pcR = knotCol(i + 1, Nxy);
+        const bool yL = m >= 1, yR = m + 1 <= Nyaw - 1;
+        const int qL = knotCol(m, Nyaw), qR = knotCol(m + 1, Nyaw);
+        constexpr int WB = STAGE ? UPH_SCALING_WB_LDS : UPH_SCALING_WB;
+        auto columns = [&](auto WL, auto WR, auto VL, auto VR) {
+        for (int c0 = 3; c0 < Nxy + 2; c0 += WB) {
+            double w[4][WB];
+#pragma unroll
+            for (int u = 0; u < WB; u++) {
+                const int cc = c0 + u < Nxy + 2 ? c0 + u : Nxy + 1;
+                w[0][u] = WL[cc]; w[1][u] = WL[nbx + cc]; w[2][u] = WR[cc]; w[3][u] = WR[nbx + cc];
+            }
+#pragma unroll
+            for (int q = 0; q < NQS; q++) {
+                const double c00 = inL ? dvL[q][0] : 0.0, c01 = inL ? dvL[q][1] : 0.0, c10 = inL ? daL[q][0] : 0.0, c11 = inL ? daL[q][1] : 0.0;
+                const double c20 = inR ? dvR[q][0] : 0.0, c21 = inR ? dvR[q][1] : 0.0, c30 = inR ? daR[q][0] : 0.0, c31 = inR ? daR[q][1] : 0.0;
+                double mq = mx[q];
+#pragma unroll
+                for (int u = 0; u < WB; u++) {
+                    const int col = c0 + u;
+                    double a0 = (w[0][u] * c00 + w[1][u] * c10) + (w[2][u] * c20 + w[3][u] * c30);
+                    double a1 = (w[0][u] * c01 + w[1][u] * c11) + (w[2][u] * c21 + w[3][u] * c31);
+                    if (col == pcL) { a0 += dpL[q][0]; a1 += dpL[q][1]; }
+                    if (col == pcR) { a0 += dpR[q][0]; a1 += dpR[q][1]; }
+                    if (col < Nxy + 2) mq = dmax(mq, dmax(fabs(a0), fabs(a1)));
+                }
+                mx[q] = mq;
+            }
+        }
+        double htx[NQS], hty[NQS];
+        {
+            const int sc[4] = {1, 2, Nxy + 3, Nxy + 4};
+            double w[4][4];
+#pragma unroll
+            for (int u = 0; u < 4; u++) { w[0][u] = WL[sc[u]]; w[1][u] = WL[nbx + sc[u]]; w[2][u] = WR[sc[u]]; w[3][u] = WR[nbx + sc[u]]; }
+#pragma unroll
+            for (int q = 0; q < NQS; q++) {
+                const double c00 = inL ? dvL[q][0] : 0.0, c01 = inL ? dvL[q][1] : 0.0, c10 = inL ? daL[q][0] : 0.0, c11 = inL ? daL[q][1] : 0.0;
+                const double c20 = inR ? dvR[q][0] : 0.0, c21 = inR ? dvR[q][1] : 0.0, c30 = inR ? daR[q][0] : 0.0, c31 = inR ? daR[q][1] : 0.0;
+                double a0[4], a1[4];
+#pragma unroll
+                for (int u = 0; u < 4; u++) {
+                    a0[u] = (w[0][u] * c00 + w[1][u] * c10) + (w[2][u] * c20 + w[3][u] * c30);
+                    a1[u] = (w[0][u] * c01 + w[1][u] * c11) + (w[2][u] * c21 + w[3][u] * c31);
+                }
+                if (!inL) { a0[0] += dvL[q][0]; a1[0] += dvL[q][1]; a0[1] += daL[q][0]; a1[1] += daL[q][1]; }
+                if (!inR) { a0[2] += dvR[q][0]; a1[2] += dvR[q][1]; a0[3] += daR[q][0]; a1[3] += daR[q][1]; }
+                double headtail_x = 0.0;
+                headtail_x += a0[0] * hd[2] + a1[0] * hd[3];
+                headtail_x += 2.0 * Tx * (a0[1] * hd[4] + a1[1] * hd[5]);
+                headtail_x += a0[2] * hd[8] + a1[2] * hd[9];
+                headtail_x += 2.0 * Tx * (a0[3] * hd[10] + a1[3] * hd[11]);
+                htx[q] = headtail_x;
+            }
+        }
+        for (int c0 = 3; c0 < Nyaw + 2; c0 += WB) {
+            double w[4][WB];
+#pragma unroll
+            for (int u = 0; u < WB; u++) {
+                const int cc = c0 + u < Nyaw + 2 ? c0 + u : Nyaw + 1;
+                w[0][u] = VL[cc]; w[1][u] = VL[nby + cc]; w[2][u] = VR[cc]; w[3][u] = VR[nby + cc];
+            }
+#pragma unroll
+            for (int q = 0; q < NQS; q++) {
+                const double y0_ = yL ? yvL[q] : 0.0, y1_ = yL ? yaL[q] : 0.0, y2_ = yR ? yvR[q] : 0.0, y3_ = yR ? yaR[q] : 0.0;
+                double mq = mx[q];
+#pragma unroll
+                for (int u = 0; u < WB; u++) {
+                    const int col = c0 + u;
+                    double a0 = (w[0][u] * y0_ + w[1][u] * y1_) + (w[2][u] * y2_ + w[3][u] * y3_);
+                    if (col == qL) a0 += ypL[q];
+                    if (col == qR) a0 += ypR[q];
+                    if (col < Nyaw + 2) mq = dmax(mq, fabs(a0));
+                }
+                mx[q] = mq;
+            }
+        }
+        {
+            const int sc[4] = {1, 2, Nyaw + 3, Nyaw + 4};
+            double w[4][4];
+#pragma unroll
+            for (int u = 0; u < 4; u++) { w[0][u] = VL[sc[u]]; w[1][u] = VL[nby + sc[u]]; w[2][u] = VR[sc[u]]; w[3][u] = VR[nby + sc[u]]; }
+#pragma unroll
+            for (int q = 0; q < NQS; q++) {
+                const double y0_ = yL ? yvL[q] : 0.0, y1_ = yL ? yaL[q] : 0.0, y2_ = yR ? yvR[q] : 0.0, y3_ = yR ? yaR[q] : 0.0;
+                double a0[4];
+#pragma unroll
+                for (int u = 0; u < 4; u++) a0[u] = (w[0][u] * y0_ + w[1][u] * y1_) + (w[2][u] * y2_ + w[3][u] * y3_);
+                if (!yL) { a0[0] += yvL[q]; a0[1] += yaL[q]; }
+                if (!yR) { a0[2] += yvR[q]; a0[3] += yaR[q]; }
+                double headtail_y = 0.0;
+                headtail_y += a0[0] * hd[13];
+                headtail_y += 2.0 * Ty * a0[1] * hd[14];
+                headtail_y += a0[2] * hd[16];
+                headtail_y += 2.0 * Ty * a0[3] * hd[17];
+                hty[q] = headtail_y;
+            }
+        }
+#pragma unroll
+        for (int q = 0; q < NQS; q++) {
+            const double gTau = ((sumx[q] + htx[q]) / Nxy + (sumy[q] + hty[q]) / Nyaw) * dTau;
+            scl[(Q0 + q) * S + s] = 1.0 / dmax(1.0, dmax(mx[q], fabs(gTau)));
+        }
+        };
+        columns(UPH_AS_STAGED(sx + (size_t)(inL ? 2 * (i - 1) - rx0 : 0) * nbx), UPH_AS_STAGED(sx + (size_t)(inR ? 2 * i - rx0 : 0) * nbx),
+                UPH_AS_STAGED(sy + (size_t)(yL ? 2 * (m - 1) - ry0 : 0) * nby), UPH_AS_STAGED(sy + (size_t)(yR ? 2 * m - ry0 : 0) * nby));
         }
     }
 
@@ -1301,17 +1482,25 @@
 #endif
     }
 
+    template <bool STAGE = true>
     UPH_HD void prepare(TrajState& st) {
         const double* gx0 = bd.x0 + td.off_x;
         double* gx = bd.x + td.off_x;
-        rho = wg.bcast(st.rho);
+        rho = wg.bcast(bd.reset_state ? bd.reset_rho : st.rho);
         scale_fx = 1.0;
-        wg.pfor(S > n ? S : n, [&](int t) {
+        constexpr int SW = (int)(sizeof(TrajState) / 8);
+        static_assert(sizeof(TrajState) % 8 == 0, "TrajState is reset in 8-byte words");
+        const int np = S > n ? S : n;
+        wg.pfor(np > SW ? np : SW, [&](int t) {
+            if (bd.reset_state && t < SW) {
+                const double v = t == 0 ? bd.reset_rho : 0.0;
+                __builtin_memcpy((char*)&st + 8 * t, &v, 8);
+            }
             if (t < n) { x[t] = gx0[t]; gx[t] = gx0[t]; }
             if (t < S) for (int q = 0; q < 7; q++) { dual[q * S + t] = 0.0; res[q * S + t] = 0.0; scl[q * S + t] = 1.0; }
         });
         const long long tstart = wg.clock();
-        if (P.use_scaling) initScaling(x);
+        if (P.use_scaling) initScaling<STAGE>(x);
         cyc[5] += wg.clock() - tstart;
         wg.pfor(1, [&](int) { st.scale_fx = scale_fx; st.cyc[5] = cyc[5]; });
     }
@@ -1470,11 +1659,12 @@
             else { double* o = bd.pen_out + (size_t)bidx * 3; o[0] = sm[0]; o[1] = sm[1]; o[2] = sm[2]; }
         });
     }
+    template <bool STAGE = true>
     UPH_HD void scalingOnly(TrajState& st) {
         const double* gx0 = bd.x + td.off_x;
         rho = wg.bcast(st.rho); scale_fx = 1.0;
         wg.pfor(n, [&](int t) { x[t] = gx0[t]; });
-        initScaling(x);
+        initScaling<STAGE>(x);
         storeTrajectory(st);
     }
 
diff --git a/uneven_planner_amd/csrc/unevenhip.hip b/uneven_planner_amd/csrc/unevenhip.hip
--- a/uneven_planner_amd/csrc/unevenhip.hip
+++ b/uneven_planner_amd/csrc/unevenhip.hip
@@ -111,6 +111,19 @@
         }
     }
     __device__ __forceinline__ void sync() { bar(0); }
+    __device__ __forceinline__ void stage(double* dst, const double* src, int n) {
+        typedef double d2_t __attribute__((ext_vector_type(2)));
+        const auto s = (const __attribute__((address_space(1))) d2_t*)src;
+        const auto d = (__attribute__((address_space(3))) d2_t*)dst;
+        const int n2 = uni(n) >> 1;
+        for (int i = ftid(); i < n2; i += 4 * NT) {
+            d2_t v[4];
+#pragma unroll
+            for (int u = 0; u < 4; u++) { const int k = i + u * NT; v[u] = s[k < n2 ? k : n2 - 1]; }
+#pragma unroll
+            for (int u = 0; u < 4; u++) { const int k = i + u * NT; if (k < n2) d[k] = v[u]; }
+        }
+    }
     __device__ __forceinline__ int size() const { return NT; }
 #ifndef UPH_CYC
 #define UPH_CYC 0
@@ -499,6 +512,8 @@
 
 template <int NT, class F>
 __device__ __forceinline__ void asideKnotSolve(DevWG<NT>& wg, int lenW, int lenX, int n, F f) { wg.aside(lenW, lenX, n, f); }
+template <int NT>
+__device__ __forceinline__ const double* stageRows(DevWG<NT>& wg, double* dst, const double* src, int n) { wg.stage(dst, src, n); return dst; }
 
 template <int NT, int WPS, int MODE, bool F32S = false>
 __global__ __launch_bounds__(NT, WPS) void uph_solver_kernel(GridDev grid, OptParams P, BatchDev bd, int repeat) {
@@ -511,13 +526,15 @@
     Solver<DevWG<NT>, SR> sol(wg, grid, P, bd, b, lds + DevWG<NT>::SCRATCH);
     TrajState& st = bd.state[b];
     if (MODE == 0) sol.evalOnly(st, repeat);
-    else if (MODE == 1) sol.prepare(st);
+    else if (MODE == 1) sol.template prepare<true>(st);
+    else if (MODE == 9) sol.template prepare<false>(st);
+    else if (MODE == 10) sol.template scalingOnly<false>(st);
     else if (MODE == 2) sol.optimize(st, repeat);
     else if (MODE == 7) sol.resumeHook(st, repeat >> 1, repeat & 1);
     else if (MODE == 8) { if (repeat & 1) sol.template penaltyOnly<true>(st, repeat >> 1); else sol.template penaltyOnly<false>(st, repeat >> 1); }
     else if (MODE == 3) sol.report(st);
     else if (MODE == 5) sol.microbench(st, repeat);
-    else sol.scalingOnly(st);
+    else sol.template scalingOnly<true>(st);
 }
 
 __global__ void uph_fill_kernel(double* __restrict__ p, size_t n, double v) {
@@ -698,6 +715,7 @@
     bd.grid_mem = c->d_gridmem.as<GridDev>();
     bd.params_mem = c->d_parammem.as<OptParams>();
     bd.rs_d = c->d_rsd.as<double>(); bd.rs = c->d_rs.as<double>();
+    bd.reset_state = c->reset_on_prepare ? 1 : 0; bd.reset_rho = c->rho;
     return bd;
 }
 
@@ -763,6 +781,21 @@
     if (c->d_parammem.ensure(sizeof(OptParams))) return UPH_ERR_HIP;
     HIPCHK(hipMemcpyAsync(c->d_parammem.p, &c->P, sizeof(OptParams), hipMemcpyHostToDevice, c->stream));
     BatchDev bd = makeBatchDev(c);
+    const bool scaling = mode == 1 || mode == 4;
+    const int km = scaling && !c->scaling_stage ? (mode == 1 ? 9 : 10) : mode;
+    size_t stage_cap[2] = {0, 0}, stage_bytes[2] = {0, 0};
+    if (scaling && c->scaling_stage) {
+        for (int k = 0; k < (c->n_main < c->B ? 2 : 1); k++) {
+            const size_t base = k == 0 ? c->lds_bytes : c->lds_big, slack = Solver<DevWG<64>>::STAGE_SLACK;
+            const size_t room = base + 8 * slack < 160 * 1024 ? (160 * 1024 - base) / 8 - slack : 0;
+            if (c->stage_min[k] > room) {
+                setError("the operator rows of initScaling do not fit the LDS next to this batch's largest trajectory: uph_ctx_set_scaling_stage(c, 0) reads them from global memory");
+                return UPH_ERR_LIMIT;
+            }
+            stage_cap[k] = std::min(c->stage_full[k], room);
+            stage_bytes[k] = 8 * (stage_cap[k] + slack);
+        }
+    }
 #define UPH_LAUNCH(NTL, WPS, MODE)                                                                                                     \
     do {                                                                                                                             \
         const size_t ldsmax = 160 * 1024;    \
@@ -770,24 +803,28 @@
         HIPCHK(hipEventRecord(evb, c->stream));                                                                                   \
         BatchDev bm = bd;                                                                                                            \
         bm.B = c->n_main;                                                                                                            \
+        bm.stage_cap = (int)stage_cap[0];                                                                                            \
         if (c->n_main < c->B) {            \
             BatchDev bb = bd;              \
             bb.B = c->B - c->n_main;                                                                                                 \
             bb.order = bd.order + c->n_main;                                                                                         \
+            bb.stage_cap = (int)stage_cap[1];                                                                                        \
             HIPCHK(hipStreamWaitEvent(c->stream2, evb, 0));                                                                       \
-            hipLaunchKernelGGL((uph_solver_kernel<NTL, WPS, MODE>), dim3(bb.B), dim3(NTL), c->lds_big, c->stream2, grid, c->P, bb, repeat); \
+            hipLaunchKernelGGL((uph_solver_kernel<NTL, WPS, MODE>), dim3(bb.B), dim3(NTL), c->lds_big + stage_bytes[1], c->stream2, grid, c->P, bb, repeat); \
             HIPCHK(hipEventRecord(c->ev2, c->stream2));                                                                              \
         }                                                                                                                            \
-        hipLaunchKernelGGL((uph_solver_kernel<NTL, WPS, MODE>), dim3(c->n_main), dim3(NTL), c->lds_bytes, c->stream, grid, c->P, bm, repeat); \
+        hipLaunchKernelGGL((uph_solver_kernel<NTL, WPS, MODE>), dim3(c->n_main), dim3(NTL), c->lds_bytes + stage_bytes[0], c->stream, grid, c->P, bm, repeat); \
         if (c->n_main < c->B) HIPCHK(hipStreamWaitEvent(c->stream, c->ev2, 0));                                                      \
     } while (0)
 #define UPH_LAUNCH_MODE(NTL, WPS)                                                                                                      \
     do {                                                                                                                             \
-        if (mode == 0) UPH_LAUNCH(NTL, WPS, 0);                                                                                      \
-        else if (mode == 1) UPH_LAUNCH(NTL, WPS, 1);                                                                                 \
-        else if (mode == 2) UPH_LAUNCH(NTL, WPS, 2);                                                                                 \
-        else if (mode == 3) UPH_LAUNCH(NTL, WPS, 3);                                                                                 \
-        else if (mode == 5) UPH_LAUNCH(NTL, WPS, 5);                                                                                 \
+        if (km == 0) UPH_LAUNCH(NTL, WPS, 0);                                                                                        \
+        else if (km == 1) UPH_LAUNCH(NTL, WPS, 1);                                                                                   \
+        else if (km == 2) UPH_LAUNCH(NTL, WPS, 2);                                                                                   \
+        else if (km == 3) UPH_LAUNCH(NTL, WPS, 3);                                                                                   \
+        else if (km == 5) UPH_LAUNCH(NTL, WPS, 5);                                                                                   \
+        else if (km == 9) UPH_LAUNCH(NTL, WPS, 9);                                                                                   \
+        else if (km == 10) UPH_LAUNCH(NTL, WPS, 10);                                                                                 \
         else UPH_LAUNCH(NTL, WPS, 4);                                                                                                \
     } while (0)
 #define UPH_LAUNCH32(NTL, WPS, MODE)                                                                                                   \
@@ -828,7 +865,8 @@
     }
     else if (c->lanes == 64 && c->wps_forced == 2) UPH_LAUNCH_MODE(64, 2);
     else if (c->lanes == 64) UPH_LAUNCH_MODE(64, 1);
-    else if (c->lanes == 128 && mode == 1) UPH_LAUNCH(128, 1, 1);
+    else if (c->lanes == 128 && km == 9) UPH_LAUNCH(128, 1, 9);
+    else if (c->lanes == 128 && km == 1) UPH_LAUNCH(128, 1, 1);
     else if (c->lanes == 128) UPH_LAUNCH_MODE(128, UPH_WPS128);
     else if (c->lanes == 512) UPH_LAUNCH_MODE(512, 1);
     else if (c->wps == 2 && mode == 2 && c->lds_bytes <= 80 * 1024) UPH_LAUNCH(256, 2, 2);
@@ -945,6 +983,7 @@
 }
 int uph_ctx_set_rho(uph_ctx* c, double rho) { if (!c) return UPH_ERR_INVALID; c->rho = rho; return UPH_OK; }
 int uph_ctx_set_trial_abandon(uph_ctx* c, int32_t on) { if (!c || (on != 0 && on != 1)) return UPH_ERR_INVALID; c->P.no_trial_abandon = on ? 0 : 1; return UPH_OK; }
+int uph_ctx_set_scaling_stage(uph_ctx* c, int32_t on) { if (!c || (on != 0 && on != 1)) return UPH_ERR_INVALID; c->scaling_stage = on != 0; return UPH_OK; }
 int uph_ctx_get_rho(uph_ctx* c, double* rho) { if (!c || !rho) return UPH_ERR_INVALID; *rho = c->rho; return UPH_OK; }
 
 int uph_ctx_set_trace(uph_ctx* c, int32_t cap) { if (!c || cap < 0) return UPH_ERR_INVALID; c->trace_cap = cap; return UPH_OK; }
@@ -1128,6 +1167,12 @@
             std::stable_partition(c->order.begin(), c->order.end(), [&](int a) { return c->fp_bytes[a] <= limit; });
             c->n_main = B - nbig; c->lds_bytes = mmain; c->lds_big = mbig;
         }
+        for (int k = 0; k < 2; k++) c->stage_full[k] = c->stage_min[k] = 0;
+        for (int b = 0; b < B; b++) {
+            const int k = c->lds_big > 0 && c->fp_bytes[b] > limit ? 1 : 0;
+            c->stage_full[k] = std::max(c->stage_full[k], Solver<DevWG<64>>::stageNeed(c->desc[b].Nxy, c->desc[b].Nyaw, c->P.int_K, c->lanes));
+            c->stage_min[k] = std::max(c->stage_min[k], Solver<DevWG<64>>::stageNeed(c->desc[b].Nxy, c->desc[b].Nyaw, c->P.int_K, 1));
+        }
     }
     c->state_host.assign(B, TrajState());
     for (int b = 0; b < B; b++) { std::memset(&c->state_host[b], 0, sizeof(TrajState)); c->state_host[b].rho = c->rho; c->state_host[b].scale_fx = 1.0; }
@@ -1452,9 +1497,9 @@
     if (!c || c->B <= 0) { setError("uph_batch_solve_async: no batch uploaded"); return UPH_ERR_INVALID; }
     if (c->pending) { setError("uph_batch_solve_async: the previous asynchronous solve has not been waited for"); return UPH_ERR_INVALID; }
     HIPCHK(hipSetDevice(uphMapDevice(c->map)));
-    for (int b = 0; b < c->B; b++) { std::memset(&c->state_host[b], 0, sizeof(TrajState)); c->state_host[b].rho = c->rho; c->state_host[b].scale_fx = 1.0; }
-    HIPCHK(hipMemcpyAsync(c->d_state.p, c->state_host.data(), sizeof(TrajState) * c->B, hipMemcpyHostToDevice, c->stream));
+    c->reset_on_prepare = true;
     int r = launchSolver(c, 1, 1, true, c->evp0, c->evp1);
+    c->reset_on_prepare = false;
     if (r != UPH_OK) { hipStreamSynchronize(c->stream); return r; }
     r = launchSolver(c, 2, 0, true, c->ev0, c->ev1);
     if (r != UPH_OK) { hipStreamSynchronize(c->stream); if (c->stream2) hipStreamSynchronize(c->stream2); return r; }
diff --git a/uneven_planner_amd/csrc/uph_common.hpp b/uneven_planner_amd/csrc/uph_common.hpp
--- a/uneven_planner_amd/csrc/uph_common.hpp
+++ b/uneven_planner_amd/csrc/uph_common.hpp
@@ -14,6 +14,11 @@
 #define UPH_AS_GLOBAL(p) ((const __attribute__((address_space(1))) double*)(p))
 #else
 #define UPH_AS_GLOBAL(p) (p)
+#endif
+#if defined(__HIP_DEVICE_COMPILE__)
+#define UPH_AS_STAGED(p) ((const __attribute__((address_space(3))) double*)(p))
+#else
+#define UPH_AS_STAGED(p) (p)
 #endif
 
 #if defined(UPH_ISA_MARKS) && defined(__HIP_DEVICE_COMPILE__)
@@ -159,6 +164,9 @@
     const GridDev* grid_mem;
     int grid_per_traj;
     const double* thomas;
+    int reset_state;
+    double reset_rho;
+    int stage_cap;
 };
 
 #if defined(__HIP_DEVICE_COMPILE__)
diff --git a/uneven_planner_amd/csrc/uph_ctx.hpp b/uneven_planner_amd/csrc/uph_ctx.hpp
--- a/uneven_planner_amd/csrc/uph_ctx.hpp
+++ b/uneven_planner_amd/csrc/uph_ctx.hpp
@@ -49,6 +49,9 @@
     double lo[2], hi[2];
     double turn = 0.0, kink = 0.0;
 };
+#ifndef UPH_SCALING_STAGE_DEFAULT
+#define UPH_SCALING_STAGE_DEFAULT 0
+#endif
 struct uph_ctx {
     uph_map* map = nullptr;
     int device = 0;
@@ -68,6 +71,10 @@
     size_t lds_bytes = 0;
     size_t lds_big = 0;
     int n_main = 0;
+    bool reset_on_prepare = false;
+    bool scaling_stage = UPH_SCALING_STAGE_DEFAULT != 0;
+    size_t stage_full[2] = {0, 0};
+    size_t stage_min[2] = {0, 0};
     std::vector<int> rejected;
     int n_rejected = 0;
     bool all_rejected = false;
```

Measured after the change: 54060, median of 6. About the same (+0.1%).
